# choyingw/SynergyNet

Hardware: AMD Instinct MI355X
Metric: faces/sec (120x120, 68-lmk + 53215-vert) (higher is better)
Workload: dtype f32 (fp16x2 split operands, fp32 accumulate)

## Files before the change

include/synergy_hip.h:

```cpp
#ifndef SYNERGY_HIP_H
#define SYNERGY_HIP_H

#include <stddef.h>
#include <stdint.h>

#ifdef __cplusplus
extern "C" {
#endif

typedef struct syn_handle syn_handle;

typedef enum {
    SYN_OK = 0,
    SYN_ERR_INVALID = -1,
    SYN_ERR_HIP = -2,
    SYN_ERR_NOT_LOADED = -3,
    SYN_ERR_PARAM_LEN = -4
} syn_status;

#define SYN_PARAM_DIM 62
#define SYN_POOL_DIM 1280
#define SYN_STD_SIZE 120

const char *syn_last_error(void);
int syn_abi_version(void);

int syn_create(int device, syn_handle **out);
int syn_destroy(syn_handle *h);


size_t syn_backbone_flat_count(void);

int syn_load_backbone(syn_handle *h, const float *flat, size_t n_floats);

int syn_numerics_report(syn_handle *h, char *buf, size_t n);

int syn_set_schedule(syn_handle *h, int fusion);

int syn_backbone_calibrate(syn_handle *h, const uint8_t *crops_u8, int B, float tol, void *stream);

int syn_backbone_range_status(syn_handle *h, float *layer_max, int max_layers, int fallback);
int syn_backbone_range_events(syn_handle *h);

size_t syn_resnet50_flat_count(void);
int syn_load_backbone_resnet50(syn_handle *h, const float *flat, size_t n_floats);
double syn_resnet50_flops_per_face(void);

int syn_load_basis(syn_handle *h, const float *w_shp, const float *w_exp, const float *u,
                   const float *param_mean, const float *param_std,
                   const int64_t *keypoints, int n_lmk, int n_vert);

size_t syn_constants_bytes(syn_handle *h);
int syn_export_constants(syn_handle *h, void *dev_dst, size_t bytes, void *stream);
int syn_import_constants(syn_handle *h, const void *dev_src, size_t bytes, void *stream);
int syn_bcast_constants(syn_handle *h, void *nccl_comm, int root, void *stream);
int syn_describe_constants(syn_handle *h, void *host_header, size_t bytes);

size_t syn_pack_constants_host_bytes(int arch, int have_backbone, int n_vert, int n_lmk);
int syn_pack_constants_host(int arch, const float *backbone_flat, size_t n_floats, const float *w_shp, const float *w_exp,
                            const float *u, const float *param_mean, const float *param_std, const int64_t *keypoints,
                            int n_lmk, int n_vert, void *host_dst, size_t bytes);
int syn_check_constants_host(const void *host_blob, size_t bytes);


size_t syn_workspace_bytes(syn_handle *h, int B);

int syn_backbone_forward(syn_handle *h, const float *img, int B, float *param, float *pool,
                         void *stream);

int syn_backbone_forward_u8(syn_handle *h, const uint8_t *img_hwc, int B, float *param,
                            float *pool, void *stream);

int syn_crop_resize(syn_handle *h, const uint8_t *frame, int H, int W, const int *box, const int *xofs,
                    const int16_t *xcoef, const int *yofs, const int16_t *ycoef, uint8_t *out, int B, void *stream);

int syn_crop_resize_frames(syn_handle *h, const uint8_t *frames, const long long *frame_off, const int *frame_dim,
                           const int *face_frame, const int *box, const int *xofs, const int16_t *xcoef, const int *yofs,
                           const int16_t *ycoef, uint8_t *out, int B, void *stream);

int syn_reconstruct(syn_handle *h, const float *param, int B, int param_len, int dense,
                    int transform, const float *roi, float *out, void *stream);

int syn_reconstruct_pitched(syn_handle *h, const float *param, int B, int param_len, int dense,
                            int transform, const float *roi, float *out, int row_pitch, int pad_writable, void *stream);

int syn_load_triangles(syn_handle *h, const int32_t *tri, int ntri, int nver);

int syn_mesh_shade(syn_handle *h, const float *vertices, int F, int planar, const float *cfg16, float *normal,
                   float *light, void *stream);

int syn_rasterize(syn_handle *h, const float *vertices, const float *colors, int F, int planar, int channels,
                  uint8_t *image, int H, int W, int reverse, void *stream);

int syn_add_weighted(syn_handle *h, const uint8_t *a, float alpha, const uint8_t *b, float beta, uint8_t *out,
                     size_t n, void *stream);

int syn_load_uv_map(syn_handle *h, const int32_t *coord_u, const int32_t *coord_v, int nver, const int32_t *keep_ind, int n_keep,
                    const int32_t *tri_kept, int ntri_kept);

int syn_select_topology(syn_handle *h, int slot);

int syn_uv_colors(syn_handle *h, const uint8_t *uv_tex, int T, int tex_h, int tex_w, int channels, int kept, int normalize, float *out,
                  void *stream);

int syn_gather_vertices(syn_handle *h, const float *vertices, int F, int planar, float *out, void *stream);

int syn_mesh_shade_textured(syn_handle *h, const float *vertices, int F, int planar, const float *cfg16, float *normal, float *light,
                            float *tex, int shared, float *colors, void *stream);

int syn_rasterize_triangles(syn_handle *h, const float *vertices, int F, int planar, float *depth_buffer, int32_t *triangle_buffer,
                            float *barycentric_weight, int H, int W, void *stream);

int syn_vertex_visibility(syn_handle *h, const int32_t *triangle_buffer, int F, int H, int W, uint8_t *visible, void *stream);

int syn_sample_vertex_colors(syn_handle *h, const float *vertices, int F, int planar, const uint8_t *image, int H, int W, int channels,
                             int normalize, float *out, void *stream);

int syn_uv_scatter(syn_handle *h, const float *colors, const uint8_t *visible, int F, int channels, uint8_t *tex, uint8_t *mask, int tex_h,
                   int tex_w, void *stream);

int syn_texture_fill(syn_handle *h, const uint8_t *tex_in, const uint8_t *mask, int T, int tex_h, int tex_w, int channels, int merge,
                     uint8_t *tex_out, void *stream);

int syn_load_tex_coords(syn_handle *h, const float *tex_coords, int tex_nver, const int32_t *tex_triangles);

int syn_render_texture(syn_handle *h, const float *vertices, int F, int planar, const void *texture, int tex_u8, int T, int tex_h, int tex_w,
                       int tex_c, int mapping_type, void *image, int image_u8, float *depth_buffer, int H, int W, int c, int shared,
                       void *stream);

size_t syn_detector_flat_count(void);
int syn_load_detector(syn_handle *h, const float *flat, size_t count);
int syn_detector_prior_count(int Hs, int Ws);
int syn_detect(syn_handle *h, const uint8_t *frame, int H, int W, int Hs, int Ws, float scale, float conf_thr, float nms_thr,
               int top_k, int keep_top_k, float *dets, int *n_dets, void *stream);

int syn_nme(syn_handle *h, const float *fit, const float *gt, const float *roi, float *nme, int N, void *stream);

int syn_pose(syn_handle *h, const float *param, int B, const float *roi, double *angles,
             float *t3d, void *stream);

int syn_landmarks_pose(syn_handle *h, const float *param, int B, int param_len, int transform, const float *roi ,
                       float *lmk, double *angles , float *t3d , void *stream);

int syn_pose_matrix(syn_handle *h, const float *param, int B, float *pmat, void *stream);

size_t syn_synergy_flat_count(void);
size_t syn_synergy_folded_count(void);
int syn_fold_synergy_host(const float *flat, size_t n, float *folded, size_t n_folded);

int syn_load_synergy(syn_handle *h, const float *flat, size_t n);

int syn_refine_landmarks(syn_handle *h, const float *param , const float *pool , int B, int transform,
                         const float *roi , float *lmk_coarse , float *lmk_refined ,
                         float *global_feat , void *stream);

int syn_refine_points(syn_handle *h, const float *lmk , const float *pool, const float *param, int B, float *lmk_refined,
                      float *global_feat , void *stream);

int syn_landmarks_to_param(syn_handle *h, const float *lmk , int B, float *param , void *stream);


int syn_backbone_launch_count(syn_handle *h);

int syn_backbone_profile(syn_handle *h, const uint8_t *img_hwc, int B, int max_launches,
                         int *feature_of_launch, float *ms_of_launch, double *flops_of_launch);

int syn_reconstruct_profile(syn_handle *h, const float *param, int B, const float *roi, float *out, int row_pitch, int pad_writable,
                            float *ms2);

double syn_backbone_flops_per_face(void);
double syn_pointwise_flops_per_face(void);

#ifdef __cplusplus
}
#endif
#endif
```

synergynet_amd/abi.py:

```python
from __future__ import annotations

import ctypes as C
import os

import torch

from .build import LIB

SYN_ERR_INVALID, SYN_ERR_NOT_LOADED = -1, -3
SYN_ERR_PARAM_LEN = -4
_lib = None


class SynergyHipError(RuntimeError):
    def __init__(self, code, msg):
        super().__init__(f'libsynergy_hip: {msg} (status {code})')
        self.code = code
        self.msg = msg


_SIGS = {
    'syn_last_error': (C.c_char_p, []),
    'syn_abi_version': (C.c_int, []),
    'syn_create': (C.c_int, [C.c_int, C.POINTER(C.c_void_p)]),
    'syn_destroy': (C.c_int, [C.c_void_p]),
    'syn_backbone_flat_count': (C.c_size_t, []),
    'syn_load_backbone': (C.c_int, [C.c_void_p, C.c_void_p, C.c_size_t]),
    'syn_numerics_report': (C.c_int, [C.c_void_p, C.c_char_p, C.c_size_t]),
    'syn_set_schedule': (C.c_int, [C.c_void_p, C.c_int]),
    'syn_backbone_range_status': (C.c_int, [C.c_void_p, C.c_void_p, C.c_int, C.c_int]),
    'syn_backbone_range_events': (C.c_int, [C.c_void_p]),
    'syn_backbone_calibrate': (C.c_int, [C.c_void_p, C.c_void_p, C.c_int, C.c_float, C.c_void_p]),
    'syn_resnet50_flat_count': (C.c_size_t, []),
    'syn_load_backbone_resnet50': (C.c_int, [C.c_void_p, C.c_void_p, C.c_size_t]),
    'syn_resnet50_flops_per_face': (C.c_double, []),
    'syn_load_basis': (C.c_int, [C.c_void_p] + [C.c_void_p] * 6 + [C.c_int, C.c_int]),
    'syn_constants_bytes': (C.c_size_t, [C.c_void_p]),
    'syn_export_constants': (C.c_int, [C.c_void_p, C.c_void_p, C.c_size_t, C.c_void_p]),
    'syn_import_constants': (C.c_int, [C.c_void_p, C.c_void_p, C.c_size_t, C.c_void_p]),
    'syn_bcast_constants': (C.c_int, [C.c_void_p, C.c_void_p, C.c_int, C.c_void_p]),
    'syn_describe_constants': (C.c_int, [C.c_void_p, C.c_void_p, C.c_size_t]),
    'syn_pack_constants_host_bytes': (C.c_size_t, [C.c_int, C.c_int, C.c_int, C.c_int]),
    'syn_pack_constants_host': (C.c_int, [C.c_int, C.c_void_p, C.c_size_t] + [C.c_void_p] * 6 + [C.c_int, C.c_int, C.c_void_p, C.c_size_t]),
    'syn_check_constants_host': (C.c_int, [C.c_void_p, C.c_size_t]),
    'syn_workspace_bytes': (C.c_size_t, [C.c_void_p, C.c_int]),
    'syn_backbone_forward': (C.c_int, [C.c_void_p, C.c_void_p, C.c_int, C.c_void_p, C.c_void_p, C.c_void_p]),
    'syn_backbone_forward_u8': (C.c_int, [C.c_void_p, C.c_void_p, C.c_int, C.c_void_p, C.c_void_p, C.c_void_p]),
    'syn_crop_resize': (C.c_int, [C.c_void_p, C.c_void_p, C.c_int, C.c_int] + [C.c_void_p] * 6 + [C.c_int, C.c_void_p]),
    'syn_crop_resize_frames': (C.c_int, [C.c_void_p] * 11 + [C.c_int, C.c_void_p]),
    'syn_detector_flat_count': (C.c_size_t, []),
    'syn_load_detector': (C.c_int, [C.c_void_p, C.c_void_p, C.c_size_t]),
    'syn_detector_prior_count': (C.c_int, [C.c_int, C.c_int]),
    'syn_detect': (C.c_int, [C.c_void_p, C.c_void_p, C.c_int, C.c_int, C.c_int, C.c_int, C.c_float, C.c_float, C.c_float, C.c_int, C.c_int,
                             C.c_void_p, C.POINTER(C.c_int), C.c_void_p]),
    'syn_nme': (C.c_int, [C.c_void_p, C.c_void_p, C.c_void_p, C.c_void_p, C.c_void_p, C.c_int, C.c_void_p]),
    'syn_load_triangles': (C.c_int, [C.c_void_p, C.c_void_p, C.c_int, C.c_int]),
    'syn_mesh_shade': (C.c_int, [C.c_void_p, C.c_void_p, C.c_int, C.c_int, C.c_void_p, C.c_void_p, C.c_void_p, C.c_void_p]),
    'syn_rasterize': (C.c_int, [C.c_void_p, C.c_void_p, C.c_void_p, C.c_int, C.c_int, C.c_int, C.c_void_p, C.c_int, C.c_int, C.c_int, C.c_void_p]),
    'syn_add_weighted': (C.c_int, [C.c_void_p, C.c_void_p, C.c_float, C.c_void_p, C.c_float, C.c_void_p, C.c_size_t, C.c_void_p]),
    'syn_load_uv_map': (C.c_int, [C.c_void_p, C.c_void_p, C.c_void_p, C.c_int, C.c_void_p, C.c_int, C.c_void_p, C.c_int]),
    'syn_select_topology': (C.c_int, [C.c_void_p, C.c_int]),
    'syn_uv_colors': (C.c_int, [C.c_void_p, C.c_void_p, C.c_int, C.c_int, C.c_int, C.c_int, C.c_int, C.c_int, C.c_void_p, C.c_void_p]),
    'syn_gather_vertices': (C.c_int, [C.c_void_p, C.c_void_p, C.c_int, C.c_int, C.c_void_p, C.c_void_p]),
    'syn_mesh_shade_textured': (C.c_int, [C.c_void_p, C.c_void_p, C.c_int, C.c_int, C.c_void_p, C.c_void_p, C.c_void_p, C.c_void_p, C.c_int,
                                          C.c_void_p, C.c_void_p]),
    'syn_rasterize_triangles': (C.c_int, [C.c_void_p, C.c_void_p, C.c_int, C.c_int, C.c_void_p, C.c_void_p, C.c_void_p, C.c_int, C.c_int, C.c_void_p]),
    'syn_vertex_visibility': (C.c_int, [C.c_void_p, C.c_void_p, C.c_int, C.c_int, C.c_int, C.c_void_p, C.c_void_p]),
    'syn_sample_vertex_colors': (C.c_int, [C.c_void_p, C.c_void_p, C.c_int, C.c_int, C.c_void_p, C.c_int, C.c_int, C.c_int, C.c_int, C.c_void_p,
                                           C.c_void_p]),
    'syn_uv_scatter': (C.c_int, [C.c_void_p, C.c_void_p, C.c_void_p, C.c_int, C.c_int, C.c_void_p, C.c_void_p, C.c_int, C.c_int, C.c_void_p]),
    'syn_texture_fill': (C.c_int, [C.c_void_p, C.c_void_p, C.c_void_p, C.c_int, C.c_int, C.c_int, C.c_int, C.c_int, C.c_void_p, C.c_void_p]),
    'syn_load_tex_coords': (C.c_int, [C.c_void_p, C.c_void_p, C.c_int, C.c_void_p]),
    'syn_render_texture': (C.c_int, [C.c_void_p, C.c_void_p, C.c_int, C.c_int, C.c_void_p, C.c_int, C.c_int, C.c_int, C.c_int, C.c_int, C.c_int,
                                     C.c_void_p, C.c_int, C.c_void_p, C.c_int, C.c_int, C.c_int, C.c_int, C.c_void_p]),
    'syn_reconstruct': (C.c_int, [C.c_void_p, C.c_void_p, C.c_int, C.c_int, C.c_int, C.c_int, C.c_void_p, C.c_void_p, C.c_void_p]),
    'syn_reconstruct_pitched': (C.c_int, [C.c_void_p, C.c_void_p, C.c_int, C.c_int, C.c_int, C.c_int, C.c_void_p, C.c_void_p, C.c_int, C.c_int, C.c_void_p]),
    'syn_pose': (C.c_int, [C.c_void_p, C.c_void_p, C.c_int, C.c_void_p, C.c_void_p, C.c_void_p, C.c_void_p]),
    'syn_landmarks_pose': (C.c_int, [C.c_void_p, C.c_void_p, C.c_int, C.c_int, C.c_int, C.c_void_p, C.c_void_p, C.c_void_p, C.c_void_p, C.c_void_p]),
    'syn_pose_matrix': (C.c_int, [C.c_void_p, C.c_void_p, C.c_int, C.c_void_p, C.c_void_p]),
    'syn_synergy_flat_count': (C.c_size_t, []),
    'syn_synergy_folded_count': (C.c_size_t, []),
    'syn_fold_synergy_host': (C.c_int, [C.c_void_p, C.c_size_t, C.c_void_p, C.c_size_t]),
    'syn_load_synergy': (C.c_int, [C.c_void_p, C.c_void_p, C.c_size_t]),
    'syn_refine_landmarks': (C.c_int, [C.c_void_p, C.c_void_p, C.c_void_p, C.c_int, C.c_int, C.c_void_p, C.c_void_p, C.c_void_p, C.c_void_p, C.c_void_p]),
    'syn_refine_points': (C.c_int, [C.c_void_p, C.c_void_p, C.c_void_p, C.c_void_p, C.c_int, C.c_void_p, C.c_void_p, C.c_void_p]),
    'syn_landmarks_to_param': (C.c_int, [C.c_void_p, C.c_void_p, C.c_int, C.c_void_p, C.c_void_p]),
    'syn_backbone_launch_count': (C.c_int, [C.c_void_p]),
    'syn_backbone_profile': (C.c_int, [C.c_void_p, C.c_void_p, C.c_int, C.c_int, C.c_void_p, C.c_void_p, C.c_void_p]),
    'syn_reconstruct_profile': (C.c_int, [C.c_void_p, C.c_void_p, C.c_int, C.c_void_p, C.c_void_p, C.c_int, C.c_int, C.c_void_p]),
    'syn_backbone_flops_per_face': (C.c_double, []),
    'syn_pointwise_flops_per_face': (C.c_double, []),
}

EXPORTED_SYMBOLS = tuple(_SIGS)
_SIGS = dict(_SIGS, syn_debug_feature=(C.c_int, [C.c_void_p, C.c_void_p, C.c_int, C.c_int, C.c_void_p, C.c_void_p]),
             syn_debug_profile_block=(C.c_int, [C.c_void_p, C.c_void_p, C.c_int, C.c_int, C.c_void_p]),
             syn_debug_detect_raw=(C.c_int, [C.c_void_p, C.c_void_p, C.c_int, C.c_int, C.c_int, C.c_int, C.c_float] + [C.c_void_p] * 5),
             syn_debug_poison_workspace=(C.c_int, [C.c_void_p, C.c_int, C.c_int]))


def lib():
    global _lib
    if _lib is None:
        path = os.environ.get('SYNERGY_HIP_LIB', LIB)
        if not os.path.isfile(path):
            raise SynergyHipError(-100, f'{path} not built; run `python -c "import __graft_entry__ as g; g.build()"`')
        l = C.CDLL(path)
        for name, (res, args) in _SIGS.items():
            fn = getattr(l, name)
            fn.restype, fn.argtypes = res, args
        _lib = l
    return _lib


def check(rc: int):
    if rc != 0:
        msg = lib().syn_last_error().decode(errors='replace')
        raise SynergyHipError(rc, msg)
```

synergynet_amd/csrc/head_kernel.hip:

```cpp
#include <cstdlib>

#include "syn_internal.h"

namespace syn {

typedef float f32x4 __attribute__((ext_vector_type(4)));

namespace {
constexpr int NF = 2, PX = NF * 16, K = 320, KCH = K / 16, N = 1280, NTL = N / 16, XS = K + 4;
__device__ __forceinline__ float r6h(float v) { return __builtin_amdgcn_fmed3f(v, 0.0f, 6.0f); }
__device__ __forceinline__ float row16_sum(float v) {
    v += __builtin_bit_cast(float, __builtin_amdgcn_update_dpp(0, __builtin_bit_cast(int, v), 0xB1, 0xF, 0xF, true));
    v += __builtin_bit_cast(float, __builtin_amdgcn_update_dpp(0, __builtin_bit_cast(int, v), 0x4E, 0xF, 0xF, true));
    v += __builtin_bit_cast(float, __builtin_amdgcn_update_dpp(0, __builtin_bit_cast(int, v), 0x141, 0xF, 0xF, true));
    v += __builtin_bit_cast(float, __builtin_amdgcn_update_dpp(0, __builtin_bit_cast(int, v), 0x140, 0xF, 0xF, true));
    return v;
}
__device__ __forceinline__ float wave64_sum(float v) {
    const int b = __builtin_bit_cast(int, row16_sum(v));
    return __builtin_bit_cast(float, __builtin_amdgcn_readlane(b, 0)) + __builtin_bit_cast(float, __builtin_amdgcn_readlane(b, 16)) +
           __builtin_bit_cast(float, __builtin_amdgcn_readlane(b, 32)) + __builtin_bit_cast(float, __builtin_amdgcn_readlane(b, 48));
}
}

__global__ __launch_bounds__(256) void head_kernel(const float *__restrict__ X , const float *__restrict__ Wpk,
                                                   const float *__restrict__ scale, const float *__restrict__ shift,
                                                   const float *__restrict__ Wfc , const float *__restrict__ bfc,
                                                   float *__restrict__ param, float *__restrict__ pool, int B) {
    __shared__ __attribute__((aligned(16))) float Xs[PX * XS];
    __shared__ __attribute__((aligned(16))) float Ps[NF * N];
    const int tid = threadIdx.x, lane = tid & 63, wave = __builtin_amdgcn_readfirstlane(tid >> 6);
    const int r16 = lane & 15, g = lane >> 4;
    const int f0 = blockIdx.x * NF;
    const f32x4 z4 = {0.f, 0.f, 0.f, 0.f};

    f32x4 an[KCH], hn;
    auto fetch = [&](int nt) {
        const float *w = Wpk + (size_t)nt * KCH * 256 + lane * 4;
#pragma unroll
        for (int kc = 0; kc < KCH; ++kc) an[kc] = *(const f32x4 *)(w + kc * 256);
        hn = *(const f32x4 *)&shift[nt * 16 + 4 * g];
    };
    fetch(wave);
    for (int it = tid; it < PX * (K / 4); it += 256) {
        const int c4 = it % (K / 4), p = it / (K / 4);
        const int f = f0 + (p >> 4);
        f32x4 v = z4;
        if (f < B) v = *(const f32x4 *)&X[((size_t)f * 16 + (p & 15)) * K + 4 * c4];
        *(f32x4 *)&Xs[p * XS + 4 * c4] = v;
    }
    __syncthreads();

    for (int nt = wave; nt < NTL; nt += 4) {
        f32x4 a[KCH];
#pragma unroll
        for (int kc = 0; kc < KCH; ++kc) a[kc] = an[kc];
        const f32x4 sh = hn;
        if (nt + 4 < NTL) fetch(nt + 4);
        f32x4 acc[NF];
#pragma unroll
        for (int j = 0; j < NF; ++j) acc[j] = sh;
        f32x4 bc[NF], bn[NF];
#pragma unroll
        for (int j = 0; j < NF; ++j) bc[j] = *(const f32x4 *)&Xs[(j * 16 + r16) * XS + 4 * g];
#pragma unroll
        for (int kc = 0; kc < KCH; ++kc) {
            if (kc + 1 < KCH) {
#pragma unroll
                for (int j = 0; j < NF; ++j) bn[j] = *(const f32x4 *)&Xs[(j * 16 + r16) * XS + (kc + 1) * 16 + 4 * g];
            }
#pragma unroll
            for (int s = 0; s < 4; ++s)
#pragma unroll
                for (int j = 0; j < NF; ++j) acc[j] = __builtin_amdgcn_mfma_f32_16x16x4f32(a[kc][s], bc[j][s], acc[j], 0, 0, 0);
#pragma unroll
            for (int j = 0; j < NF; ++j) bc[j] = bn[j];
            __builtin_amdgcn_sched_barrier(0);
        }
#pragma unroll
        for (int j = 0; j < NF; ++j) {
            f32x4 v;
#pragma unroll
            for (int t = 0; t < 4; ++t) v[t] = r6h(acc[j][t]);
#pragma unroll
            for (int t = 0; t < 4; ++t) v[t] = row16_sum(v[t]);
            if (r16 == 0) *(f32x4 *)&Ps[j * N + nt * 16 + 4 * g] = v * 0.0625f;
        }
    }
    __syncthreads();
    if (pool) {
        for (int it = tid; it < NF * (N / 4); it += 256) {
            const int j = it / (N / 4), c4 = it % (N / 4);
            if (f0 + j < B) *(f32x4 *)&pool[(size_t)(f0 + j) * N + 4 * c4] = *(const f32x4 *)&Ps[j * N + 4 * c4];
        }
    }
    {
        f32x4 xv[NF][N / 256];
#pragma unroll
        for (int j = 0; j < NF; ++j)
#pragma unroll
            for (int i = 0; i < N / 256; ++i) xv[j][i] = *(const f32x4 *)&Ps[j * N + (i * 64 + lane) * 4];
#pragma unroll 2
        for (int o = wave; o < kParam; o += 4) {
            const float *wr = Wfc + (size_t)o * N;
            f32x4 wv[N / 256];
#pragma unroll
            for (int i = 0; i < N / 256; ++i) wv[i] = *(const f32x4 *)&wr[(i * 64 + lane) * 4];
            const float bo = bfc[o];
#pragma unroll
            for (int j = 0; j < NF; ++j) {
                float a = 0.f;
#pragma unroll
                for (int i = 0; i < N / 256; ++i)
                    a += wv[i][0] * xv[j][i][0] + wv[i][1] * xv[j][i][1] + wv[i][2] * xv[j][i][2] + wv[i][3] * xv[j][i][3];
                const float tot = wave64_sum(a);
                if (lane == 0 && f0 + j < B) param[(size_t)(f0 + j) * kParam + o] = tot + bo;
            }
        }
    }
}

void launch_head(const float *X, const float *Wpk, const float *scale, const float *shift, const float *Wfc,
                 const float *bfc, float *param, float *pool, int B, hipStream_t s) {
    head_kernel<<<(B + NF - 1) / NF, 256, 0, s>>>(X, Wpk, scale, shift, Wfc, bfc, param, pool, B);
}


typedef _Float16 f16x8 __attribute__((ext_vector_type(8)));
typedef _Float16 f16x2 __attribute__((ext_vector_type(2)));
typedef unsigned u32x4 __attribute__((ext_vector_type(4)));
typedef unsigned u32x2 __attribute__((ext_vector_type(2)));

namespace {
constexpr int KC32 = K / 32;
constexpr int XSD = K / 2 + 4;
constexpr int PLANE = PX * XSD;
__device__ __forceinline__ void split2(float x0, float x1, unsigned &a, unsigned &b) {
    a = __builtin_bit_cast(unsigned, __builtin_amdgcn_cvt_pkrtz(x0, x1));
    float r0, r1;
    asm("v_fma_mix_f32 %0, %1, -1.0, %2 op_sel_hi:[1,0,0]" : "=v"(r0) : "v"(a), "v"(x0));
    asm("v_fma_mix_f32 %0, %1, -1.0, %2 op_sel:[1,0,0] op_sel_hi:[1,0,0]" : "=v"(r1) : "v"(a), "v"(x1));
    b = __builtin_bit_cast(unsigned, __builtin_amdgcn_cvt_pkrtz(r0, r1));
}
__device__ __forceinline__ f32x4 mfma_h(u32x4 a, u32x4 b, f32x4 c) {
    return __builtin_amdgcn_mfma_f32_16x16x32_f16(__builtin_bit_cast(f16x8, a), __builtin_bit_cast(f16x8, b), c, 0, 0, 0);
}
}

template <int NR, int NFK = NF, int NWV = 4>
__device__ __forceinline__ void fc_rows(const f32x4 (&xv)[NFK][N / 256], const float *__restrict__ Wfc, const float *__restrict__ bfc,
                                        float *__restrict__ param, int f0, int B, int rbase, int wave, int lane) {
    f32x4 wq[2][N / 256];
    auto ldw = [&](int o, f32x4(&w)[N / 256]) {
        const float *wr = Wfc + (size_t)(o < kParam ? o : kParam - 1) * N;
#pragma unroll
        for (int i = 0; i < N / 256; ++i) w[i] = *(const f32x4 *)&wr[(i * 64 + lane) * 4];
    };
    ldw(wave + NWV * rbase, wq[0]);
#pragma unroll
    for (int r = 0; r < NR; ++r) {
        const int o = wave + NWV * (rbase + r);
        if (r + 1 < NR) ldw(o + NWV, wq[(r + 1) & 1]);
        if (o >= kParam) continue;
        const f32x4(&wv)[N / 256] = wq[r & 1];
        const float bo = bfc[o];
#pragma unroll
        for (int j = 0; j < NFK; ++j) {
            float a = 0.f;
#pragma unroll
            for (int i = 0; i < N / 256; ++i)
                a += wv[i][0] * xv[j][i][0] + wv[i][1] * xv[j][i][1] + wv[i][2] * xv[j][i][2] + wv[i][3] * xv[j][i][3];
            const float tot = wave64_sum(a);
            if (lane == 0 && f0 + j < B) param[(size_t)(f0 + j) * kParam + o] = tot + bo;
        }
    }
}

constexpr int kFcRounds = (kParam + 3) / 4;

template <int NS, int NFK = NF, int NWV = 4, bool SIN = false>
__global__ __launch_bounds__(NWV * 64) void head_f16x2_kernel(const float *__restrict__ X ,
                                                          const unsigned *__restrict__ Wb3 ,
                                                          const float *__restrict__ shift, const float *__restrict__ Wfc,
                                                          const float *__restrict__ bfc, float *__restrict__ param,
                                                          float *__restrict__ pool, int B, HeadSliced hs = HeadSliced{nullptr, 0, nullptr, nullptr}) {
    constexpr int PXK = NFK * 16, PLANEK = PXK * XSD, NT = NWV * 64;
    __shared__ __attribute__((aligned(16))) unsigned Xb[2 * PLANEK];
    __shared__ __attribute__((aligned(16))) float Ps[NFK * N];
    const int tid = threadIdx.x, lane = tid & 63, wave = __builtin_amdgcn_readfirstlane(tid >> 6);
    const int r16 = lane & 15, g = lane >> 4;
    const int gsw = g ^ (((r16 >> 2) ^ (r16 >> 3)) & 1);
    const int f0 = blockIdx.x * NFK;
    const float S = __builtin_bit_cast(float, Wb3[80 * 10 * 2 * 256]), inv_s = __builtin_bit_cast(float, Wb3[80 * 10 * 2 * 256 + 1]);
    constexpr int NTS = NTL / NS;
    static_assert(NTL % NS == 0 && NTS % NWV == 0, "whole rounds of the waves per slice");
    const int nt0 = NS > 1 ? (int)blockIdx.y * NTS : 0, nt_end = nt0 + NTS;

    u32x4 ring[5][2];
    auto lda = [&](int nt, int kc, u32x4(&dst)[2]) {
        const unsigned *w = Wb3 + ((size_t)(nt * KC32 + kc) * 2) * 256 + lane * 4;
#pragma unroll
        for (int p = 0; p < 2; ++p) dst[p] = *(const u32x4 *)(w + p * 256);
    };
#pragma unroll
    for (int kc = 0; kc < 5; ++kc) lda(nt0 + wave, kc, ring[kc]);
    {
        constexpr int XI = PXK * (K / 4) / NT;
        static_assert(PXK * (K / 4) % NT == 0, "whole rounds");
        f32x4 xv[XI];
        if constexpr (SIN) {
            const size_t total = (size_t)B * 16 * K;
            size_t at[XI];
#pragma unroll
            for (int ii = 0; ii < XI; ++ii) {
                const int it = tid + ii * NT, c4 = it % (K / 4), p = it / (K / 4);
                int f = f0 + (p >> 4);
                f = f < B ? f : B - 1;
                at[ii] = ((size_t)f * 16 + (p & 15)) * K + 4 * c4;
                xv[ii] = *(const f32x4 *)&hs.part[at[ii]];
            }
            for (int sl = 1; sl < hs.S; sl += 2) {
                const bool two = sl + 1 < hs.S;
                f32x4 t0[XI], t1[XI];
#pragma unroll
                for (int ii = 0; ii < XI; ++ii) t0[ii] = *(const f32x4 *)&hs.part[(size_t)sl * total + at[ii]];
#pragma unroll
                for (int ii = 0; ii < XI; ++ii) t1[ii] = *(const f32x4 *)&hs.part[(size_t)(two ? sl + 1 : sl) * total + at[ii]];
#pragma unroll
                for (int ii = 0; ii < XI; ++ii) { xv[ii] += t0[ii]; if (two) xv[ii] += t1[ii]; }
            }
            const float inv_p = *hs.inv_p;
#pragma unroll
            for (int ii = 0; ii < XI; ++ii) {
                const int c4 = (tid + ii * NT) % (K / 4);
                xv[ii] = xv[ii] * inv_p + *(const f32x4 *)&hs.p_shift[4 * c4];
            }
        } else {
#pragma unroll
        for (int ii = 0; ii < XI; ++ii) {
            const int it = tid + ii * NT, c4 = it % (K / 4), p = it / (K / 4);
            int f = f0 + (p >> 4);
            f = f < B ? f : B - 1;
            xv[ii] = *(const f32x4 *)&X[((size_t)f * 16 + (p & 15)) * K + 4 * c4];
        }
        }
#pragma unroll
        for (int ii = 0; ii < XI; ++ii) asm volatile("" : "+v"(xv[ii]));
#pragma unroll
        for (int ii = 0; ii < XI; ++ii) {
            const int it = tid + ii * NT, c4 = it % (K / 4), p = it / (K / 4);
            const f32x4 v = f0 + (p >> 4) < B ? xv[ii] : (f32x4){0.f, 0.f, 0.f, 0.f};
            unsigned a0, b0, a1, b1;
            split2(v[0], v[1], a0, b0);
            split2(v[2], v[3], a1, b1);
            const int csw = ((((c4 >> 1) ^ ((((p & 15) >> 2) ^ ((p & 15) >> 3)) & 1)) << 1) | (c4 & 1)) * 2;
            *(u32x2 *)&Xb[0 * PLANEK + p * XSD + csw] = (u32x2){a0, a1};
            *(u32x2 *)&Xb[1 * PLANEK + p * XSD + csw] = (u32x2){b0, b1};
        }
    }
    __syncthreads();

    f32x4 sh_n = *(const f32x4 *)&shift[(nt0 + wave) * 16 + 4 * g];
    auto tile = [&](int nt) __attribute__((always_inline)) {
        const f32x4 sh = sh_n * S;
        sh_n = *(const f32x4 *)&shift[(nt + NWV < nt_end ? nt + NWV : nt) * 16 + 4 * g];
        f32x4 acc[NFK];
#pragma unroll
        for (int j = 0; j < NFK; ++j) acc[j] = sh;
        u32x4 bq[2][NFK][2];
        auto ldb = [&](int kc, u32x4(&b)[NFK][2]) {
#pragma unroll
            for (int j = 0; j < NFK; ++j)
#pragma unroll
                for (int p = 0; p < 2; ++p) b[j][p] = *(const u32x4 *)&Xb[p * PLANEK + (j * 16 + r16) * XSD + kc * 16 + 4 * gsw];
        };
        ldb(0, bq[0]);
#pragma unroll
        for (int kc = 0; kc < KC32; ++kc) {
            if (kc + 1 < KC32) ldb(kc + 1, bq[(kc + 1) & 1]);
            const u32x4(&bc)[NFK][2] = bq[kc & 1];
            const u32x4 aa = ring[kc % 5][0], ab = ring[kc % 5][1];
#pragma unroll
            for (int j = 0; j < NFK; ++j) acc[j] = mfma_h(ab, bc[j][0], acc[j]);
#pragma unroll
            for (int j = 0; j < NFK; ++j) acc[j] = mfma_h(aa, bc[j][1], acc[j]);
#pragma unroll
            for (int j = 0; j < NFK; ++j) acc[j] = mfma_h(aa, bc[j][0], acc[j]);
            if (kc + 5 < KC32) lda(nt, kc + 5, ring[kc % 5]);
            else lda(nt + NWV < nt_end ? nt + NWV : nt, kc + 5 - KC32, ring[kc % 5]);
            __builtin_amdgcn_sched_barrier(0);
        }
#pragma unroll
        for (int j = 0; j < NFK; ++j) {
            f32x4 v;
#pragma unroll
            for (int t = 0; t < 4; ++t) v[t] = row16_sum(r6h(acc[j][t] * inv_s));
            if (r16 == 0) *(f32x4 *)&Ps[j * N + nt * 16 + 4 * g] = v * 0.0625f;
        }
    };
    tile(nt0 + wave);
    for (int nt = nt0 + wave + NWV; nt < nt_end; nt += NWV) tile(nt);
    __syncthreads();
    if (NS > 1) {
        for (int it = tid; it < NFK * (NTS * 4); it += NT) {
            const int j = it / (NTS * 4), c4 = nt0 * 4 + it % (NTS * 4);
            if (f0 + j < B) *(f32x4 *)&pool[(size_t)(f0 + j) * N + 4 * c4] = *(const f32x4 *)&Ps[j * N + 4 * c4];
        }
        return;
    }
    if (pool) {
        for (int it = tid; it < NFK * (N / 4); it += NT) {
            const int j = it / (N / 4), c4 = it % (N / 4);
            if (f0 + j < B) *(f32x4 *)&pool[(size_t)(f0 + j) * N + 4 * c4] = *(const f32x4 *)&Ps[j * N + 4 * c4];
        }
    }
    f32x4 xv[NFK][N / 256];
#pragma unroll
    for (int j = 0; j < NFK; ++j)
#pragma unroll
        for (int i = 0; i < N / 256; ++i) xv[j][i] = *(const f32x4 *)&Ps[j * N + (i * 64 + lane) * 4];
    fc_rows<(kParam + NWV - 1) / NWV, NFK, NWV>(xv, Wfc, bfc, param, f0, B, 0, wave, lane);
}

constexpr int kFcSlices = 4;
__global__ __launch_bounds__(256) void head_fc_kernel(const float *__restrict__ pool, const float *__restrict__ Wfc,
                                                      const float *__restrict__ bfc, float *__restrict__ param, int B) {
    const int tid = threadIdx.x, lane = tid & 63, wave = __builtin_amdgcn_readfirstlane(tid >> 6);
    const int f0 = blockIdx.x * NF;
    f32x4 xv[NF][N / 256];
#pragma unroll
    for (int j = 0; j < NF; ++j) {
        const int f = f0 + j < B ? f0 + j : B - 1;
#pragma unroll
        for (int i = 0; i < N / 256; ++i) xv[j][i] = *(const f32x4 *)&pool[(size_t)f * N + (i * 64 + lane) * 4];
    }
    fc_rows<kFcRounds / kFcSlices>(xv, Wfc, bfc, param, f0, B, blockIdx.y * (kFcRounds / kFcSlices), wave, lane);
}

void launch_head_f16x2(const float *X, const unsigned *Wb3, const float *shift, const float *Wfc, const float *bfc,
                        float *param, float *pool, float *scratch, int B, hipStream_t s, const HeadSliced *sin) {
    const int grid = (B + NF - 1) / NF;
    if (grid <= 96) {
        float *pl = pool ? pool : scratch;
        if (sin) head_f16x2_kernel<5, NF, 4, true><<<dim3(grid, 5), 256, 0, s>>>(X, Wb3, shift, Wfc, bfc, param, pl, B, *sin);
        else head_f16x2_kernel<5><<<dim3(grid, 5), 256, 0, s>>>(X, Wb3, shift, Wfc, bfc, param, pl, B);
        head_fc_kernel<<<dim3(grid, kFcSlices), 256, 0, s>>>(pl, Wfc, bfc, param, B);
        return;
    }
    if (sin) {
        head_f16x2_kernel<1, NF, 4, true><<<grid, 256, 0, s>>>(X, Wb3, shift, Wfc, bfc, param, pool, B, *sin);
        return;
    }
    static const int wide_min = (int)test_knob("head_wide_min", 513);
    if (B >= wide_min) {
        head_f16x2_kernel<1, 4, 8><<<(B + 3) / 4, 512, 0, s>>>(X, Wb3, shift, Wfc, bfc, param, pool, B);
        return;
    }
    head_f16x2_kernel<1><<<grid, 256, 0, s>>>(X, Wb3, shift, Wfc, bfc, param, pool, B);
}
}
```

synergynet_amd/csrc/recon_kernels.hip:

```cpp
#include <cstdio>
#include <cstdlib>

#include "syn_internal.h"

namespace syn {

typedef float f32x2 __attribute__((ext_vector_type(2)));
typedef float f32x4 __attribute__((ext_vector_type(4)));
typedef float f32x16 __attribute__((ext_vector_type(16)));

__device__ __forceinline__ void lds_barrier() { asm volatile("s_waitcnt lgkmcnt(0)\n\ts_barrier" ::: "memory"); }

constexpr int kFaceRec = 64;
constexpr int kStageStride = 132;

__global__ __launch_bounds__(64) void recon_prep_kernel(const float *__restrict__ param, const float *__restrict__ mean,
                                                        const float *__restrict__ stdv, const float *__restrict__ roi,
                                                        int transform, float *__restrict__ rec, int B) {
    const int b = blockIdx.x;
    const int l = threadIdx.x;
    __shared__ float p[64];
    if (l < kParam) p[l] = param[(size_t)b * kParam + l] * stdv[l] + mean[l];
    __syncthreads();
    float *r = rec + (size_t)b * kFaceRec;
    if (l < 50) r[l] = p[12 + l];
    else if (l == 50) r[l] = 1.0f;
    else if (l == 51) r[l] = 0.0f;
    else if (l < 55) {
        const int c = l - 52;
        float sc = 1.0f, of = 0.0f;
        if (roi) {
            const float sx = roi[b * 5 + 0], sy = roi[b * 5 + 1], ex = roi[b * 5 + 2], ey = roi[b * 5 + 3];
            const float scx = (ex - sx) / 120.0f, scy = (ey - sy) / 120.0f;
            if (c == 0) { sc = scx; of = sx; }
            else if (c == 1) { sc = scy; of = sy; }
            else { sc = (scx + scy) * 0.5f; }
        }
        float m0 = p[4 * c + 0], m1 = p[4 * c + 1], m2 = p[4 * c + 2], t = p[4 * c + 3];
        if (transform && c == 1) { m0 = -m0; m1 = -m1; m2 = -m2; t = (float)(kImg + 1) - t; }
        r[52 + 3 * c + 0] = m0 * sc;
        r[52 + 3 * c + 1] = m1 * sc;
        r[52 + 3 * c + 2] = m2 * sc;
        r[61 + c] = t * sc + of;
    }
}

__global__ __launch_bounds__(256) void recon_kernel(const float *__restrict__ rec, const float *__restrict__ basis,
                                                    float *__restrict__ out, int B, int n_vert, int pitch, int n_tiles,
                                                    int n_split, int ftiles_per_split, int n_ftiles, int n_units) {
    __shared__ __attribute__((aligned(16))) float smt[4][32][12];
    __shared__ __attribute__((aligned(16))) float stage[96 * kStageStride];
    const int lane = threadIdx.x & 63, wave = __builtin_amdgcn_readfirstlane(threadIdx.x >> 6);
    const int per_xcd = (n_units + 7) / 8;
    const int unit = (blockIdx.x & 7) * per_xcd + (blockIdx.x >> 3);
    if ((int)(blockIdx.x >> 3) >= per_xcd || unit >= n_units) return;
    const int tg = unit / n_split, split = unit - tg * n_split;
    int T = tg * 4 + wave;
    const bool t_ok = T < n_tiles;
    T = t_ok ? T : n_tiles - 1;
    const int j = lane & 31, h = lane >> 5;

    f32x4 bw[3][6];
    f32x2 bt[3];
    const float *bp = basis + (size_t)T * 3 * (kBasisK * 32);
#pragma unroll
    for (int c = 0; c < 3; ++c) {
        const float *bc = bp + c * (kBasisK * 32);
#pragma unroll
        for (int t = 0; t < 6; ++t) bw[c][t] = *(const f32x4 *)(bc + t * 256 + lane * 4);
        bt[c] = *(const f32x2 *)(bc + 6 * 256 + lane * 2);
    }
    const int ft0 = split * ftiles_per_split;
    int ft1 = ft0 + ftiles_per_split;
    ft1 = ft1 < n_ftiles ? ft1 : n_ftiles;
    float(*mt)[12] = smt[wave];
    const int v_base = tg * 128;
    if ((blockIdx.x >> 8) & 1) __builtin_amdgcn_s_sleep(56);

    for (int ft = ft0; ft < ft1; ++ft) {
        const int f0 = ft * 32;
        int fa = f0 + j;
        fa = fa < B ? fa : B - 1;
        const float *ra = rec + (size_t)fa * kFaceRec;
        f32x4 aw[6];
#pragma unroll
        for (int t = 0; t < 6; ++t) aw[t] = *(const f32x4 *)(ra + 8 * t + 4 * h);
        const f32x2 at = *(const f32x2 *)(ra + 48 + 2 * h);
        if (lane < 32) {
#pragma unroll
            for (int q = 0; q < 3; ++q) *(f32x4 *)&mt[lane][4 * q] = *(const f32x4 *)(ra + 52 + 4 * q);
        }
        f32x16 acc[3];
#pragma unroll
        for (int c = 0; c < 3; ++c) {
#pragma unroll
            for (int r = 0; r < 16; ++r) acc[c][r] = 0.f;
#pragma unroll
            for (int t = 0; t < 6; ++t)
#pragma unroll
                for (int s = 0; s < 4; ++s)
                    acc[c] = __builtin_amdgcn_mfma_f32_32x32x2f32(aw[t][s], bw[c][t][s], acc[c], 0, 0, 0);
#pragma unroll
            for (int s = 0; s < 2; ++s) acc[c] = __builtin_amdgcn_mfma_f32_32x32x2f32(at[s], bt[c][s], acc[c], 0, 0, 0);
        }
        __builtin_amdgcn_fence(__ATOMIC_RELEASE, "wavefront");
        __builtin_amdgcn_wave_barrier();
        __builtin_amdgcn_fence(__ATOMIC_ACQUIRE, "wavefront");
#pragma unroll
        for (int r = 0; r < 16; ++r) {
            const int i = (r & 3) + 8 * (r >> 2) + 4 * h;
            const f32x4 q0 = *(const f32x4 *)&mt[i][0];
            const f32x4 q1 = *(const f32x4 *)&mt[i][4];
            const f32x4 q2 = *(const f32x4 *)&mt[i][8];
            const float sx = acc[0][r], sy = acc[1][r], sz = acc[2][r];
            float *st = stage + (i * 3) * kStageStride + wave * 32 + j;
            st[0] = q0[0] * sx + q0[1] * sy + q0[2] * sz + q2[1];
            st[kStageStride] = q0[3] * sx + q1[0] * sy + q1[1] * sz + q2[2];
            st[2 * kStageStride] = q1[2] * sx + q1[3] * sy + q2[0] * sz + q2[3];
        }
        lds_barrier();
        {
            const int seg = threadIdx.x & 31, rsub = threadIdx.x >> 5;
            const int vq = v_base + 4 * seg;
#pragma unroll
            for (int k = 0; k < 12; ++k) {
                const int row = k * 8 + rsub;
                const int f = f0 + row / 3, c = row % 3;
                const f32x4 vv = *(const f32x4 *)&stage[row * kStageStride + 4 * seg];
                if (f < B) {
                    float *o = out + ((size_t)f * 3 + c) * pitch + vq;
                    if (vq + 3 < n_vert) *(f32x4 *)o = vv;
                    else {
#pragma unroll
                        for (int t = 0; t < 4; ++t) if (vq + t < n_vert) o[t] = vv[t];
                    }
                }
            }
        }
        lds_barrier();
    }
}

void launch_reconstruct(const float *param, const float *mean62, const float *std62, const float *basis, int n_vert,
                        int nvp, const float *roi, int transform, float *out, int pitch, int B, hipStream_t s, float *rec) {
    recon_prep_kernel<<<B, 64, 0, s>>>(param, mean62, std62, roi, transform, rec, B);
    const int n_tiles = nvp / 32;
    const int n_groups = (n_tiles + 3) / 4;
    const int n_ftiles = (B + 31) / 32;
    int n_split = (3072 + n_groups - 1) / n_groups;
    n_split = n_split < 1 ? 1 : n_split;
    n_split = n_split > n_ftiles ? n_ftiles : n_split;
    const int per = (n_ftiles + n_split - 1) / n_split;
    n_split = (n_ftiles + per - 1) / per;
    const int n_units = n_groups * n_split;
    const int grid = ((n_units + 7) / 8) * 8;
    recon_kernel<<<grid, 256, 0, s>>>(rec, basis, out, B, n_vert, pitch, n_tiles, n_split, per, n_ftiles, n_units);
}

typedef unsigned u32x4 __attribute__((ext_vector_type(4)));
typedef _Float16 f16x8r __attribute__((ext_vector_type(8)));
typedef _Float16 f16x2r __attribute__((ext_vector_type(2)));

namespace {
__device__ __forceinline__ void split2r(float x0, float x1, unsigned &a, unsigned &b) {
    a = __builtin_bit_cast(unsigned, __builtin_amdgcn_cvt_pkrtz(x0, x1));
    float r0, r1;
    asm("v_fma_mix_f32 %0, %1, -1.0, %2 op_sel_hi:[1,0,0]" : "=v"(r0) : "v"(a), "v"(x0));
    asm("v_fma_mix_f32 %0, %1, -1.0, %2 op_sel:[1,0,0] op_sel_hi:[1,0,0]" : "=v"(r1) : "v"(a), "v"(x1));
    b = __builtin_bit_cast(unsigned, __builtin_amdgcn_cvt_pkrtz(r0, r1));
}
__device__ __forceinline__ f32x16 mfma32(u32x4 a, u32x4 b, f32x16 c) {
    return __builtin_amdgcn_mfma_f32_32x32x16_f16(__builtin_bit_cast(f16x8r, a), __builtin_bit_cast(f16x8r, b), c, 0, 0, 0);
}
}

__global__ __launch_bounds__(64) void recon_prep_f16_kernel(const float *__restrict__ param, const float *__restrict__ mean,
                                                           const float *__restrict__ stdv, const float *__restrict__ roi,
                                                           int transform, unsigned *__restrict__ rec3, int B) {
    const int ft = blockIdx.x, l = threadIdx.x, i = l & 31, hh = l >> 5;
    const int b = ft * 32 + i;
    const bool ok = b < B;
    const float *pp = param + (size_t)(ok ? b : 0) * kParam;
    unsigned *rt = rec3 + (size_t)ft * kRecTileF16;
    float al[3][8];
    float amax = 0.f;
#pragma unroll
    for (int ks = 0; ks < 3; ++ks)
#pragma unroll
        for (int e = 0; e < 8; ++e) {
            const int k = 12 + 16 * ks + 8 * hh + e;
            al[ks][e] = ok ? pp[k] * stdv[k] + mean[k] : 0.f;
            amax = fmaxf(amax, fabsf(al[ks][e]));
        }
    const float a48 = ok ? pp[12 + 48] * stdv[12 + 48] + mean[12 + 48] : 0.f;
    const float a49 = ok ? pp[12 + 49] * stdv[12 + 49] + mean[12 + 49] : 0.f;
    amax = fmaxf(amax, fmaxf(fabsf(a48), fabsf(a49)));
    amax = fmaxf(amax, __shfl_xor(amax, 32));
    const float cu = mean[62];
    amax = fmaxf(amax, cu);
    int ex = (int)((__builtin_bit_cast(unsigned, amax) >> 23) & 0xff) - 126;
    ex = 14 - ex;
    const int ex_cu = (int)((__builtin_bit_cast(unsigned, cu) >> 23) & 0xff) - 127;
    ex = ex < -14 - ex_cu ? -14 - ex_cu : ex;
    ex = ex < -100 ? -100 : (ex > 100 ? 100 : ex);
    const float Sa = __builtin_bit_cast(float, (unsigned)(127 + ex) << 23);
    const float inv_ab = __builtin_bit_cast(float, (unsigned)(127 - ex) << 23);
#pragma unroll
    for (int ks = 0; ks < 3; ++ks) {
        u32x4 pc[2];
#pragma unroll
        for (int d = 0; d < 4; ++d) {
            unsigned a, b2;
            split2r(al[ks][2 * d] * Sa, al[ks][2 * d + 1] * Sa, a, b2);
            pc[0][d] = a; pc[1][d] = b2;
        }
#pragma unroll
        for (int p = 0; p < 2; ++p) *(u32x4 *)&rt[((ks * 2 + p) * 64 + l) * 4] = pc[p];
    }
    {
        unsigned a, b2;
        split2r(a48 * Sa, a49 * Sa, a, b2);
        const unsigned a8 = a & 0xffffu, b8 = b2 & 0xffffu, a9 = a >> 16, b9 = b2 >> 16;
        const unsigned sa16 = ok ? (__builtin_bit_cast(unsigned, __builtin_amdgcn_cvt_pkrtz(cu * Sa, cu * Sa)) & 0xffffu) : 0u;
        u32x4 fx = {0u, 0u, 0u, 0u};
        if (hh == 0) fx = (u32x4){a8 | (b8 << 16), a8 | (a9 << 16), b9 | (a9 << 16), sa16 | (sa16 << 16)};
        *(u32x4 *)&rt[(6 * 64 + l) * 4] = fx;
    }
    if (hh == 0) {
        float r[16];
        float p12[12];
#pragma unroll
        for (int q = 0; q < 12; ++q) p12[q] = ok ? pp[q] * stdv[q] + mean[q] : 0.f;
#pragma unroll
        for (int c = 0; c < 3; ++c) {
            float sc = 1.0f, of = 0.0f;
            if (roi && ok) {
                const float sx = roi[b * 5 + 0], sy = roi[b * 5 + 1], ex = roi[b * 5 + 2], ey = roi[b * 5 + 3];
                const float scx = (ex - sx) / 120.0f, scy = (ey - sy) / 120.0f;
                if (c == 0) { sc = scx; of = sx; }
                else if (c == 1) { sc = scy; of = sy; }
                else { sc = (scx + scy) * 0.5f; }
            }
            float m0 = p12[4 * c + 0], m1 = p12[4 * c + 1], m2 = p12[4 * c + 2], t = p12[4 * c + 3];
            if (transform && c == 1) { m0 = -m0; m1 = -m1; m2 = -m2; t = (float)(kImg + 1) - t; }
            r[3 * c + 0] = m0 * sc * inv_ab; r[3 * c + 1] = m1 * sc * inv_ab; r[3 * c + 2] = m2 * sc * inv_ab;
            r[9 + c] = t * sc + of;
        }
        r[12] = 0.f; r[13] = 0.f; r[14] = 0.f; r[15] = 0.f;
        float *rr = reinterpret_cast<float *>(rt + 7 * 256) + i * 16;
#pragma unroll
        for (int q = 0; q < 4; ++q) *(f32x4 *)&rr[4 * q] = (f32x4){r[4 * q], r[4 * q + 1], r[4 * q + 2], r[4 * q + 3]};
    }
}

#define RLAP(i) do { if (PROF) { asm volatile("s_waitcnt vmcnt(0) lgkmcnt(0)" ::: "memory"); tn = __builtin_amdgcn_s_memtime(); pt_[i] += tn - tk; tk = tn; } } while (0)
template <int WPG, bool FAST, bool PROF = false, bool PK = false>
__global__ __launch_bounds__(WPG * 64) __attribute__((amdgpu_waves_per_eu(2, 2)))
void recon_f16_kernel(const unsigned *__restrict__ rec3, const unsigned *__restrict__ basis3, float *__restrict__ out, int B,
                     int n_vert, int pitch, int n_tiles, int n_split, int ftiles_per_split, int ft_lo, int ft_hi, int n_units,
                     unsigned long long *prof = nullptr) {
    unsigned long long pt_[8] = {0, 0, 0, 0, 0, 0, 0, 0}, tk = PROF ? __builtin_amdgcn_s_memtime() : 0ull, tn = 0;
    constexpr int SS = WPG * 32 + 4;
    constexpr int NTH = WPG * 64, TQ = kRecTileF16 / 4, NPF = (TQ + NTH - 1) / NTH, TQP = NPF * NTH;
    __shared__ __attribute__((aligned(16))) unsigned optile[2][TQP * 4];
    __shared__ __attribute__((aligned(16))) float stage[96 * SS];
    const int lane = threadIdx.x & 63, wave = __builtin_amdgcn_readfirstlane(threadIdx.x >> 6);
    const int per_xcd = (n_units + 7) / 8;
    const int unit = (blockIdx.x & 7) * per_xcd + (blockIdx.x >> 3);
    if ((int)(blockIdx.x >> 3) >= per_xcd || unit >= n_units) return;
    const int tg = unit / n_split, split = unit - tg * n_split;
    constexpr int RUN = WPG * 32;
    static_assert(!PK || !FAST, "the packed-row schedule has its own store path");
    constexpr int PKW = (WPG - 1) * 32;
    int T = tg * (PK ? WPG - 1 : WPG) + wave;
    T = T < n_tiles ? T : n_tiles - 1;
    const int j = lane & 31, h = lane >> 5;

    u32x4 bb[3][3][2], bx[3];
#pragma unroll
    for (int c = 0; c < 3; ++c) {
        const unsigned *bc = basis3 + ((size_t)T * 3 + c) * kBasisF16;
#pragma unroll
        for (int ks = 0; ks < 3; ++ks)
#pragma unroll
            for (int p = 0; p < 2; ++p) bb[c][ks][p] = *(const u32x4 *)(bc + ((ks * 2 + p) * 64 + lane) * 4);
        bx[c] = *(const u32x4 *)(bc + (6 * 64 + lane) * 4);
    }
    const int ft0 = ft_lo + split * ftiles_per_split;
    int ft1 = ft0 + ftiles_per_split;
    ft1 = ft1 < ft_hi ? ft1 : ft_hi;
    const int v_base = tg * (PK ? PKW : RUN);
    if (ft0 >= ft1) return;

    u32x4 pf[NPF];
    auto fetch = [&](int ft) {
        const unsigned *rt = rec3 + (size_t)ft * kRecTileF16;
#pragma unroll
        for (int i = 0; i < NPF; ++i) pf[i] = *(const u32x4 *)(rt + 4 * (i * NTH + (int)threadIdx.x));
    };
    auto park = [&](int buf) {
#pragma unroll
        for (int i = 0; i < NPF; ++i) *(u32x4 *)&optile[buf][4 * (i * NTH + (int)threadIdx.x)] = pf[i];
    };
    fetch(ft0);
    park(0);
    __builtin_amdgcn_s_waitcnt(0x0F70);
    RLAP(0);
    lds_barrier();

    for (int ft = ft0; ft < ft1; ++ft) {
        const int f0 = ft * 32, buf = (ft - ft0) & 1;
        const unsigned *ot = optile[buf];
        f32x16 acc[3];
        {
            const u32x4 ax = *(const u32x4 *)(ot + (6 * 64 + lane) * 4);
            const f32x16 z16 = {0.f, 0.f, 0.f, 0.f, 0.f, 0.f, 0.f, 0.f, 0.f, 0.f, 0.f, 0.f, 0.f, 0.f, 0.f, 0.f};
#pragma unroll
            for (int c = 0; c < 3; ++c) acc[c] = mfma32(bx[c], ax, z16);
        }
#pragma unroll
        for (int ks = 0; ks < 3; ++ks) {
            u32x4 aa[2];
#pragma unroll
            for (int p = 0; p < 2; ++p) aa[p] = *(const u32x4 *)(ot + ((ks * 2 + p) * 64 + lane) * 4);
            constexpr int PA[3] = {1, 0, 0}, PB[3] = {0, 1, 0};
#pragma unroll
            for (int q = 0; q < 3; ++q)
#pragma unroll
                for (int c = 0; c < 3; ++c) acc[c] = mfma32(bb[c][ks][PB[q]], aa[PA[q]], acc[c]);
        }
        RLAP(1);
        fetch(ft + 1 < ft1 ? ft + 1 : ft);
        RLAP(2);
        {
            const float *rec = reinterpret_cast<const float *>(ot + 7 * 256) + j * 16;
// ... 20 lines not shown
        {
            if constexpr (PK) {
                constexpr int LPRK = PKW / 4, RPIK = WPG * 64 / LPRK, NIT = (96 + RPIK - 1) / RPIK;
                int tid_ = threadIdx.x;
                asm volatile("" : "+v"(tid_));
                const int seg = tid_ % LPRK, rsub = tid_ / LPRK;
                const int nv32 = n_vert & 31;
                const long long r0 = 3ll * f0;
                long long tile_rows = 3ll * B - r0;
                tile_rows = tile_rows < 96 ? tile_rows : 96;
                const __amdgpu_buffer_rsrc_t rs_o = __builtin_amdgcn_make_buffer_rsrc(out + (size_t)r0 * n_vert, 0, (int)(tile_rows * n_vert * 4), 0x00027000);
#pragma unroll
                for (int k = 0; k < NIT; ++k) {
                    const int rr = RPIK * k + rsub;
                    const int sh = (32 - (int)(((r0 + rr) * nv32) & 31)) & 31;
                    const int vq = v_base + sh + 4 * seg;
                    const float *sp = &stage[(rr < 96 ? rr : 95) * SS + sh + 4 * seg];
                    const f32x4 vv = {sp[0], sp[1], sp[2], sp[3]};
                    const bool ok = rsub < RPIK && rr < 96 && vq + 3 < n_vert;
                    __builtin_amdgcn_raw_buffer_store_b128(__builtin_bit_cast(u32x4, vv), rs_o, ok ? (unsigned)(rr * n_vert + vq) * 4u : 0x80000000u, 0, 0);
                }
                __builtin_amdgcn_sched_barrier(0);
                park(buf ^ 1);
                __builtin_amdgcn_sched_barrier(0);
                if (tg == 0 || v_base + PKW + 31 + 3 >= n_vert) {
#pragma unroll 1
                    for (int k = 0; k < NIT; ++k) {
                        const int rr = RPIK * k + rsub;
                        const long long r = r0 + rr;
                        if (rsub >= RPIK || rr >= 96 || r >= 3ll * B) continue;
                        const int sh = (32 - (int)((r * nv32) & 31)) & 31;
                        const int vq = v_base + sh + 4 * seg;
                        if (vq < n_vert && vq + 3 >= n_vert) {
                            for (int t = 0; t < 4; ++t) if (vq + t < n_vert) out[(size_t)r * n_vert + vq + t] = stage[rr * SS + sh + 4 * seg + t];
                        }
                        if (tg == 0 && 4 * seg < sh) {
                            for (int t = 0; t < 4; ++t) if (4 * seg + t < sh) out[(size_t)r * n_vert + 4 * seg + t] = stage[rr * SS + 4 * seg + t];
                        }
                    }
                }
            } else {
            constexpr int LPR = RUN / 4, RPI = WPG * 64 / LPR;
            int tid_ = threadIdx.x;
            asm volatile("" : "+v"(tid_));
            const int seg = tid_ % LPR, rsub = tid_ / LPR;
            const int vq = v_base + 4 * seg;
            const int rows_live = 3 * (B - f0);
            float *o = out + ((size_t)3 * f0 + rsub) * pitch + vq;
            const size_t ostep = (size_t)RPI * pitch;
            const float *sp = &stage[rsub * SS + 4 * seg];
            if (FAST) {
#pragma unroll
                for (int k = 0; k < 96 / RPI; ++k, o += ostep) *(f32x4 *)o = *(const f32x4 *)(sp + k * RPI * SS);
            } else {
                const bool whole = vq + 3 < n_vert;
#pragma unroll
                for (int k = 0; k < 96 / RPI; ++k, o += ostep) {
                    const f32x4 vv = *(const f32x4 *)(sp + k * RPI * SS);
                    if (k * RPI + rsub < rows_live) {
                        if (whole) *(f32x4 *)o = vv;
                        else {
#pragma unroll
                            for (int t = 0; t < 4; ++t) if (vq + t < n_vert) o[t] = vv[t];
                        }
                    }
                }
            }
            __builtin_amdgcn_sched_barrier(0);
            park(buf ^ 1);
            }
        }
        RLAP(5);
        lds_barrier();
        RLAP(6);
    }
    if (PROF && threadIdx.x == 0) {
        for (int i = 0; i < 7; ++i) atomicAdd(&prof[i], pt_[i]);
        atomicAdd(&prof[7], 1ull);
    }
}

void launch_reconstruct_f16(const float *param, const float *mean62, const float *std62, const unsigned *basis3, int n_vert,
                           int nvp, const float *roi, int transform, float *out, int pitch, int pad_writable, int B, hipStream_t s, float *rec3f,
                           hipEvent_t *marks ) {
    unsigned *rec3 = reinterpret_cast<unsigned *>(rec3f);
    const int n_ftiles = (B + 31) / 32;
    if (marks) (void)hipEventRecord(marks[0], s);
    recon_prep_f16_kernel<<<n_ftiles, 64, 0, s>>>(param, mean62, std62, roi, transform, rec3, B);
    if (marks) (void)hipEventRecord(marks[1], s);
    const int n_tiles = nvp / 32;
    constexpr int WPG = 4;
    const int fast_groups = (n_tiles + WPG - 1) / WPG;
    const bool fast_ok = pad_writable && pitch >= fast_groups * WPG * 32;
    const bool pk = !fast_ok && pitch == n_vert && n_vert >= 4096 && (reinterpret_cast<uintptr_t>(out) & 127) == 0 && !test_knob("recon_no_pk", 0);
    static const int pk_wpg = (int)test_knob("recon_pk_wpg", 8);
    const int pkw = (pk_wpg == 8 ? 7 : 3) * 32;
    const int n_groups = pk ? (n_vert + pkw - 1) / pkw : fast_groups;
    static const int wg_target = (int)test_knob("recon_wgs", 1664);
    static const int prof3 = (int)test_knob("recon_prof", 0);
    auto run = [&](int lo, int hi, bool fast) {
        const int nft = hi - lo;
        if (nft <= 0) return;
        const int target = (pk && pk_wpg == 8 && !test_knob_set("recon_wgs")) ? wg_target / 2 : wg_target;
        int n_split = (target + n_groups - 1) / n_groups;
        n_split = n_split < 1 ? 1 : n_split;
        n_split = n_split > nft ? nft : n_split;
        const int per = (nft + n_split - 1) / n_split;
        n_split = (nft + per - 1) / per;
        const int n_units = n_groups * n_split;
        const int grid = ((n_units + 7) / 8) * 8;
        if (prof3 && fast && n_vert > 1000) {
            unsigned long long *d = nullptr, hst[8];
            (void)hipMalloc((void **)&d, sizeof(hst));
            (void)hipMemsetAsync(d, 0, sizeof(hst), s);
            recon_f16_kernel<WPG, true, true><<<grid, WPG * 64, 0, s>>>(rec3, basis3, out, B, n_vert, pitch, n_tiles, n_split, per, lo, hi, n_units, d);
            (void)hipStreamSynchronize(s);
            (void)hipMemcpy(hst, d, sizeof(hst), hipMemcpyDeviceToHost);
            (void)hipFree(d);
            const char *nm[7] = {"basis+first tile", "mfma", "fetch issue", "epilogue", "barrier1", "store+park", "barrier2"};
            for (int i = 0; i < 7; ++i) fprintf(stderr, "recon prof %-18s %10.0f ticks/wg\n", nm[i], (double)hst[i] / (double)hst[7]);
            fprintf(stderr, "recon prof workgroups %llu\n", hst[7]);
        } else if (fast)
            recon_f16_kernel<WPG, true><<<grid, WPG * 64, 0, s>>>(rec3, basis3, out, B, n_vert, pitch, n_tiles, n_split, per, lo, hi, n_units);
        else if (pk && pk_wpg == 8)
            recon_f16_kernel<8, false, false, true><<<grid, 8 * 64, 0, s>>>(rec3, basis3, out, B, n_vert, pitch, n_tiles, n_split, per, lo, hi, n_units);
        else if (pk)
            recon_f16_kernel<WPG, false, false, true><<<grid, WPG * 64, 0, s>>>(rec3, basis3, out, B, n_vert, pitch, n_tiles, n_split, per, lo, hi, n_units);
        else
            recon_f16_kernel<WPG, false><<<grid, WPG * 64, 0, s>>>(rec3, basis3, out, B, n_vert, pitch, n_tiles, n_split, per, lo, hi, n_units);
    };
    if (fast_ok) {
        run(0, B / 32, true);
        run(B / 32, n_ftiles, false);
    } else
        run(0, n_ftiles, false);
    if (marks) (void)hipEventRecord(marks[2], s);
}

__device__ __forceinline__ void pose_of_face(const float (&p)[12], const float *__restrict__ roi5 , double *__restrict__ angles3 ,
                                             float *__restrict__ t3d3, float *__restrict__ pmat12 ) {
    const float n1 = sqrtf(p[0] * p[0] + p[1] * p[1] + p[2] * p[2]);
    const float n2 = sqrtf(p[4] * p[4] + p[5] * p[5] + p[6] * p[6]);
    const float r1[3] = {p[0] / n1, p[1] / n1, p[2] / n1};
    const float r2[3] = {p[4] / n2, p[5] / n2, p[6] / n2};
    const float r3[3] = {r1[1] * r2[2] - r1[2] * r2[1], r1[2] * r2[0] - r1[0] * r2[2], r1[0] * r2[1] - r1[1] * r2[0]};
    const double PI = 3.14159265358979323846;
    double x, y, z;
    if (r3[0] != 1.0f && r3[0] != -1.0f) {
        x = asin((double)r3[0]);
        const double cx = cos(x);
        y = atan2((double)r2[2] / cx, (double)r3[2] / cx);
        z = atan2((double)r1[1] / cx, (double)r1[0] / cx);
    } else {
        z = 0.0;
        if (r3[0] == -1.0f) { x = PI / 2; y = z + atan2((double)r1[1], (double)r1[2]); }
        else                { x = -PI / 2; y = -z + atan2(-(double)r1[1], -(double)r1[2]); }
    }
    if (pmat12) {
        float *m = pmat12;
        m[0] = r1[0]; m[1] = r1[1]; m[2] = r1[2]; m[3] = p[3];
        m[4] = r2[0]; m[5] = r2[1]; m[6] = r2[2]; m[7] = p[7];
        m[8] = r3[0]; m[9] = r3[1]; m[10] = r3[2]; m[11] = p[11];
    }
    if (!angles3) return;
    angles3[0] = x * 180.0 / PI;
    angles3[1] = y * 180.0 / PI;
    angles3[2] = z * 180.0 / PI;
    float tx = p[3], ty = p[7], tz = p[11];
    if (roi5) {
        const float sx = roi5[0], sy = roi5[1], ex = roi5[2], ey = roi5[3];
        tx = tx * ((ex - sx) / 120.0f) + sx;
        ty = ty * ((ey - sy) / 120.0f) + sy;
    }
    t3d3[0] = tx;
    t3d3[1] = ty;
    t3d3[2] = tz;
}

__global__ __launch_bounds__(64) void pose_kernel(const float *__restrict__ param, const float *__restrict__ mean,
                                                  const float *__restrict__ stdv, const float *__restrict__ roi,
                                                  double *__restrict__ angles, float *__restrict__ t3d,
                                                  float *__restrict__ pmat , int B) {
    const int b = blockIdx.x * 64 + threadIdx.x;
    if (b >= B) return;
    float p[12];
#pragma unroll
    for (int i = 0; i < 12; ++i) p[i] = param[(size_t)b * kParam + i] * stdv[i] + mean[i];
    pose_of_face(p, roi ? roi + (size_t)b * 5 : nullptr, angles ? angles + (size_t)b * 3 : nullptr, t3d + (size_t)b * 3, pmat ? pmat + (size_t)b * 12 : nullptr);
}

void launch_pose(const float *param, const float *mean62, const float *std62, const float *roi, double *angles,
                 float *t3d, float *pmat, int B, hipStream_t s) {
    pose_kernel<<<(B + 63) / 64, 64, 0, s>>>(param, mean62, std62, roi, angles, t3d, pmat, B);
}

__global__ __launch_bounds__(256) void lmk_pose_kernel(const float *__restrict__ param, const float *__restrict__ mean, const float *__restrict__ stdv,
                                                       const float *__restrict__ basis , int n_lmk, int nlp,
                                                       const float *__restrict__ roi, int transform, float *__restrict__ lmk ,
                                                       double *__restrict__ angles, float *__restrict__ t3d, int B) {
    const int b = blockIdx.x, l = threadIdx.x;
    __shared__ float p[64];
    if (l < kParam) p[l] = param[(size_t)b * kParam + l] * stdv[l] + mean[l];
    __syncthreads();
    if (l == 255 && angles) {
        float pp[12];
#pragma unroll
        for (int i = 0; i < 12; ++i) pp[i] = p[i];
        pose_of_face(pp, roi ? roi + (size_t)b * 5 : nullptr, angles + (size_t)b * 3, t3d + (size_t)b * 3, nullptr);
    }
    float aff[12];
#pragma unroll
    for (int c = 0; c < 3; ++c) {
        float sc = 1.0f, of = 0.0f;
        if (roi) {
            const float sx = roi[b * 5 + 0], sy = roi[b * 5 + 1], ex = roi[b * 5 + 2], ey = roi[b * 5 + 3];
            const float scx = (ex - sx) / 120.0f, scy = (ey - sy) / 120.0f;
            if (c == 0) { sc = scx; of = sx; }
            else if (c == 1) { sc = scy; of = sy; }
            else { sc = (scx + scy) * 0.5f; }
        }
        float m0 = p[4 * c + 0], m1 = p[4 * c + 1], m2 = p[4 * c + 2], t = p[4 * c + 3];
        if (transform && c == 1) { m0 = -m0; m1 = -m1; m2 = -m2; t = (float)(kImg + 1) - t; }
        aff[3 * c + 0] = m0 * sc;
        aff[3 * c + 1] = m1 * sc;
        aff[3 * c + 2] = m2 * sc;
        aff[9 + c] = t * sc + of;
    }
    for (int v = l; v < n_lmk; v += 256) {
        const int T = v >> 5, j = v & 31;
        float S[3];
#pragma unroll
        for (int c = 0; c < 3; ++c) {
            const float *bc = basis + ((size_t)T * 3 + c) * (kBasisK * 32);
            float acc = 0.f;
#pragma unroll
            for (int t = 0; t < 6; ++t)
#pragma unroll
                for (int h = 0; h < 2; ++h) {
                    const f32x4 w = *(const f32x4 *)(bc + t * 256 + (32 * h + j) * 4);
#pragma unroll
                    for (int s = 0; s < 4; ++s) acc = __builtin_fmaf(w[s], p[12 + 8 * t + 4 * h + s], acc);
                }
            const f32x2 w0 = *(const f32x2 *)(bc + 6 * 256 + j * 2), w1 = *(const f32x2 *)(bc + 6 * 256 + (32 + j) * 2);
            acc = __builtin_fmaf(w0[0], p[12 + 48], acc);
            acc = __builtin_fmaf(w0[1], p[12 + 49], acc);
            acc += w1[0];
            S[c] = acc;
        }
#pragma unroll
        for (int c = 0; c < 3; ++c)
            lmk[((size_t)b * 3 + c) * n_lmk + v] = aff[3 * c + 0] * S[0] + aff[3 * c + 1] * S[1] + aff[3 * c + 2] * S[2] + aff[9 + c];
    }
}

void launch_lmk_pose(const float *param, const float *mean62, const float *std62, const float *basis_lmk, int n_lmk, int nlp, const float *roi,
                     int transform, float *lmk, double *angles, float *t3d, int B, hipStream_t s) {
    lmk_pose_kernel<<<B, 256, 0, s>>>(param, mean62, std62, basis_lmk, n_lmk, nlp, roi, transform, lmk, angles, t3d, B);
}

}
```

synergynet_amd/csrc/syn_internal.h:

```cpp
#pragma once
#include <hip/hip_runtime.h>
#include <stddef.h>
#include <stdint.h>

namespace syn {

#ifdef __HIPCC__
__device__ __forceinline__ void l2_touch(const void *base, unsigned bytes, unsigned gi, unsigned nth, unsigned &sink) {
    for (unsigned ofs = gi * 128u; ofs < bytes; ofs += nth * 128u) {
        const char *p = static_cast<const char *>(base) + ofs;
        asm volatile("global_load_dword %0, %1, off" : "+v"(sink) : "v"(p) : "memory");
    }
}
__device__ __forceinline__ void l2_touch_done(unsigned &sink) { asm volatile("s_waitcnt vmcnt(0)" : "+v"(sink) :: "memory"); }
#endif

long long test_knob(const char *name, long long dflt);
bool test_knob_set(const char *name);

constexpr int kImg = 120;
constexpr int kParam = 62;
constexpr int kPool = 1280;
constexpr int kBasisK = 52;
constexpr int kVertTile = 32;


void launch_stem(const float *img_nchw, const uint8_t *img_hwc_u8, const float *w27x32,
                 const float *scale, const float *shift, float *out, int B, hipStream_t s);

void launch_pointwise(const float *A, const float *W, const float *scale, const float *shift,
                      const float *residual, float *C, int M, int K, int Kpad, int N,
                      int relu6, hipStream_t s);

void launch_depthwise(const float *in, const float *w9xC, const float *scale, const float *shift,
                      float *out, int B, int Hin, int Hout, int C, int stride, hipStream_t s);

void launch_pool_fc(const float *feat , const float *Wfc ,
                    const float *bias , float *param , float *pool ,
                    int B, hipStream_t s);

struct FusedBlockArgs {
    const float *X;
    const float *We, *e_scale, *e_shift;
    const float *Wd, *d_scale, *d_shift;
    const float *Wp, *p_scale, *p_shift;
    float *Y;
    unsigned long long *prof = nullptr;
    const unsigned *We3 = nullptr, *Wp3 = nullptr;
    const float *scl_e = nullptr, *scl_p = nullptr;
    const unsigned *Arm_e = nullptr, *Arm_p = nullptr;
    const unsigned *Alb_p = nullptr;
    const unsigned *Alb_e = nullptr;
    const float *Tlb = nullptr;
    const unsigned *Glb = nullptr;
    float *scratch = nullptr;
    size_t scratch_floats = 0;
};
bool launch_fused_block(int feature, const FusedBlockArgs &a, int B, hipStream_t s);
constexpr int early_block_hc(int hid) { return hid % 32 == 0 ? 32 : 48; }
bool launch_fused_block_early(int feature, const FusedBlockArgs &a, int B, hipStream_t s);
constexpr int rm_expand_dwords(int cin, int hid) { return ((hid + 31) / 32) * ((cin + 15) / 16) * 512; }
constexpr int rm_project_dwords(int hid) { return ((hid + 31) / 32) * 2 * 512; }
bool launch_fused_block_rm(int feature, const FusedBlockArgs &a, int B, hipStream_t s);
bool launch_fused_pair_rm(int first, const FusedBlockArgs &a, const FusedBlockArgs &b, int B, hipStream_t s);
bool launch_fused_pair_f16(const FusedBlockArgs &a5, const FusedBlockArgs &a6, int B, hipStream_t s);
constexpr int lb_project_dwords(int hid, int cout) { return (hid / 32) * (cout / 16) * 512; }
constexpr int lb_expand_dwords(int cin, int hid) { return (hid / 16) * (cin / 32) * 512; }
constexpr int lb_table_floats(int hid) { return (hid / 32) * 12 * 32; }
bool launch_fused_block_lb(int feature, const FusedBlockArgs &a, int B, hipStream_t s);
int lb_chain_mode(int B, bool small = true);
bool launch_fused_chain_lb(const FusedBlockArgs *a, int first, int n_blocks, int B, hipStream_t s);
constexpr int lb4_group_dwords(int cin, int cout) { return (2 * (cin / 32) * 512 + (cout / 16) * 512 + 512 + 2047) / 2048 * 2048; }
bool launch_fused_block_lb4(int feature, const FusedBlockArgs &a, int B, hipStream_t s);
bool launch_fused_chain_lb4(const FusedBlockArgs *a, int B, hipStream_t s);
bool launch_fused_block_f16(int feature, const FusedBlockArgs &a, int B, hipStream_t s);

void launch_stem_block1(const float *img_nchw, const uint8_t *img_hwc_u8, const float *w0, const unsigned *w0b3, const float *s0,
                        const float *b0, const float *wd, const float *sd, const float *bd, const float *wp_pk,
                        const float *sp, const float *bp, float *Y, int B, hipStream_t s);

constexpr int rm_stem_set_dwords() { return 3 * 2 * 256 + 32 + 4; }
constexpr int rm_stem_dwords() { return 2 * rm_stem_set_dwords(); }
bool launch_stem_rm(const uint8_t *img8, const unsigned *As3, const float *s_shift, const float *Wd, const float *d_shift,
                    const unsigned *Ap3, const float *p_shift, const float *scl_p, float *Y, int B, hipStream_t s);
bool launch_stem_rm_f32(const float *img, const unsigned *As3, const float *s_shift, const float *Wd, const float *d_shift,
                        const unsigned *Ap3, const float *p_shift, const float *scl_p, float *Y, int B, hipStream_t s);

void launch_head(const float *X, const float *Wpk , const float *scale, const float *shift,
                 const float *Wfc , const float *bfc, float *param, float *pool , int B,
                 hipStream_t s);

struct HeadSliced {
    const float *part;
    int S;
    const float *inv_p;
    const float *p_shift;
};
void launch_head_f16x2(const float *X, const unsigned *Wb3 , const float *shift, const float *Wfc,
                        const float *bfc, float *param, float *pool, float *scratch , int B, hipStream_t s,
                       const HeadSliced *sliced_in = nullptr);
bool launch_lb4_sliced17_deferred(const FusedBlockArgs &a, int B, hipStream_t s, HeadSliced *out);

void launch_crop_resize(const uint8_t *frame, int H, int W, const int *box, const int *xofs, const short *xcoef,
                        const int *yofs, const short *ycoef, uint8_t *out, int B, hipStream_t s,
                        const long long *foff = nullptr, const int *fdim = nullptr, const int *fidx = nullptr);

constexpr int kFmtOutPair = 1, kFmtResPair = 2;
void launch_conv(const float *in, const float *W, const float *scale, const float *shift, const float *residual, float *out,
                 int B, int Hin, int Hout, int Cin, int N, int KH, int KW, int stride, int pad, int act, hipStream_t s,
                 float *stat = nullptr , int in_pair = 0, int fmt = 0);
void launch_conv_f16x2(const float *in, const unsigned *W3, const float *scale, const float *shift, const float *residual,
                     float *out, int B, int Hin, int Hout, int Cin, int N, int KH, int KW, int stride, int pad, int act,
                     hipStream_t s, float *stat = nullptr, int lt = 0 ,
                     int fmt = kFmtOutPair);
constexpr float kRangeHi = 6.0e4f, kRangeLo = 9.765625e-4f;
constexpr int kRangeSub = 64, kRangeStride = 64;
struct C2Args {
    const float *T1 = nullptr;
    const unsigned *W2 = nullptr;
    const float *scale2 = nullptr, *shift2 = nullptr;
    int Hin = 0, Hout = 0, stride = 1;
    unsigned in_bytes = 0;
    float *stat2 = nullptr;
};
bool launch_conv_c3f(const float *T2, const unsigned *W3, const float *scale3, const float *shift3, const float *identity, float *out,
                     const unsigned *W1f, const float *s1 , const float *scale1, const float *shift1, float *T1n, int M, int K, int N3, int N1,
                     hipStream_t s, float *stat3, float *stat1, int res_pair, const C2Args *c2 = nullptr);
bool launch_conv_c3f_ds(const float *T2, const unsigned *W3, const float *scale3, const float *shift3, const float *X, const unsigned *Wd,
                        const float *scale_d, const float *shift_d, float *out, const unsigned *W1f, const float *s1, const float *scale1,
                        const float *shift1, float *T1n, int M, int K, int Kd, int N3, int N1, hipStream_t s, float *stat3, float *stat1, const C2Args *c2 = nullptr);
bool launch_conv_dual(const float *a, const float *x, const unsigned *W3d, const float *ones, const float *shift, float *out, int B, int H, int C1,
                      int Hin2, int stride2, int Cin2, int N, int act, hipStream_t s, float *stat, int fmt);
bool conv_c3f_supported(int K, int N3, int N1);
void launch_resnet_stem(const float *img_nchw, const uint8_t *img_hwc_u8, const float *w147x64, const float *scale,
                        const float *shift, float *out , int B, hipStream_t s);
constexpr int rn_stem_dwords() { return 2 * 10 * 2 * 256 + 64 + 4; }
bool launch_resnet_stem_mfma(const uint8_t *img8, const unsigned *As3, const float *s_shift, float *out, int B, hipStream_t s, int pool = 0,
                             float *stat = nullptr, int out_pair = 0 );
void launch_maxpool3x3s2(const float *in, float *out, int B, int Hin, int Hout, int C, hipStream_t s, float *stat = nullptr, int out_pair = 0);
void launch_pool_fc_generic(const float *feat, const float *Wfc, const float *bias, float *param, float *pool, int B, int P,
                            int C, int n_out, int out_stride, hipStream_t s, const float *stat = nullptr, int n_stat = 0,
                            unsigned *guard_word = nullptr );

void launch_reconstruct(const float *param, const float *mean62, const float *std62,
                        const float *basis, int n_vert, int nvp, const float *roi,
                        int transform, float *out, int pitch , int B, hipStream_t s, float *rec);

constexpr int kBasisF16 = (3 * 2 + 1) * 256;
constexpr int kRecTileF16 = (3 * 2 + 1) * 256 + 32 * 16;
constexpr int kRecFloatsPerFace = 96;
constexpr int kRecSlack = 4096;
void launch_reconstruct_f16(const float *param, const float *mean62, const float *std62, const unsigned *basis3, int n_vert,
                           int nvp, const float *roi, int transform, float *out, int pitch, int pad_writable, int B, hipStream_t s, float *rec3,
                           hipEvent_t *marks = nullptr);

void launch_mesh_normals(const float *vertices, const int *tri, const int *adj_off, const int *adj_tri, float *tri_normal,
                         float *normal , unsigned *mm , int F, int nver,
                         int ntri, int planar, hipStream_t s);
void launch_mesh_lighting(const float *vertices, const float *normal, const unsigned *mm, const float *cfg ,
                          float *light , int F, int nver, int planar, hipStream_t s);
void launch_mesh_lighting_tex(const float *vertices, const float *normal, const unsigned *mm, const float *cfg, float *light,
                              float *tex, int shared, float *colors , int F, int nver, int planar, hipStream_t s);
void launch_uv_colors(const unsigned char *uv_tex , const int *coord_u, const int *coord_v, const int *keep ,
                      float *out , int T, int n, int th, int tw, int ch, int normalize, hipStream_t s);
void launch_gather_vertices(const float *vertices , const int *keep, float *out , int F,
                            int n_keep, int pitch, hipStream_t s);
void launch_rasterize(const float *vertices, const int *tri, const float *colors , unsigned long long *zkey ,
                      unsigned char *image , int F, int nver, int ntri, int h, int w, int c, int planar,
                      int reverse, hipStream_t s);
void launch_add_weighted(const unsigned char *a, float alpha, const unsigned char *b, float beta, unsigned char *out, size_t n,
                         hipStream_t s);
void launch_rasterize_triangles(const float *vertices, const int *tri, unsigned long long *zkey , float *depth ,
                                int *tri_buf , float *weight , int F, int nver, int ntri, int h, int w, int planar,
                                hipStream_t s);
void launch_render_texture(const float *vertices, const int *tri, const int *tex_tri, const float *tex_coords ,
                           const void *texture, int tex_u8, int tex_per_face, int th, int tw, int tc, int mapping, unsigned long long *zkey,
                           void *image, int image_u8, float *depth, int F, int nver, int ntri, int h, int w, int c, int planar, int shared,
                           hipStream_t s);
void launch_vertex_visibility(const int *tri_buf , const int *tri, unsigned char *visible , int F,
                              int nver, int ntri, int h, int w, hipStream_t s);
void launch_sample_vertex_colors(const float *vertices, const unsigned char *image , float *out , int F, int nver,
                                 int h, int w, int ch, int planar, int normalize, hipStream_t s);
void launch_uv_scatter(const float *colors , const unsigned char *visible , const int *coord_u,
                       const int *coord_v, unsigned *owner , unsigned char *tex ,
                       unsigned char *mask , int F, int nver, int th, int tw, int ch, hipStream_t s);

constexpr int kTextureFillMaxDim = 4096;
size_t texture_fill_scratch_bytes(int Tout, int th, int tw, int ch);
void launch_texture_fill(const unsigned char *tex , const unsigned char *mask , unsigned *scratch,
                         unsigned char *out, int T, int th, int tw, int ch, int merge, hipStream_t s);

void launch_nme(const float *fit, const float *gt, const float *roi, float *nme, int N, hipStream_t s);

void launch_det_preproc(const unsigned char *frame, int H, int W, float *out, int Ho, int Wo, hipStream_t s);
void launch_det_conv(const float *in, const float *Wt, const float *shift, float *out, int Hi, int Wi, int cs_in, int ci0, int Cin, int Ho,
                     int Wo, int cs_out, int co0, int Cout, int K, int stride, int pad, int act, hipStream_t s);
void launch_det_pool(const float *in, float *out, int Hi, int Wi, int C, int Ho, int Wo, int stride, int is_max, hipStream_t s);
void launch_det_decode(const float *loc, const float *conf, int P, int Hn, int Wn, int H4, int W4, int H5, int W5, int H6, int W6,
                       float scale, float thr, float *cand, int *n_cand, int max_cand, float *boxes_out, float *scores_out,
                       hipStream_t s);
void launch_det_nms(const float *cand, const int *n_cand, int max_cand, int top_k, float nms_thr, int keep_top_k, float *dets, int *n_out,
                    hipStream_t s);
int det_sort_capacity();

constexpr int kSynPts = 68;
constexpr int kSynGlobal = 1024;
constexpr int kSynFaceK = kSynGlobal + kPool + 40 + 10;
constexpr int kSynFaceKpad = (kSynFaceK + 15) / 16 * 16;
struct SynTrunkW { const float *W[5], *scale[5], *shift[5]; };
struct SynHeadW {
    const float *W6p, *scale6, *shift6;
    const float *W7, *scale7, *shift7;
    const float *W8, *scale8, *shift8;
    const float *W9, *scale9, *shift9;
};
void launch_syn_trunk(const SynTrunkW &w, const float *lmk, int B, float *pf, float *gf, int gf_pitch, float *gf2, hipStream_t s);
void launch_syn_face_concat(const float *pool, const float *param, float *X6, int B, hipStream_t s);
void launch_syn_face_gemm(const float *X, int ldx, const float *W, int Kpad, const float *scale, const float *shift, float *out, int ldo,
                          int N, int B, hipStream_t s);
void launch_syn_point_head(const SynHeadW &w, const float *pf, const float *g6, const float *lmk_in, const float *roi, float *out, int B,
                           hipStream_t s);

void launch_pose(const float *param, const float *mean62, const float *std62, const float *roi,
                 double *angles , float *t3d, float *pmat , int B, hipStream_t s);
void launch_lmk_pose(const float *param, const float *mean62, const float *std62, const float *basis_lmk, int n_lmk, int nlp, const float *roi,
                     int transform, float *lmk, double *angles, float *t3d, int B, hipStream_t s);

}
```

synergynet_amd/csrc/synergy_abi.hip:

```cpp
#include "../../include/synergy_hip.h"

#include <algorithm>
#include <cmath>
#include <cstdarg>
#include <cstdio>
#include <cstdlib>
#include <cstring>
#include <dlfcn.h>
#include <string>
#include <vector>

#include "syn_internal.h"
#include "bcast_protocol.h"

namespace {

thread_local std::string g_err;

int fail(int code, const char *fmt, ...) {
    char buf[512];
    va_list ap;
    va_start(ap, fmt);
    vsnprintf(buf, sizeof buf, fmt, ap);
    va_end(ap);
// ... 196 lines not shown
            }
        size_t src = 0, dst = 0;
        std::vector<char> follows(convs.size(), 0);
        for (size_t bi = 1; bi < blocks.size(); ++bi) follows[blocks[bi].c1] = 1;
        for (auto &c : convs) {
            const size_t wn = (size_t)c.cout * c.cin * c.k * c.k;
            c.src_w = src; src += wn + 4 * (size_t)c.cout;
            const int npad = round_up(c.cout, 64);
            c.dst_w = dst; dst += (size_t)npad * c.cin * c.k * c.k;
            c.dst_scale = dst; dst += npad;
            c.dst_shift = dst; dst += npad;
            c.dst_w3 = 0;
            if (c.cin % 32 == 0) { c.dst_w3 = dst; dst += (size_t)npad * c.cin * c.k * c.k + 4; }
            if (c.cin == 3) { c.dst_wrm = dst; dst += syn::rn_stem_dwords(); }
            if (follows[&c - convs.data()] && c.cin <= 512) { c.dst_w1f = dst; dst += (size_t)c.cout * c.cin; }
            flops += 2.0 * c.cin * c.k * c.k * (double)c.cout * c.hout * c.hout;
            const size_t osz = (size_t)c.cout * c.hout * c.hout;
            buf_big = osz > buf_big ? osz : buf_big;
        }
        {
            int nd = 0;
            for (auto &b : blocks)
                if (b.ds >= 0 && convs[b.ds].stride == 2) {
                    const RConv &c3 = convs[b.c3], &cd = convs[b.ds];
                    b.dst_w3d = dst; dst += (size_t)c3.cout * (c3.cin + cd.cin) + 4;
                    b.dst_ones = dst; dst += c3.cout;
                    b.dst_shiftd = dst; dst += c3.cout;
                    b.dual_idx = nd++;
                }
        }
        buf_mid = 128 * 30 * 30;
        src_fc = src; src += (size_t)102 * 2048 + 102;
        flat_count = src;
        dst_fc_w = dst; dst += (size_t)104 * 2048;
        dst_fc_b = dst; dst += 104;
        dst_range = dst; dst += 4;
        packed_count = dst;
        flops += 2.0 * 2048 * 102;
    }
};
const ResNet50 &resnet50() {
    static const ResNet50 n;
    return n;
}

struct ConstHeader {
    uint64_t magic;
    uint32_t version, has_backbone, has_basis, n_vert, n_lmk, nvp, nlp, arch;
    uint64_t backbone_floats, basis_floats, total_bytes;
    uint8_t reserved[256 - 8 - 8 * 4 - 3 * 8];
};
static_assert(sizeof(ConstHeader) == 256, "header must be 256 bytes");
constexpr uint64_t kMagic = 0x53594e4833353558ull;
constexpr uint32_t kConstVersion = 6;

struct RangeInfo {
    uint32_t unsafe1 = 0, unsafe16 = 0;
    float in_bound[20] = {};
    float min_wmean[20] = {};
    float w_relerr[20] = {};
};

static_assert(sizeof(RangeInfo) <= 64 * sizeof(float), "RangeInfo must fit its slot in the backbone blob");

}

struct SynOffsets {
    size_t tW[2][5], tscale[2][5], tshift[2][5];
    size_t W6p, W6f, scale6, shift6, W7, scale7, shift7, W8, scale8, shift8, W9, scale9, shift9;
    size_t Wrev, scale_rev, shift_rev;
};

struct syn_handle {
    int device = 0;
    int arch = 0;
    float *d_backbone = nullptr;
    float *d_basis = nullptr;
    size_t basis_floats = 0;
    int n_vert = 0, n_lmk = 0, nvp = 0, nlp = 0;
    float *ws = nullptr;
    size_t ws_bytes = 0;
    float *rec = nullptr;
    size_t rec_bytes = 0;
    int *d_tri = nullptr, *d_adj_off = nullptr, *d_adj_tri = nullptr;
    int ntri = 0, tri_nver = 0;
    int *d_uv = nullptr;
    int uv_nver = 0, n_keep = 0, uv_max[4] = {0, 0, 0, 0};
    int *k_tri = nullptr, *k_adj_off = nullptr, *k_adj_tri = nullptr;
    int k_ntri = 0;
    int topo_slot = 0;
    float *d_texc[2] = {nullptr, nullptr};
    int texc_nver[2] = {0, 0}, texc_own_tri[2] = {0, 0};
    int tri_max[2] = {0, 0};
    void *rws = nullptr;
    size_t rws_bytes = 0;
    float *d_syn = nullptr;
    SynOffsets syn_off = {};
    float *sws = nullptr;
    size_t sws_bytes = 0;
    float *d_det = nullptr;
    void *dws = nullptr;
    size_t dws_bytes = 0;
    int early_rm = 2047;
    float *d_range = nullptr;
    uint32_t resnet_w_unsafe[3] = {0, 0, 0};
    int resnet_gemm = 1;
    int resnet_fuse = 4;
    int resnet_fp32 = 0;
    unsigned *guard_word = nullptr;
    unsigned *guard_word_dev = nullptr;
    int guard_armed = 0;
    int range_events = 0;
    RangeInfo ri;
    int range_guard = 1;
    int fusion = 2;
};

namespace {

size_t basis_float_count(int nvp, int nlp) {
    return (size_t)(nvp + nlp) * 3 * syn::kBasisK + 256 + (size_t)((nvp + nlp) / 32) * 3 * syn::kBasisF16;
}
const float *basis_dense(const syn_handle *h) { return h->d_basis; }
const float *basis_lmk(const syn_handle *h) { return h->d_basis + (size_t)h->nvp * 3 * syn::kBasisK; }
const float *basis_mean(const syn_handle *h) { return h->d_basis + (size_t)(h->nvp + h->nlp) * 3 * syn::kBasisK; }
const float *basis_std(const syn_handle *h) { return basis_mean(h) + 64; }
const float *basis_mean_cs(const syn_handle *h) { return basis_mean(h) + 128; }
const float *basis_std_cs(const syn_handle *h) { return basis_mean(h) + 192; }
const unsigned *basis_f16_dense(const syn_handle *h) { return reinterpret_cast<const unsigned *>(basis_mean(h) + 256); }
const unsigned *basis_f16_lmk(const syn_handle *h) { return basis_f16_dense(h) + (size_t)(h->nvp / 32) * 3 * syn::kBasisF16; }

size_t ws_floats_per_face() {
    const size_t mb = 2 * net().max_io + 2 * net().max_hidden, rn = 4 * resnet50().buf_big + 2 * resnet50().buf_mid;
    return mb > rn ? mb : rn;
}
size_t backbone_floats(int arch) { return arch == 1 ? resnet50().packed_count : net().packed_count; }

int ensure_ws(syn_handle *h, int B) {
    const size_t need = ((size_t)B * ws_floats_per_face() + 1024) * sizeof(float);
    if (need <= h->ws_bytes) return SYN_OK;
    if (h->ws) { HIP_TRY(hipDeviceSynchronize()); HIP_TRY(hipFree(h->ws)); h->ws = nullptr; h->ws_bytes = 0; }
    HIP_TRY(hipMalloc((void **)&h->ws, need));
    h->ws_bytes = need;
    return SYN_OK;
}
int ensure_rec(syn_handle *h, int B) {
    const size_t need = ((size_t)B * syn::kRecFloatsPerFace + syn::kRecSlack) * sizeof(float);
    if (need <= h->rec_bytes) return SYN_OK;
    if (h->rec) { HIP_TRY(hipDeviceSynchronize()); HIP_TRY(hipFree(h->rec)); h->rec = nullptr; h->rec_bytes = 0; }
    HIP_TRY(hipMalloc((void **)&h->rec, need));
    h->rec_bytes = need;
    return SYN_OK;
}

void pack_basis_tiles(float *dst, int n_rows_valid, int n_tiles, const float *w_shp, const float *w_exp, const float *u,
                      const int64_t *rows ) {
    auto wfull = [&](int v, int c, int k) -> float {
        if (v >= n_rows_valid) return 0.f;
        const size_t row = rows ? (size_t)rows[3 * v + c] : (size_t)3 * v + c;
        if (k < 40) return w_shp[row * 40 + k];
        if (k < 50) return w_exp[row * 10 + (k - 40)];
        if (k == 50) return u[row];
        return 0.f;
    };
    for (int t = 0; t < n_tiles; ++t)
        for (int c = 0; c < 3; ++c) {
            float *d = dst + ((size_t)t * 3 + c) * (syn::kBasisK * 32);
            for (int chunk = 0; chunk < 6; ++chunk)
                for (int lane = 0; lane < 64; ++lane)
                    for (int s = 0; s < 4; ++s)
                        d[chunk * 256 + lane * 4 + s] = wfull(32 * t + (lane & 31), c, 8 * chunk + 4 * (lane >> 5) + s);
            for (int lane = 0; lane < 64; ++lane)
                for (int s = 0; s < 2; ++s)
                    d[6 * 256 + lane * 2 + s] = wfull(32 * t + (lane & 31), c, 48 + 2 * (lane >> 5) + s);
        }
}

static unsigned f16_rtz(float x) {
    unsigned u; memcpy(&u, &x, 4);
    const unsigned sgn = (u >> 16) & 0x8000u;
    const int e = (int)((u >> 23) & 0xff) - 127 + 15;
    unsigned m = u & 0x7fffffu;
    if (((u >> 23) & 0xff) == 0) return sgn;
    if (e >= 31) return sgn | 0x7bffu;
    if (e <= 0) return e < -10 ? sgn : sgn | ((m | 0x800000u) >> (14 - e));
    return sgn | ((unsigned)e << 10) | (m >> 13);
}
static float f16_value(unsigned h) {
    const int e = (h >> 10) & 31, m = h & 1023;
    const float v = e ? ldexpf(1.0f + m / 1024.0f, e - 15) : ldexpf((float)m, -24);
    return (h & 0x8000u) ? -v : v;
}

static float pow2_scale(float mx) {
    int ex = 0;
    if (mx > 0.f && std::isfinite(mx)) { (void)frexpf(mx, &ex); ex = 14 - ex; }
    ex = ex < -100 ? -100 : (ex > 100 ? 100 : ex);
    return ldexpf(1.0f, ex);
}

void pack_basis_tiles_f16(unsigned *dst, int n_rows_valid, int n_tiles, const float *w_shp, const float *w_exp, const float *u,
                         const int64_t *rows, const float *colscale ) {
    auto wfull = [&](int v, int c, int k) -> float {
        if (v >= n_rows_valid) return 0.f;
        const size_t row = rows ? (size_t)rows[3 * v + c] : (size_t)3 * v + c;
        if (k < 40) return w_shp[row * 40 + k] * colscale[k];
        if (k < 50) return w_exp[row * 10 + (k - 40)] * colscale[k];
        return u[row] * colscale[50];
    };
    auto split = [](float x, unsigned (&pc)[2]) {
        pc[0] = f16_rtz(x);
        pc[1] = f16_rtz(x - f16_value(pc[0]));
    };
    for (int t = 0; t < n_tiles; ++t)
        for (int c = 0; c < 3; ++c) {
            unsigned *d = dst + ((size_t)t * 3 + c) * syn::kBasisF16;
            for (int ks = 0; ks < 3; ++ks)
                for (int lane = 0; lane < 64; ++lane)
                    for (int dd = 0; dd < 4; ++dd) {
                        unsigned lo[2], hi[2];
                        const int k0 = 16 * ks + 8 * (lane >> 5) + 2 * dd;
                        split(wfull(32 * t + (lane & 31), c, k0), lo);
                        split(wfull(32 * t + (lane & 31), c, k0 + 1), hi);
                        for (int pc = 0; pc < 2; ++pc) d[((ks * 2 + pc) * 64 + lane) * 4 + dd] = lo[pc] | (hi[pc] << 16);
                    }
            for (int lane = 0; lane < 64; ++lane) {
                unsigned b8[2], b9[2], uu[2];
                split(wfull(32 * t + (lane & 31), c, 48), b8);
                split(wfull(32 * t + (lane & 31), c, 49), b9);
                split(wfull(32 * t + (lane & 31), c, 50), uu);
                unsigned *x = d + (6 * 64 + lane) * 4;
                if ((lane >> 5) == 0) {
                    x[0] = b8[0] | (b8[0] << 16); x[1] = b8[1] | (b9[0] << 16); x[2] = b9[0] | (b9[1] << 16); x[3] = uu[0] | (uu[1] << 16);
                } else {
                    x[0] = x[1] = x[2] = x[3] = 0u;
                }
            }
        }
}

int run_backbone(syn_handle *h, const float *img, const uint8_t *img8, int B, float *param, float *pool, hipStream_t s,
                 int stop_feature = -1, float *feature_out = nullptr, int prof_feature = -1,
                 unsigned long long *prof = nullptr, std::vector<hipEvent_t> *marks = nullptr,
                 std::vector<int> *mark_feature = nullptr) {
    const Net &n = net();
    int rc = ensure_ws(h, B);
    if (rc) return rc;
    float *X = h->ws;
    float *Y = X + (size_t)B * n.max_io;
    float *H1 = Y + (size_t)B * n.max_io;
    float *H2 = H1 + (size_t)B * n.max_hidden;
    const float *P = h->d_backbone;
    const size_t nl = n.layers.size();
    const unsigned u1 = h->range_guard ? h->ri.unsafe1 : 0u, u16 = h->range_guard ? (h->ri.unsafe16 | h->ri.unsafe1) : 0u;
    auto any_unsafe16 = [&](int first, int last) { for (int f = first; f <= last; ++f) if ((u16 >> f) & 1u) return true; return false; };
    syn::HeadSliced head_sliced{nullptr, 0, nullptr, nullptr};
    bool have_head_sliced = false;
    auto mark = [&](int feature) {
        if (!marks) return;
        hipEvent_t e;
        if (hipEventCreate(&e) != hipSuccess) return;
        (void)hipEventRecord(e, s);
        marks->push_back(e);
        mark_feature->push_back(feature);
    };
    mark(-1);
    for (size_t li = 0; li < nl; ++li) {
        const Layer &L = n.layers[li];
        const float *w = P + L.dst_w, *sc = P + L.dst_scale, *sh = P + L.dst_shift;
        if (h->fusion && L.kind == STEM && stop_feature != 0) {
            const Layer &D = n.layers[li + 1], &Pj = n.layers[li + 2];
            const float *set32 = P + L.dst_wrm + syn::rm_stem_set_dwords();
            if (h->fusion >= 2 && (h->early_rm & 8) && !(u1 & 1u) &&
                (img8 ? syn::launch_stem_rm(img8, reinterpret_cast<const unsigned *>(P + L.dst_wrm), P + L.dst_wrm + 3 * 2 * 256, P + D.dst_wpk, P + D.dst_shift,
                                            reinterpret_cast<const unsigned *>(P + Pj.dst_wrm), P + Pj.dst_shift, P + Pj.dst_scl, X, B, s)
                      : syn::launch_stem_rm_f32(img, reinterpret_cast<const unsigned *>(set32), set32 + 3 * 2 * 256, P + D.dst_wpk, P + D.dst_shift,
                                                reinterpret_cast<const unsigned *>(P + Pj.dst_wrm), P + Pj.dst_shift, P + Pj.dst_scl, X, B, s))) {
                li += 2;
                mark(1);
                if (stop_feature == 1) {
                    HIP_TRY(hipMemcpyAsync(feature_out, X, (size_t)B * Pj.cout * Pj.hout * Pj.hout * sizeof(float), hipMemcpyDeviceToDevice, s));
                    return SYN_OK;
                }
                continue;
            }
            syn::launch_stem_block1(img, img8, P + L.dst_wpk, h->fusion >= 2 ? reinterpret_cast<const unsigned *>(P + L.dst_wb3) : nullptr, sc, sh, P + D.dst_wpk, P + D.dst_scale, P + D.dst_shift,
                                    P + Pj.dst_wpk, P + Pj.dst_scale, P + Pj.dst_shift, X, B, s);
            li += 2;
            mark(1);
            if (stop_feature == 1) {
                HIP_TRY(hipMemcpyAsync(feature_out, X, (size_t)B * Pj.cout * Pj.hout * Pj.hout * sizeof(float), hipMemcpyDeviceToDevice, s));
                return SYN_OK;
            }
            continue;
        }
        const int chain_mode = (h->fusion >= 2 && L.kind == PW && L.relu6 && (L.feature == 7 || L.feature == 8) && (h->early_rm & 128) && (h->early_rm & 512) &&
                                prof_feature < 0) ? syn::lb_chain_mode(B, (h->early_rm & 1024) != 0) : 0;
        const int chain_first = chain_mode == 3 ? 7 : 8, chain_last = chain_mode == 1 ? 13 : 14, chain_n = chain_last - chain_first + 1;
        if (chain_mode && L.feature == chain_first && !any_unsafe16(chain_first, chain_last) && (stop_feature < 0 || stop_feature >= chain_last) && li + 3 * chain_n <= nl &&
            n.max_hidden >= 2048 + 2 * (size_t)64 * 96 + 16 * 160 + 64 * 64) {
            syn::FusedBlockArgs ca[8];
            float *const Ha = H1 + (size_t)B * 2048, *const Hb = Ha + (size_t)B * 64 * 96, *const Hc = Hb + (size_t)B * 64 * 96,
                  *const Hd = Hc + (size_t)B * 16 * 160;
            float *const bin7[8] = {X, Y, Hd, Y, Hd, Ha, Hb, Ha}, *const bout7[8] = {Y, Hd, Y, Hd, Ha, Hb, Ha, Hc};
            float *const bin8[7] = {X, Y, X, Y, Ha, Hb, Ha}, *const bout8[7] = {Y, X, Y, Ha, Hb, Ha, Hc};
            float *const *bin = chain_first == 7 ? bin7 : bin8, *const *bout = chain_first == 7 ? bout7 : bout8;
            bool ok = true;
            for (int i = 0; i < chain_n && ok; ++i) {
                const Layer &E = n.layers[li + 3 * i], &Dw = n.layers[li + 3 * i + 1], &Pr = n.layers[li + 3 * i + 2];
                ok = E.kind == PW && E.relu6 && E.feature == chain_first + i && E.dst_weh && E.dst_tlb && Pr.dst_wlb;
                if (!ok) break;
                ca[i] = syn::FusedBlockArgs{bin[i], P + E.dst_wpk, P + E.dst_scale, P + E.dst_shift, P + Dw.dst_wpk, P + Dw.dst_scale, P + Dw.dst_shift,
                                            P + Pr.dst_wpk, P + Pr.dst_scale, P + Pr.dst_shift, bout[i]};
                ca[i].Alb_e = reinterpret_cast<const unsigned *>(P + E.dst_weh);
                ca[i].Alb_p = reinterpret_cast<const unsigned *>(P + Pr.dst_wlb);
                ca[i].Tlb = P + E.dst_tlb;
            }
            if (ok && syn::launch_fused_chain_lb(ca, chain_first, chain_n, B, s)) {
                li += 3 * chain_n - 1;
                X = bout[chain_n - 1];
                mark(100 * chain_first + chain_last);
                if (stop_feature == chain_last) {
                    const Layer &Lp = n.layers[li];
                    HIP_TRY(hipMemcpyAsync(feature_out, X, (size_t)B * Lp.cout * Lp.hout * Lp.hout * sizeof(float), hipMemcpyDeviceToDevice, s));
                    return SYN_OK;
                }
                continue;
// ... 17 lines not shown
                mark(1517);
                if (stop_feature == 17) {
                    const Layer &Lp = n.layers[li];
                    HIP_TRY(hipMemcpyAsync(feature_out, X, (size_t)B * Lp.cout * Lp.hout * Lp.hout * sizeof(float), hipMemcpyDeviceToDevice, s));
                    return SYN_OK;
                }
                continue;
            }
        }
        if (h->fusion && L.kind == PW && L.relu6 && L.feature >= 2 && L.feature <= 17) {
            auto block_args = [&](int l0, float *xin, float *yout) {
                const Layer &E = n.layers[l0], &D = n.layers[l0 + 1], &Pj = n.layers[l0 + 2];
                syn::FusedBlockArgs a{xin, P + E.dst_wpk, P + E.dst_scale, P + E.dst_shift, P + D.dst_wpk, P + D.dst_scale, P + D.dst_shift,
                                      P + Pj.dst_wpk, P + Pj.dst_scale, P + Pj.dst_shift, yout};
                if (prof_feature == E.feature) a.prof = prof;
                const bool ok1 = !((u1 >> E.feature) & 1u), ok16 = !((u16 >> E.feature) & 1u);
                if (h->fusion >= 2 && ok1 && E.dst_wb3 && Pj.dst_wb3) {
                    a.We3 = reinterpret_cast<const unsigned *>(P + E.dst_wb3);
                    a.Wp3 = reinterpret_cast<const unsigned *>(P + Pj.dst_wb3);
                }
                if (h->fusion >= 2 && E.dst_scl && Pj.dst_scl) { a.scl_e = P + E.dst_scl; a.scl_p = P + Pj.dst_scl; }
                if (h->fusion >= 2 && ok1 && E.dst_wrm && Pj.dst_wrm && ((h->early_rm >> (E.feature <= 4 ? E.feature - 2 : E.feature)) & 1)) {
                    a.Arm_e = reinterpret_cast<const unsigned *>(P + E.dst_wrm);
                    a.Arm_p = reinterpret_cast<const unsigned *>(P + Pj.dst_wrm);
                }
                if (h->fusion >= 2 && ok16 && a.We3 && Pj.dst_wlb && E.dst_tlb && (h->early_rm & 128)) {
                    a.Alb_p = reinterpret_cast<const unsigned *>(P + Pj.dst_wlb);
                    a.Alb_e = reinterpret_cast<const unsigned *>(P + E.dst_weh);
                    a.Tlb = P + E.dst_tlb;
                }
                if (h->fusion >= 2 && ok16 && E.dst_glb && (h->early_rm & 256)) a.Glb = reinterpret_cast<const unsigned *>(P + E.dst_glb);
                a.scratch = H2; a.scratch_floats = (size_t)B * n.max_hidden;
                return a;
            };
            syn::FusedBlockArgs a = block_args(li, X, Y);
            if ((L.feature == 3 || L.feature == 5) && (a.Arm_e || (L.feature == 5 && a.We3)) && prof_feature < 0 && (stop_feature < 0 || stop_feature >= L.feature + 1) && li + 6 <= nl &&
                n.layers[li + 3].kind == PW && n.layers[li + 3].relu6 && n.layers[li + 3].feature == L.feature + 1) {
                const Layer &Pb = n.layers[li + 5];
                const size_t in_a = (size_t)L.cin * L.hin * L.hin, out_b = (size_t)Pb.cout * Pb.hout * Pb.hout;
                float *const out2 = (L.feature == 3 && in_a + out_b <= n.max_io) ? X + (size_t)B * in_a : (L.feature == 5 ? X : nullptr);
                const syn::FusedBlockArgs b = block_args(li + 3, Y, out2);
                if (out2 && ((a.Arm_e && b.Arm_e && syn::launch_fused_pair_rm(L.feature, a, b, B, s)) ||
                             (L.feature == 5 && a.We3 && b.We3 && B < 513 && syn::launch_fused_pair_f16(a, b, B, s)))) {
                    X = out2;
                    li += 5;
                    mark(100 * L.feature + L.feature + 1);
                    if (stop_feature == L.feature + 1) {
                        const Layer &Lp = n.layers[li];
                        HIP_TRY(hipMemcpyAsync(feature_out, X, (size_t)B * Lp.cout * Lp.hout * Lp.hout * sizeof(float), hipMemcpyDeviceToDevice, s));
                        return SYN_OK;
                    }
                    continue;
                }
            }
            if (L.feature == 17 && a.Glb && stop_feature < 0 && prof_feature < 0 && !((u1 >> 18) & 1u) && syn::launch_lb4_sliced17_deferred(a, B, s, &head_sliced)) {
                have_head_sliced = true;
                float *t = X; X = Y; Y = t;
                li += 2;
                mark(L.feature);
                continue;
            }
            if ((a.Arm_e && syn::launch_fused_block_rm(L.feature, a, B, s)) ||
                (a.Alb_p && syn::launch_fused_block_lb(L.feature, a, B, s)) ||
                (a.Glb && syn::launch_fused_block_lb4(L.feature, a, B, s)) ||
                (a.We3 && (syn::launch_fused_block_early(L.feature, a, B, s) || syn::launch_fused_block_f16(L.feature, a, B, s))) ||
                syn::launch_fused_block(L.feature, a, B, s)) {
                float *t = X; X = Y; Y = t;
                li += 2;
                mark(L.feature);
                const Layer &Lp = n.layers[li];
                if (stop_feature >= 0 && Lp.feature == stop_feature) {
                    HIP_TRY(hipMemcpyAsync(feature_out, X, (size_t)B * Lp.cout * Lp.hout * Lp.hout * sizeof(float), hipMemcpyDeviceToDevice, s));
                    return SYN_OK;
                }
                continue;
            }
        }
        if (L.kind == STEM) {
            syn::launch_stem(img, img8, w, sc, sh, X, B, s);
        } else if (L.kind == DW) {
            const bool has_expand = li > 0 && n.layers[li - 1].kind == PW && n.layers[li - 1].feature == L.feature;
            syn::launch_depthwise(has_expand ? H1 : X, w, sc, sh, H2, B, L.hin, L.hout, L.cout, L.stride, s);
        } else if (L.feature == 18 && h->fusion >= 2 && !((u1 >> 18) & 1u) && stop_feature != 18) {
            syn::launch_head_f16x2(X, reinterpret_cast<const unsigned *>(P + n.dst_head_f16), sh, P + n.dst_fc_w, P + n.dst_fc_b,
                                    param, pool, H1, B, s, have_head_sliced ? &head_sliced : nullptr);
            mark(19);
            HIP_TRY(hipGetLastError());
            return SYN_OK;
        } else if (L.feature == 18 && h->fusion && stop_feature != 18) {
            syn::launch_head(X, P + L.dst_wpk, sc, sh, P + n.dst_fc_w, P + n.dst_fc_b, param, pool, B, s);
            mark(19);
            HIP_TRY(hipGetLastError());
            return SYN_OK;
        } else if (L.feature == 18) {
            syn::launch_pointwise(X, w, sc, sh, nullptr, H1, B * L.hout * L.hout, L.cin, L.kpad, L.cout, 1, s);
        } else if (L.relu6) {
            syn::launch_pointwise(X, w, sc, sh, nullptr, H1, B * L.hout * L.hout, L.cin, L.kpad, L.cout, 1, s);
        } else {
            syn::launch_pointwise(H2, w, sc, sh, L.residual ? X : nullptr, Y, B * L.hout * L.hout, L.cin, L.kpad, L.cout, 0, s);
            float *t = X; X = Y; Y = t;
        }
        mark(L.feature);
        if (stop_feature >= 0 && L.feature == stop_feature && (li + 1 == nl || n.layers[li + 1].feature != L.feature)) {
            const float *src = L.feature == 18 ? H1 : X;
            HIP_TRY(hipMemcpyAsync(feature_out, src, (size_t)B * L.cout * L.hout * L.hout * sizeof(float), hipMemcpyDeviceToDevice, s));
            return SYN_OK;
        }
    }
    syn::launch_pool_fc(H1, P + n.dst_fc_w, P + n.dst_fc_b, param, pool, B, s);
    mark(19);
    HIP_TRY(hipGetLastError());
    return SYN_OK;
}

constexpr int kResnetStat = 54;
bool resnet_stat_used(int slot) {
    const ResNet50 &n = resnet50();
    if (slot == 0) return true;
    const int ci = slot - 1;
    if (ci <= 0 || ci >= (int)n.convs.size()) return false;
    for (const RBlock &b : n.blocks) if (b.ds == ci) return false;
    return ci != n.blocks.back().c3;
}
constexpr size_t kRangeFloats = (size_t)64 * syn::kRangeSub * syn::kRangeStride;
float *range_slot(float *base, int t) { return base + (size_t)t * syn::kRangeSub * syn::kRangeStride; }
int ensure_range(syn_handle *h) {
    if (h->d_range) return SYN_OK;
    if (!h->guard_word) {
        HIP_TRY(hipHostMalloc((void **)&h->guard_word, 64, hipHostMallocMapped));
        h->guard_word[0] = 0;
        HIP_TRY(hipHostGetDevicePointer((void **)&h->guard_word_dev, h->guard_word, 0));
    }
    HIP_TRY(hipMalloc((void **)&h->d_range, 2 * kRangeFloats * sizeof(float)));
    std::vector<float> init(kRangeFloats, 0.f);
    for (int t = 0; t < 64; ++t)
        if (!(t < kResnetStat && resnet_stat_used(t)))
            for (int i = 0; i < syn::kRangeSub; ++i) init[((size_t)t * syn::kRangeSub + i) * syn::kRangeStride] = 1.0f;
    HIP_TRY(hipMemcpy(h->d_range + kRangeFloats, init.data(), kRangeFloats * sizeof(float), hipMemcpyHostToDevice));
    HIP_TRY(hipMemcpy(h->d_range, init.data(), kRangeFloats * sizeof(float), hipMemcpyHostToDevice));
    return SYN_OK;
}

int run_resnet50(syn_handle *h, const float *img, const uint8_t *img8, int B, float *param, float *pool, hipStream_t s,
                 int n_out = 62) {
    const ResNet50 &n = resnet50();
    int rc = ensure_ws(h, B);
    if (rc) return rc;
    float *A = h->ws, *X = A + (size_t)B * n.buf_big, *Y = X + (size_t)B * n.buf_big, *D = Y + (size_t)B * n.buf_big;
    float *T1 = D + (size_t)B * n.buf_big, *T2 = T1 + (size_t)B * n.buf_mid;
    const float *P = h->d_backbone;
    if (h->guard_word && *(volatile unsigned *)h->guard_word != 0 && h->range_guard) {
        *(volatile unsigned *)h->guard_word = 0;
        if (!h->resnet_fp32) { h->resnet_fp32 = 1; h->range_events += 1; }
    }
    const bool f16 = h->fusion >= 2 && !h->resnet_fp32;
    const bool guard = f16 && h->range_guard;
    h->guard_armed = guard;
    float *stat = nullptr;
    if (guard) {
        rc = ensure_range(h);
        if (rc) return rc;
        stat = h->d_range;
        HIP_TRY(hipMemcpyAsync(stat, stat + kRangeFloats, kRangeFloats * sizeof(float), hipMemcpyDeviceToDevice, s));
    }
    const int PF = f16 ? 1 : 0;
    static const unsigned long long force_exact = (unsigned long long)syn::test_knob("resnet_exact_mask", 0);
    auto unsafe_w = [&](int ci) { return ((force_exact >> ci) & 1ull) || (h->range_guard && ((h->resnet_w_unsafe[ci >> 5] >> (ci & 31)) & 1u)); };
    auto conv = [&](int ci, const float *in, const float *res, float *out, int act, int out_pair, int res_pair) {
// ... 1142 lines not shown

size_t syn_constants_bytes(syn_handle *h) {
    if (!h) return 0;
    return sizeof(ConstHeader) + ((h->d_backbone ? backbone_floats(h->arch) : 0) + (h->d_basis ? h->basis_floats : 0)) * sizeof(float);
}

static ConstHeader make_const_header(syn_handle *h) {
    ConstHeader hd{};
    hd.magic = kMagic; hd.version = kConstVersion;
    hd.has_backbone = h->d_backbone ? 1 : 0; hd.has_basis = h->d_basis ? 1 : 0;
    hd.n_vert = h->n_vert; hd.n_lmk = h->n_lmk; hd.nvp = h->nvp; hd.nlp = h->nlp;
    hd.arch = h->arch;
    hd.backbone_floats = hd.has_backbone ? backbone_floats(h->arch) : 0;
    hd.basis_floats = hd.has_basis ? h->basis_floats : 0;
    hd.total_bytes = syn_constants_bytes(h);
    return hd;
}

int syn_describe_constants(syn_handle *h, void *host_header, size_t bytes) {
    if (!h || !host_header) return fail(SYN_ERR_INVALID, "syn_describe_constants: NULL argument");
    if (bytes < sizeof(ConstHeader)) return fail(SYN_ERR_INVALID, "syn_describe_constants: %zu bytes is smaller than the header (%zu)", bytes, sizeof(ConstHeader));
    const ConstHeader hd = make_const_header(h);
    memcpy(host_header, &hd, sizeof hd);
    return SYN_OK;
}

int syn_export_constants(syn_handle *h, void *dev_dst, size_t bytes, void *stream) {
    if (!h || !dev_dst) return fail(SYN_ERR_INVALID, "syn_export_constants: NULL argument");
    const size_t need = syn_constants_bytes(h);
    if (bytes < need) return fail(SYN_ERR_INVALID, "syn_export_constants: buffer %zu < %zu bytes", bytes, need);
    ConstHeader hd = make_const_header(h);
    DeviceGuard g(h->device);
    hipStream_t s = (hipStream_t)stream;
    char *d = (char *)dev_dst;
    HIP_TRY(hipMemcpyAsync(d, &hd, sizeof hd, hipMemcpyHostToDevice, s));
    HIP_TRY(hipStreamSynchronize(s));
    d += sizeof hd;
    if (hd.has_backbone) {
        HIP_TRY(hipMemcpyAsync(d, h->d_backbone, hd.backbone_floats * sizeof(float), hipMemcpyDeviceToDevice, s));
        d += hd.backbone_floats * sizeof(float);
    }
    if (hd.has_basis) HIP_TRY(hipMemcpyAsync(d, h->d_basis, hd.basis_floats * sizeof(float), hipMemcpyDeviceToDevice, s));
    return SYN_OK;
}

int syn_import_constants(syn_handle *h, const void *dev_src, size_t bytes, void *stream) {
    if (!h || !dev_src) return fail(SYN_ERR_INVALID, "syn_import_constants: NULL argument");
    if (bytes < sizeof(ConstHeader)) return fail(SYN_ERR_INVALID, "syn_import_constants: %zu bytes is smaller than the header", bytes);
    DeviceGuard g(h->device);
    hipStream_t s = (hipStream_t)stream;
    ConstHeader hd{};
    HIP_TRY(hipMemcpyAsync(&hd, dev_src, sizeof hd, hipMemcpyDeviceToHost, s));
    HIP_TRY(hipStreamSynchronize(s));
    if (int rc = check_const_header(hd, bytes, "syn_import_constants")) return rc;
    const char *d = (const char *)dev_src + sizeof hd;
    if (hd.has_backbone) {
        if (h->d_backbone && h->arch != (int)hd.arch) { HIP_TRY(hipFree(h->d_backbone)); h->d_backbone = nullptr; }
        h->arch = (int)hd.arch;
        if (!h->d_backbone) HIP_TRY(hipMalloc((void **)&h->d_backbone, hd.backbone_floats * sizeof(float)));
        HIP_TRY(hipMemcpyAsync(h->d_backbone, d, hd.backbone_floats * sizeof(float), hipMemcpyDeviceToDevice, s));
        h->ri = RangeInfo{};
        h->resnet_fp32 = 0; h->range_events = 0; h->guard_armed = 0; if (h->guard_word) { (void)hipDeviceSynchronize(); *(volatile unsigned *)h->guard_word = 0; }
        h->resnet_w_unsafe[0] = h->resnet_w_unsafe[1] = h->resnet_w_unsafe[2] = 0;
        if (h->arch == 0) {
            HIP_TRY(hipMemcpyAsync(&h->ri, d + net().dst_range * sizeof(float), sizeof h->ri, hipMemcpyDeviceToHost, s));
            HIP_TRY(hipStreamSynchronize(s));
        } else {
            HIP_TRY(hipMemcpyAsync(h->resnet_w_unsafe, d + resnet50().dst_range * sizeof(float), sizeof h->resnet_w_unsafe, hipMemcpyDeviceToHost, s));
            HIP_TRY(hipStreamSynchronize(s));
        }
        d += hd.backbone_floats * sizeof(float);
    }
    if (hd.has_basis) {
        if (h->d_basis && h->basis_floats != hd.basis_floats) { HIP_TRY(hipFree(h->d_basis)); h->d_basis = nullptr; }
        if (!h->d_basis) HIP_TRY(hipMalloc((void **)&h->d_basis, hd.basis_floats * sizeof(float)));
        HIP_TRY(hipMemcpyAsync(h->d_basis, d, hd.basis_floats * sizeof(float), hipMemcpyDeviceToDevice, s));
        h->basis_floats = hd.basis_floats; h->n_vert = hd.n_vert; h->n_lmk = hd.n_lmk; h->nvp = hd.nvp; h->nlp = hd.nlp;
    }
    return SYN_OK;
}

size_t syn_workspace_bytes(syn_handle *, int B) {
    if (B <= 0) return 0;
    return ((size_t)B * (ws_floats_per_face() + syn::kRecFloatsPerFace) + 1024 + syn::kRecSlack) * sizeof(float);
}

int syn_backbone_forward(syn_handle *h, const float *img, int B, float *param, float *pool, void *stream) {
    if (!h || !img || !param) return fail(SYN_ERR_INVALID, "syn_backbone_forward: NULL argument");
    if (B <= 0) return fail(SYN_ERR_INVALID, "syn_backbone_forward: B=%d", B);
    if (!h->d_backbone) return fail(SYN_ERR_NOT_LOADED, "syn_backbone_forward: backbone weights not loaded");
    DeviceGuard g(h->device);
    if (h->arch == 1) return run_resnet50(h, img, nullptr, B, param, pool, (hipStream_t)stream);
    return run_backbone(h, img, nullptr, B, param, pool, (hipStream_t)stream);
}

int syn_backbone_forward_u8(syn_handle *h, const uint8_t *img, int B, float *param, float *pool, void *stream) {
    if (!h || !img || !param) return fail(SYN_ERR_INVALID, "syn_backbone_forward_u8: NULL argument");
    if (B <= 0) return fail(SYN_ERR_INVALID, "syn_backbone_forward_u8: B=%d", B);
    if (!h->d_backbone) return fail(SYN_ERR_NOT_LOADED, "syn_backbone_forward_u8: backbone weights not loaded");
    DeviceGuard g(h->device);
    if (h->arch == 1) return run_resnet50(h, nullptr, img, B, param, pool, (hipStream_t)stream);
    return run_backbone(h, nullptr, img, B, param, pool, (hipStream_t)stream);
}

int syn_backbone_profile(syn_handle *h, const uint8_t *img_hwc, int B, int max_launches, int *feature_of_launch,
                         float *ms_of_launch, double *flops_of_launch) {
    if (!h || !img_hwc || B <= 0 || !feature_of_launch || !ms_of_launch || !flops_of_launch)
        return fail(SYN_ERR_INVALID, "syn_backbone_profile: bad argument");
    if (!h->d_backbone) return fail(SYN_ERR_NOT_LOADED, "syn_backbone_profile: backbone weights not loaded");
    DeviceGuard g(h->device);
    float *param = nullptr;
    HIP_TRY(hipMalloc((void **)&param, (size_t)B * 62 * sizeof(float)));
    std::vector<hipEvent_t> marks;
    std::vector<int> feats;
    int rc = run_backbone(h, nullptr, img_hwc, B, param, nullptr, nullptr, -1, nullptr, -1, nullptr, &marks, &feats);
    int count = 0;
    if (rc == SYN_OK) {
        HIP_TRY(hipDeviceSynchronize());
        const Net &n = net();
        for (size_t i = 1; i < marks.size() && count < max_launches; ++i, ++count) {
            float ms = 0.f;
            (void)hipEventElapsedTime(&ms, marks[i - 1], marks[i]);
            feature_of_launch[count] = feats[i];
            ms_of_launch[count] = ms;
            double fl = 0;
            if (feats[i] == 19) {
                fl = 2.0 * 1280 * 62 + 16.0 * 1280;
                bool has18 = false;
                for (size_t j = 1; j < feats.size(); ++j) has18 |= feats[j] == 18;
                if (!has18) fl += 2.0 * 320 * 1280 * 16;
            }
            else if (feats[i] >= 100) {
                for (const Layer &L : n.layers)
                    if (L.feature >= feats[i] / 100 && L.feature <= feats[i] % 100)
                        fl += 2.0 * (L.kind == DW ? 9.0 * L.cout : (double)L.cin * L.cout) * L.hout * L.hout;
            }
            else if (i == 1 && feats[i] == 1) { for (const Layer &L : n.layers) if (L.feature <= 1) fl += 2.0 * (L.kind == STEM ? 27.0 * 32 : L.kind == DW ? 9.0 * L.cout : (double)L.cin * L.cout) * L.hout * L.hout; }
            else {
                int same = 0;
                for (size_t j = 1; j < feats.size(); ++j) same += feats[j] == feats[i];
                int seen = 0;
                for (size_t j = 1; j <= i; ++j) seen += feats[j] == feats[i];
                int idx = 0;
                for (const Layer &L : n.layers) {
                    if (L.feature != feats[i]) continue;
                    ++idx;
                    if (same > 1 && idx != seen) continue;
                    fl += 2.0 * (L.kind == STEM ? 27.0 * 32 : L.kind == DW ? 9.0 * L.cout : (double)L.cin * L.cout) * L.hout * L.hout;
                }
            }
            flops_of_launch[count] = fl * B;
        }
    }
    for (hipEvent_t e : marks) (void)hipEventDestroy(e);
    (void)hipFree(param);
    return rc == SYN_OK ? count : rc;
}

int syn_debug_profile_block(syn_handle *h, const float *img, int B, int feature, unsigned long long *out8) {
    if (!h || !img || !out8 || B <= 0) return fail(SYN_ERR_INVALID, "syn_debug_profile_block: bad argument");
    if (!h->d_backbone) return fail(SYN_ERR_NOT_LOADED, "syn_debug_profile_block: backbone weights not loaded");
    DeviceGuard g(h->device);
    unsigned long long *d = nullptr;
    HIP_TRY(hipMalloc((void **)&d, 32 * sizeof(unsigned long long)));
    HIP_TRY(hipMemset(d, 0, 32 * sizeof(unsigned long long)));
    float *param = nullptr;
    HIP_TRY(hipMalloc((void **)&param, (size_t)B * 62 * sizeof(float)));
    int rc = run_backbone(h, img, nullptr, B, param, nullptr, nullptr, -1, nullptr, feature, d);
    if (rc == SYN_OK) {
        HIP_TRY(hipDeviceSynchronize());
        HIP_TRY(hipMemcpy(out8, d, 32 * sizeof(unsigned long long), hipMemcpyDeviceToHost));
    }
    (void)hipFree(d);
    (void)hipFree(param);
    return rc;
}

int syn_debug_feature(syn_handle *h, const float *img, int B, int feature, float *out, void *stream) {
    if (!h || !img || !out || B <= 0 || feature < 0 || feature > 18) return fail(SYN_ERR_INVALID, "syn_debug_feature: bad argument");
    if (!h->d_backbone) return fail(SYN_ERR_NOT_LOADED, "syn_debug_feature: backbone weights not loaded");
    DeviceGuard g(h->device);
    return run_backbone(h, img, nullptr, B, nullptr, nullptr, (hipStream_t)stream, feature, out);
}

int syn_backbone_calibrate(syn_handle *h, const uint8_t *crops_u8, int B, float tol, void *stream) {
    if (!h || !crops_u8) return fail(SYN_ERR_INVALID, "syn_backbone_calibrate: NULL argument");
    if (B <= 0 || B > 256) return fail(SYN_ERR_INVALID, "syn_backbone_calibrate: B=%d (1 .. 256 crops)", B);
    if (!(tol > 0.f)) return fail(SYN_ERR_INVALID, "syn_backbone_calibrate: tol=%g", (double)tol);
    if (!h->d_backbone) return fail(SYN_ERR_NOT_LOADED, "syn_backbone_calibrate: backbone weights not loaded");
    if (h->arch != 0) return 0;
    DeviceGuard g(h->device);
    hipStream_t s = (hipStream_t)stream;
    const Net &n = net();
    const size_t cap = (size_t)B * 60 * 60 * 16;
    float *d_a = nullptr, *d_b = nullptr;
    HIP_TRY(hipMalloc((void **)&d_a, 2 * cap * sizeof(float)));
    d_b = d_a + cap;
    std::vector<float> ha(cap), hb(cap);
    const int fusion0 = h->fusion;
    int switched = 0, rc = SYN_OK;
    for (int f = 1; f <= 17 && rc == SYN_OK; ++f) {
        size_t count = 0;
        for (const Layer &L : n.layers) if (L.feature == f) count = (size_t)B * L.cout * L.hout * L.hout;
        const unsigned bit = f == 1 ? 1u : 1u << f;
        if ((h->ri.unsafe1 & bit) || count == 0 || count > cap) continue;
        h->fusion = 2;
        rc = run_backbone(h, nullptr, crops_u8, B, nullptr, nullptr, s, f, d_a);
        h->fusion = 1;
        if (rc == SYN_OK) rc = run_backbone(h, nullptr, crops_u8, B, nullptr, nullptr, s, f, d_b);
        h->fusion = fusion0;
        if (rc != SYN_OK) break;
        if (hipMemcpyAsync(ha.data(), d_a, count * sizeof(float), hipMemcpyDeviceToHost, s) != hipSuccess ||
            hipMemcpyAsync(hb.data(), d_b, count * sizeof(float), hipMemcpyDeviceToHost, s) != hipSuccess || hipStreamSynchronize(s) != hipSuccess) {
            rc = fail(SYN_ERR_HIP, "syn_backbone_calibrate: reading features.%d back failed", f);
            break;
        }
        double worst = 0, mag = 0;
        bool finite = true;
        for (size_t i = 0; i < count; ++i) {
            finite = finite && std::isfinite(ha[i]) && std::isfinite(hb[i]);
            const double d = fabs((double)ha[i] - (double)hb[i]);
            worst = d > worst ? d : worst;
            mag = fabs((double)hb[i]) > mag ? fabs((double)hb[i]) : mag;
        }
        if (!finite || worst > (double)tol * (mag > 0 ? mag : 1.0)) {
            h->ri.unsafe1 |= bit; h->ri.unsafe16 |= bit;
            ++switched;
        }
    }
    (void)hipFree(d_a);
    if (rc != SYN_OK) return rc;
    if (switched) HIP_TRY(hipMemcpy(h->d_backbone + n.dst_range, &h->ri, sizeof h->ri, hipMemcpyHostToDevice));
    return switched;
}

int syn_debug_poison_workspace(syn_handle *h, int B, int byte) {
    if (!h || B <= 0) return fail(SYN_ERR_INVALID, "syn_debug_poison_workspace: bad argument");
    DeviceGuard g(h->device);
    int rc = ensure_ws(h, B);
    if (rc) return rc;
    rc = ensure_rec(h, B);
    if (rc) return rc;
    HIP_TRY(hipDeviceSynchronize());
    HIP_TRY(hipMemset(h->ws, byte, h->ws_bytes));
    HIP_TRY(hipMemset(h->rec, byte, h->rec_bytes));
    if (h->rws) HIP_TRY(hipMemset(h->rws, byte, h->rws_bytes));
    if (h->dws) HIP_TRY(hipMemset(h->dws, byte, h->dws_bytes));
    HIP_TRY(hipDeviceSynchronize());
    return SYN_OK;
}

int syn_crop_resize(syn_handle *h, const uint8_t *frame, int H, int W, const int *box, const int *xofs, const int16_t *xcoef,
                    const int *yofs, const int16_t *ycoef, uint8_t *out, int B, void *stream) {
    if (!h || !frame || !box || !xofs || !xcoef || !yofs || !ycoef || !out) return fail(SYN_ERR_INVALID, "syn_crop_resize: NULL argument");
    if (B <= 0 || H <= 0 || W <= 0) return fail(SYN_ERR_INVALID, "syn_crop_resize: B=%d H=%d W=%d", B, H, W);
    DeviceGuard g(h->device);
    syn::launch_crop_resize(frame, H, W, box, xofs, xcoef, yofs, ycoef, out, B, (hipStream_t)stream);
    HIP_TRY(hipGetLastError());
    return SYN_OK;
}

int syn_crop_resize_frames(syn_handle *h, const uint8_t *frames, const long long *frame_off, const int *frame_dim, const int *face_frame,
                           const int *box, const int *xofs, const int16_t *xcoef, const int *yofs, const int16_t *ycoef, uint8_t *out, int B,
                           void *stream) {
    if (!h || !frames || !frame_off || !frame_dim || !face_frame || !box || !xofs || !xcoef || !yofs || !ycoef || !out)
        return fail(SYN_ERR_INVALID, "syn_crop_resize_frames: NULL argument");
    if (B <= 0) return fail(SYN_ERR_INVALID, "syn_crop_resize_frames: B=%d", B);
    DeviceGuard g(h->device);
    syn::launch_crop_resize(frames, 0, 0, box, xofs, xcoef, yofs, ycoef, out, B, (hipStream_t)stream, frame_off, frame_dim, face_frame);
    HIP_TRY(hipGetLastError());
    return SYN_OK;
}

int syn_reconstruct_pitched(syn_handle *h, const float *param, int B, int param_len, int dense, int transform, const float *roi,
                            float *out, int row_pitch, int pad_writable, void *stream) {
    if (!h || !param || !out) return fail(SYN_ERR_INVALID, "syn_reconstruct: NULL argument");
    if (param_len != SYN_PARAM_DIM) return fail(SYN_ERR_PARAM_LEN, "length of params mismatch");
    if (B <= 0) return fail(SYN_ERR_INVALID, "syn_reconstruct: B=%d", B);
    if (!h->d_basis) return fail(SYN_ERR_NOT_LOADED, "syn_reconstruct: 3DMM basis not loaded");
    const int n = dense ? h->n_vert : h->n_lmk;
    if (row_pitch < n) return fail(SYN_ERR_INVALID, "syn_reconstruct: row_pitch=%d < %d columns", row_pitch, n);
    DeviceGuard g(h->device);
    int rc = ensure_rec(h, B);
    if (rc) return rc;
    float *rec = h->rec;
    hipStream_t s = (hipStream_t)stream;
    if (h->fusion >= 2)
        syn::launch_reconstruct_f16(param, basis_mean_cs(h), basis_std_cs(h), dense ? basis_f16_dense(h) : basis_f16_lmk(h), n, dense ? h->nvp : h->nlp,
                                   roi, transform, out, row_pitch, pad_writable, B, s, rec);
    else
        syn::launch_reconstruct(param, basis_mean(h), basis_std(h), dense ? basis_dense(h) : basis_lmk(h), n, dense ? h->nvp : h->nlp,
                                roi, transform, out, row_pitch, B, s, rec);
    HIP_TRY(hipGetLastError());
    return SYN_OK;
}

int syn_reconstruct_profile(syn_handle *h, const float *param, int B, const float *roi, float *out, int row_pitch, int pad_writable, float *ms2) {
    if (!h || !param || !out || !ms2) return fail(SYN_ERR_INVALID, "syn_reconstruct_profile: NULL argument");
    if (B <= 0 || !h->d_basis || row_pitch < h->n_vert) return fail(SYN_ERR_INVALID, "syn_reconstruct_profile: bad argument");
    if (h->fusion < 2) return fail(SYN_ERR_INVALID, "syn_reconstruct_profile: the fp16x2 schedule only");
    DeviceGuard g(h->device);
    int rc = ensure_rec(h, B);
    if (rc) return rc;
    hipEvent_t ev[3];
    for (auto &e : ev) HIP_TRY(hipEventCreate(&e));
    syn::launch_reconstruct_f16(param, basis_mean_cs(h), basis_std_cs(h), basis_f16_dense(h), h->n_vert, h->nvp, roi, 1, out, row_pitch, pad_writable, B,
                                nullptr, h->rec, ev);
    hipError_t e = hipDeviceSynchronize();
    if (e == hipSuccess) { (void)hipEventElapsedTime(&ms2[0], ev[0], ev[1]); (void)hipEventElapsedTime(&ms2[1], ev[1], ev[2]); }
    for (auto &x : ev) (void)hipEventDestroy(x);
    if (e != hipSuccess) return fail(SYN_ERR_HIP, "syn_reconstruct_profile: %s", hipGetErrorString(e));
    return SYN_OK;
}

int syn_reconstruct(syn_handle *h, const float *param, int B, int param_len, int dense, int transform, const float *roi,
                    float *out, void *stream) {
    if (!h) return fail(SYN_ERR_INVALID, "syn_reconstruct: NULL argument");
    return syn_reconstruct_pitched(h, param, B, param_len, dense, transform, roi, out, dense ? h->n_vert : h->n_lmk, 0, stream);
}

namespace {
int ensure_rws(syn_handle *h, size_t bytes) {
    if (bytes <= h->rws_bytes) return SYN_OK;
    if (h->rws) { HIP_TRY(hipDeviceSynchronize()); HIP_TRY(hipFree(h->rws)); h->rws = nullptr; h->rws_bytes = 0; }
    HIP_TRY(hipMalloc(&h->rws, bytes));
    h->rws_bytes = bytes;
    return SYN_OK;
}
size_t align256(size_t x) { return (x + 255) & ~(size_t)255; }
}

namespace {
int upload_topology(syn_handle *h, const int32_t *tri, int ntri, int nver, int **d_tri, int **d_adj_off, int **d_adj_tri) {
    std::vector<int> off(nver + 1, 0), adj(3 * (size_t)ntri);
    for (int i = 0; i < 3 * ntri; ++i) off[tri[i] + 1]++;
    for (int v = 0; v < nver; ++v) off[v + 1] += off[v];
    std::vector<int> cur(off.begin(), off.end() - 1);
    for (int t = 0; t < ntri; ++t)
        for (int j = 0; j < 3; ++j) adj[cur[tri[3 * t + j]]++] = t;
    if (*d_tri) { HIP_TRY(hipDeviceSynchronize()); (void)hipFree(*d_tri); (void)hipFree(*d_adj_off); (void)hipFree(*d_adj_tri); *d_tri = *d_adj_off = *d_adj_tri = nullptr; }
    HIP_TRY(hipMalloc((void **)d_tri, sizeof(int) * 3 * (size_t)ntri));
    HIP_TRY(hipMalloc((void **)d_adj_off, sizeof(int) * (nver + 1)));
    HIP_TRY(hipMalloc((void **)d_adj_tri, sizeof(int) * 3 * (size_t)ntri));
    HIP_TRY(hipMemcpy(*d_tri, tri, sizeof(int) * 3 * (size_t)ntri, hipMemcpyHostToDevice));
    HIP_TRY(hipMemcpy(*d_adj_off, off.data(), sizeof(int) * (nver + 1), hipMemcpyHostToDevice));
    HIP_TRY(hipMemcpy(*d_adj_tri, adj.data(), sizeof(int) * 3 * (size_t)ntri, hipMemcpyHostToDevice));
    return SYN_OK;
}
struct Topo { const int *tri, *adj_off, *adj_tri; int ntri, nver; };
int drop_tex_coords(syn_handle *h, int slot) {
    if (h->d_texc[slot]) { HIP_TRY(hipDeviceSynchronize()); (void)hipFree(h->d_texc[slot]); h->d_texc[slot] = nullptr; }
    h->texc_nver[slot] = h->texc_own_tri[slot] = 0;
    return SYN_OK;
}
Topo current_topo(const syn_handle *h) {
    if (h->topo_slot == 1) return Topo{h->k_tri, h->k_adj_off, h->k_adj_tri, h->k_ntri, h->n_keep};
    return Topo{h->d_tri, h->d_adj_off, h->d_adj_tri, h->ntri, h->tri_nver};
}
}

int syn_load_triangles(syn_handle *h, const int32_t *tri, int ntri, int nver) {
    if (!h || !tri || ntri <= 0 || nver <= 0) return fail(SYN_ERR_INVALID, "syn_load_triangles: bad argument");
    if (ntri >= (1 << 24)) return fail(SYN_ERR_INVALID, "syn_load_triangles: ntri=%d exceeds the 24-bit z-key field", ntri);
    for (int i = 0; i < 3 * ntri; ++i)
        if (tri[i] < 0 || tri[i] >= nver) return fail(SYN_ERR_INVALID, "syn_load_triangles: tri[%d]=%d out of range", i, tri[i]);
    DeviceGuard g(h->device);
    int rc = drop_tex_coords(h, 0);
    if (rc) return rc;
    rc = upload_topology(h, tri, ntri, nver, &h->d_tri, &h->d_adj_off, &h->d_adj_tri);
    if (rc) { h->ntri = h->tri_nver = 0; return rc; }
    h->ntri = ntri; h->tri_nver = nver;
    h->tri_max[0] = *std::max_element(tri, tri + 3 * (size_t)ntri);
// ... 719 lines not shown
```

synergynet_amd/streams.py:

```python
from __future__ import annotations

import torch


_REC_STREAMS = {}


def reconstruction_stream(dev, priority=-1):
    key = (torch.device(dev).index, priority)
    if key not in _REC_STREAMS:
        _REC_STREAMS[key] = torch.cuda.Stream(device=dev, priority=priority)
    return _REC_STREAMS[key]


class OverlappedPipeline:
    def __init__(self, model, overlap=True, rec_priority=-1):
        self.model = model
        self.dev = model.device
        self.s_main = torch.cuda.current_stream(self.dev)
        self.s_rec = reconstruction_stream(self.dev, rec_priority) if overlap else self.s_main
        self._inflight = [None, None]
        self._n = 0
        self._tail_stream = None
        self.last_done = None

    def submit(self, crops_u8, rois, lmk_out=None, mesh_out=None, dense=True):
        m, k = self.model, self._n & 1
        self._n += 1
        if self._inflight[k] is not None:
            self.s_main.wait_event(self._inflight[k][1])
        with torch.cuda.stream(self.s_main):
            param = m.forward_crops_u8(crops_u8)
            ready = torch.cuda.Event()
            ready.record(self.s_main)
        s_tail = self.s_rec if dense else self.s_main
        with torch.cuda.stream(s_tail):
            s_tail.wait_event(ready)
            if self._tail_stream is not s_tail and self.last_done is not None:
                s_tail.wait_event(self.last_done)
            self._tail_stream = s_tail
            lmk, pose = m.landmarks_and_pose(param, roi=rois, out=lmk_out)
            mesh = m.reconstruct(param, roi=rois, dense=True, out=mesh_out) if dense else None
            done = torch.cuda.Event()
            done.record(s_tail)
        self._inflight[k] = ((param, lmk, mesh, pose, crops_u8, rois), done)
        self.last_done = done
        return param, lmk, mesh, pose

    def wait(self):
        for slot in self._inflight:
            if slot is not None:
                slot[1].synchronize()


class ReplicaRing:

    def __init__(self, make_model=None, n=4, models=None):
        self.models = list(models) if models is not None else [make_model() for _ in range(n)]
        dev = self.models[0].device
        self.streams = [torch.cuda.Stream(device=dev) for _ in self.models]
        self._k = 0

    def submit(self, crops_u8, rois, dense=False, lmk_out=None, mesh_out=None):
        i = self._k % len(self.models)
        self._k += 1
        m, st = self.models[i], self.streams[i]
        st.wait_stream(torch.cuda.current_stream(m.device))
        with torch.cuda.stream(st):
            param = m.forward_crops_u8(crops_u8)
            lmk, pose = m.landmarks_and_pose(param, roi=rois, out=lmk_out)
            mesh = m.reconstruct(param, roi=rois, dense=True, out=mesh_out) if dense else None
            done = torch.cuda.Event()
            done.record(st)
        for t in (crops_u8, rois):
            if isinstance(t, torch.Tensor) and t.is_cuda:
                t.record_stream(st)
        return param, lmk, mesh, pose, done

    def wait(self):
        for st in self.streams:
            st.synchronize()
```

synergynet_amd/synergy3DMM.py:

```python
from __future__ import annotations

import ctypes as C
import os
import warnings

import numpy as np
import torch
import torch.nn as nn

from . import abi
from .params import ParamsPack
from .synth import HEADS, RESNET_HEADS, mbv2_layers, resnet50_convs

BACKBONE_PREFIX = 'I2P.backbone.'
_BASIS_BUFFERS = ('param_mean', 'param_std', 'w_shp', 'u', 'w_exp', 'u_base', 'w_shp_base', 'w_exp_base')


def parse_param_62(param):
    p_ = param[:, :12].reshape(-1, 3, 4)
    p = p_[:, :, :3]
    offset = p_[:, :, -1].reshape(-1, 3, 1)
    alpha_shp = param[:, 12:52].reshape(-1, 40, 1)
    alpha_exp = param[:, 52:62].reshape(-1, 10, 1)
    return p, offset, alpha_shp, alpha_exp
# ... 296 lines not shown
            self.load_synergy_state(syn_sd)

    def load_synergy_state(self, sd, prefix=''):
        from .synth import flatten_synergy
        flat = flatten_synergy({k: (v.detach().cpu().numpy() if isinstance(v, torch.Tensor) else v) for k, v in sd.items()}, prefix)
        assert flat.size == self._lib.syn_synergy_flat_count()
        abi.check(self._lib.syn_load_synergy(self._h, flat.ctypes.data_as(C.c_void_p), flat.size))
        self.has_synergy = True

    def constants_nbytes(self) -> int:
        return int(self._lib.syn_constants_bytes(self._h))

    def export_constants(self) -> torch.Tensor:
        n = self.constants_nbytes()
        buf = torch.empty(n, dtype=torch.uint8, device=self.device)
        abi.check(self._lib.syn_export_constants(self._h, buf.data_ptr(), n, self._stream()))
        return buf

    def import_constants(self, buf: torch.Tensor):
        assert buf.is_cuda and buf.dtype == torch.uint8 and buf.is_contiguous()
        hdr = parse_constants_header(buf[:256].cpu().numpy().tobytes())
        abi.check(self._lib.syn_import_constants(self._h, buf.data_ptr(), buf.numel(), self._stream()))
        torch.cuda.current_stream(self.device).synchronize()
        self._follow_constants(hdr)

    def _after_import(self):
        raw = C.create_string_buffer(256)
        abi.check(self._lib.syn_describe_constants(self._h, raw, 256))
        self._follow_constants(parse_constants_header(raw.raw))

    def _follow_constants(self, hdr):
        if hdr['has_backbone']:
            self.arch = ('mobilenet_v2', 'resnet50')[hdr['arch']]
            self._have_backbone = True
            self._range_checked = False
            self._range_events = 0
            self._warn_numerics()
        if hdr['has_basis']:
            self._n_vert, self._n_lmk = hdr['n_vert'], hdr['n_lmk']
            self._have_basis = True

    @property
    def pool_dim(self):
        return 2048 if self.arch == 'resnet50' else 1280

    def _stream(self):
        return C.c_void_p(torch.cuda.current_stream(self.device).cuda_stream)

    def _dev_f32(self, t):
        if not isinstance(t, torch.Tensor):
            t = torch.as_tensor(np.asarray(t))
        return t.to(device=self.device, dtype=torch.float32).contiguous()

    def forward_test(self, input, return_pool=False):
        was_cpu = isinstance(input, torch.Tensor) and not input.is_cuda
        x = self._dev_f32(input)
        if x.dim() != 4 or tuple(x.shape[1:]) != (3, 120, 120):
            raise RuntimeError(f'forward_test expects [B,3,120,120], got {tuple(x.shape)}')
        B = x.shape[0]
        with torch.cuda.device(self.device):
            param = torch.empty((B, 62), dtype=torch.float32, device=self.device)
            pool = torch.empty((B, self.pool_dim), dtype=torch.float32, device=self.device) if return_pool else None
            self._guarded(lambda: abi.check(self._lib.syn_backbone_forward(self._h, x.data_ptr(), B, param.data_ptr(),
                                                                          pool.data_ptr() if return_pool else None, self._stream())))
        if was_cpu:
            param = param.cpu()
            pool = pool.cpu() if return_pool else None
        return (param, pool) if return_pool else param

    def forward_crops_u8(self, crops, return_pool=False):
        if not isinstance(crops, torch.Tensor):
            crops = torch.as_tensor(np.asarray(crops))
        if crops.dtype != torch.uint8 or crops.dim() != 4 or tuple(crops.shape[1:]) != (120, 120, 3):
            raise RuntimeError('forward_crops_u8 expects uint8 [B,120,120,3]')
        x = crops.to(self.device).contiguous()
        B = x.shape[0]
        with torch.cuda.device(self.device):
            param = torch.empty((B, 62), dtype=torch.float32, device=self.device)
            pool = torch.empty((B, self.pool_dim), dtype=torch.float32, device=self.device) if return_pool else None
            self._guarded(lambda: abi.check(self._lib.syn_backbone_forward_u8(self._h, x.data_ptr(), B, param.data_ptr(),
                                                                             pool.data_ptr() if return_pool else None, self._stream())))
        return (param, pool) if return_pool else param

    def reconstruct(self, param, roi=None, dense=False, transform=True, out=None):
        p = self._dev_f32(param)
        if p.dim() != 2:
            raise RuntimeError('param must be [B,62]')
        B = p.shape[0]
        n = self._n_vert if dense else self._n_lmk
        r = None
        if roi is not None:
            r = self._dev_f32(roi)
            if tuple(r.shape) != (B, 5):
                raise RuntimeError('roi must be [B,5] (sx,sy,ex,ey,score)')
        with torch.cuda.device(self.device):
            if out is None:
                out = self.empty_vertices(B, dense)
            if tuple(out.shape) != (B, 3, n) or out.dtype != torch.float32 or out.device != self.device:
                raise RuntimeError(f'out must be a float32 [B,3,{n}] tensor on {self.device}')
            pitch = out.stride(1)
            if out.stride(2) != 1 or pitch < n or (B > 1 and out.stride(0) != 3 * pitch):
                raise RuntimeError('out must have unit column stride and equally pitched rows (a [B,3,pitch][..., :n] view)')
            try:
                abi.check(self._lib.syn_reconstruct_pitched(self._h, p.data_ptr(), B, p.shape[1], int(dense), int(transform),
                                                            r.data_ptr() if r is not None else None, out.data_ptr(), int(pitch),
                                                            int(getattr(out, '_syn_pad_writable', False)), self._stream()))
            except abi.SynergyHipError as e:
                if e.code == abi.SYN_ERR_PARAM_LEN:
                    raise RuntimeError('length of params mismatch') from None
                raise
        return out

    def empty_vertices(self, B, dense=True):
        n = self._n_vert if dense else self._n_lmk
        pitch = (n + 127) // 128 * 128 if n >= 1024 else n
        out = torch.empty((B, 3, pitch), dtype=torch.float32, device=self.device)[:, :, :n]
        out._syn_pad_writable = pitch > n
        return out

    def reconstruct_vertex_62(self, param, whitening=True, dense=False, transform=True, lmk_pts=68):
        if not whitening:
            raise UnboundLocalError("local variable 'param_' referenced before assignment")
        if not dense and lmk_pts != self._n_lmk:
            raise RuntimeError(f'lmk_pts={lmk_pts} but the landmark basis has {self._n_lmk} points')
        was_cpu = isinstance(param, torch.Tensor) and not param.is_cuda
        out = self.reconstruct(param, roi=None, dense=dense, transform=transform)
        return out.cpu() if was_cpu else out

    def predict_pose_batch(self, param, roi=None):
        p = self._dev_f32(param)
        if p.dim() != 2 or p.shape[1] != 62:
            raise RuntimeError('length of params mismatch')
        B = p.shape[0]
        r = self._dev_f32(roi) if roi is not None else None
        if r is not None and tuple(r.shape) != (B, 5):
            raise RuntimeError('roi must be [B,5] (sx,sy,ex,ey,score)')
        with torch.cuda.device(self.device):
            ang = torch.empty((B, 3), dtype=torch.float64, device=self.device)
            t3d = torch.empty((B, 3), dtype=torch.float32, device=self.device)
            abi.check(self._lib.syn_pose(self._h, p.data_ptr(), B, r.data_ptr() if r is not None else None,
                                         ang.data_ptr(), t3d.data_ptr(), self._stream()))
        return ang, t3d

    def landmarks_and_pose(self, param, roi=None, transform=True, out=None):
        p = self._dev_f32(param)
        if p.dim() != 2:
            raise RuntimeError('param must be [B,62]')
        if p.shape[1] != 62:
            raise RuntimeError('length of params mismatch')
        B, n = p.shape[0], self._n_lmk
        r = self._dev_f32(roi) if roi is not None else None
        if r is not None and tuple(r.shape) != (B, 5):
            raise RuntimeError('roi must be [B,5] (sx,sy,ex,ey,score)')
        with torch.cuda.device(self.device):
            if out is None:
                out = torch.empty((B, 3, n), dtype=torch.float32, device=self.device)
            if tuple(out.shape) != (B, 3, n) or out.dtype != torch.float32 or out.device != self.device:
                raise RuntimeError(f'out must be a float32 [B,3,{n}] tensor on {self.device}')
            if not out.is_contiguous():
                self.reconstruct(p, roi=r, dense=False, transform=transform, out=out)
                return out, self.predict_pose_batch(p, roi=r)
            ang = torch.empty((B, 3), dtype=torch.float64, device=self.device)
            t3d = torch.empty((B, 3), dtype=torch.float32, device=self.device)
            abi.check(self._lib.syn_landmarks_pose(self._h, p.data_ptr(), B, 62, int(transform), r.data_ptr() if r is not None else None,
                                                   out.data_ptr(), ang.data_ptr(), t3d.data_ptr(), self._stream()))
        return out, (ang, t3d)

    def _need_synergy(self):
        if self.arch == 'resnet50':
            raise RuntimeError('the synergy refinement needs the 1280-d pooled feature of mobilenet_v2; arch=resnet50 pools 2048')
        if not self.has_synergy:
            raise RuntimeError('synergy weights not loaded: the checkpoint carried no forwardDirection.* / reverseDirection.* keys '
                               '(load_synergy_state)')

    def _check_faces(self, name, t, shape):
        t = self._dev_f32(t)
        if t.dim() != len(shape) + 1 or tuple(t.shape[1:]) != shape:
            raise RuntimeError(f'{name} must be [B,{",".join(map(str, shape))}], got {tuple(t.shape)}')
        return t

    def refine_landmarks(self, param, pool, roi=None, transform=True, return_coarse=False):
        self._need_synergy()
        p, po = self._check_faces('param', param, (62,)), self._check_faces('pool', pool, (1280,))
        B = p.shape[0]
        if po.shape[0] != B:
            raise RuntimeError('param and pool must hold the same number of faces')
        r = self._check_faces('roi', roi, (5,)) if roi is not None else None
# ... 278 lines not shown
```

Before: 1.024 million.

## Fuse landmark, pose and recon-prep tail into the backbone head kernel

```diff
diff --git a/include/synergy_hip.h b/include/synergy_hip.h
--- a/include/synergy_hip.h
+++ b/include/synergy_hip.h
@@ -15,7 +15,8 @@
     SYN_ERR_INVALID = -1,
     SYN_ERR_HIP = -2,
     SYN_ERR_NOT_LOADED = -3,
-    SYN_ERR_PARAM_LEN = -4
+    SYN_ERR_PARAM_LEN = -4,
+    SYN_ERR_STALE_RECORDS = -5
 } syn_status;
 
 #define SYN_PARAM_DIM 62
@@ -80,6 +81,7 @@
 
 int syn_reconstruct(syn_handle *h, const float *param, int B, int param_len, int dense,
                     int transform, const float *roi, float *out, void *stream);
+#define SYN_RECON_RECORDS_CURRENT 2
 
 int syn_reconstruct_pitched(syn_handle *h, const float *param, int B, int param_len, int dense,
                             int transform, const float *roi, float *out, int row_pitch, int pad_writable, void *stream);
@@ -142,6 +144,9 @@
 int syn_landmarks_pose(syn_handle *h, const float *param, int B, int param_len, int transform, const float *roi ,
                        float *lmk, double *angles , float *t3d , void *stream);
 
+int syn_forward_tail_u8(syn_handle *h, const uint8_t *crops_hwc, int B, int transform, const float *roi , float *param,
+                        float *pool , float *lmk, double *angles, float *t3d, int *records_current , void *stream);
+
 int syn_pose_matrix(syn_handle *h, const float *param, int B, float *pmat, void *stream);
 
 size_t syn_synergy_flat_count(void);
diff --git a/synergynet_amd/abi.py b/synergynet_amd/abi.py
--- a/synergynet_amd/abi.py
+++ b/synergynet_amd/abi.py
@@ -9,6 +9,8 @@
 
 SYN_ERR_INVALID, SYN_ERR_NOT_LOADED = -1, -3
 SYN_ERR_PARAM_LEN = -4
+SYN_ERR_STALE_RECORDS = -5
+SYN_RECON_RECORDS_CURRENT = 2
 _lib = None
 
 
@@ -77,6 +79,7 @@
     'syn_reconstruct_pitched': (C.c_int, [C.c_void_p, C.c_void_p, C.c_int, C.c_int, C.c_int, C.c_int, C.c_void_p, C.c_void_p, C.c_int, C.c_int, C.c_void_p]),
     'syn_pose': (C.c_int, [C.c_void_p, C.c_void_p, C.c_int, C.c_void_p, C.c_void_p, C.c_void_p, C.c_void_p]),
     'syn_landmarks_pose': (C.c_int, [C.c_void_p, C.c_void_p, C.c_int, C.c_int, C.c_int, C.c_void_p, C.c_void_p, C.c_void_p, C.c_void_p, C.c_void_p]),
+    'syn_forward_tail_u8': (C.c_int, [C.c_void_p, C.c_void_p, C.c_int, C.c_int] + [C.c_void_p] * 6 + [C.POINTER(C.c_int), C.c_void_p]),
     'syn_pose_matrix': (C.c_int, [C.c_void_p, C.c_void_p, C.c_int, C.c_void_p, C.c_void_p]),
     'syn_synergy_flat_count': (C.c_size_t, []),
     'syn_synergy_folded_count': (C.c_size_t, []),
diff --git a/synergynet_amd/csrc/head_kernel.hip b/synergynet_amd/csrc/head_kernel.hip
--- a/synergynet_amd/csrc/head_kernel.hip
+++ b/synergynet_amd/csrc/head_kernel.hip
@@ -1,6 +1,7 @@
 #include <cstdlib>
 
 #include "syn_internal.h"
+#include "tail_face.h"
 
 namespace syn {
 
@@ -147,9 +148,9 @@
 }
 }
 
-template <int NR, int NFK = NF, int NWV = 4>
+template <int NR, int NFK = NF, int NWV = 4, bool KEEP = false>
 __device__ __forceinline__ void fc_rows(const f32x4 (&xv)[NFK][N / 256], const float *__restrict__ Wfc, const float *__restrict__ bfc,
-                                        float *__restrict__ param, int f0, int B, int rbase, int wave, int lane) {
+                                        float *__restrict__ param, int f0, int B, int rbase, int wave, int lane, float *keep = nullptr) {
     f32x4 wq[2][N / 256];
     auto ldw = [&](int o, f32x4(&w)[N / 256]) {
         const float *wr = Wfc + (size_t)(o < kParam ? o : kParam - 1) * N;
@@ -172,18 +173,56 @@
                 a += wv[i][0] * xv[j][i][0] + wv[i][1] * xv[j][i][1] + wv[i][2] * xv[j][i][2] + wv[i][3] * xv[j][i][3];
             const float tot = wave64_sum(a);
             if (lane == 0 && f0 + j < B) param[(size_t)(f0 + j) * kParam + o] = tot + bo;
+            if (KEEP && lane == 0) keep[j * 64 + o] = tot + bo;
+        }
+    }
+}
+
+template <int NFK, int NT>
+__device__ __forceinline__ void head_tail_faces(const float *raw, float *dw, const HeadTail &ht, int f0, int B, int tid) {
+    for (int it = tid; it < NFK * 64; it += NT) {
+        const int l = it & 63;
+        if (l < kParam) dw[it] = raw[it] * ht.stdv[l] + ht.mean[l];
+    }
+    __syncthreads();
+    if (tid >= NT - NFK) {
+        const int j = NT - 1 - tid, b = f0 + j;
+        if (b < B) {
+            float pp[12];
+#pragma unroll
+            for (int i = 0; i < 12; ++i) pp[i] = dw[j * 64 + i];
+            pose_of_face(pp, ht.roi ? ht.roi + (size_t)b * 5 : nullptr, ht.angles + (size_t)b * 3, ht.t3d + (size_t)b * 3, nullptr);
+        }
+    }
+    for (int it = tid; it < NFK * ht.n_lmk; it += NT) {
+        const int j = it / ht.n_lmk, v = it - j * ht.n_lmk, b = f0 + j;
+        if (b < B) {
+            float aff[12];
+            lmk_affine(dw + j * 64, ht.roi, b, ht.transform, aff);
+            lmk_of_point<true>(dw + j * 64, ht.basis_lmk, aff, v, ht.n_lmk, b, ht.lmk);
+        }
+    }
+    if (ht.rec3 && tid >= NT - 128 && tid < NT - 64) {
+        const int end = f0 + NFK < B ? f0 + NFK : (B + 31) / 32 * 32;
+        for (int q = tid - (NT - 128); q < 2 * (end - f0); q += 64) {
+            const int b = f0 + (q >> 1), hh = q & 1;
+            const bool ok = b < B;
+            recon_prep_lane(raw + (ok ? b - f0 : 0) * 64, ok, b, (b & 31) + 32 * hh, ht.mean_cs, ht.std_cs, ht.roi, ht.transform,
+                            ht.rec3 + (size_t)(b >> 5) * kRecTileF16);
         }
     }
 }
 
 constexpr int kFcRounds = (kParam + 3) / 4;
 
-template <int NS, int NFK = NF, int NWV = 4, bool SIN = false>
+template <int NS, int NFK = NF, int NWV = 4, bool SIN = false, bool TAIL = false>
 __global__ __launch_bounds__(NWV * 64) void head_f16x2_kernel(const float *__restrict__ X ,
                                                           const unsigned *__restrict__ Wb3 ,
                                                           const float *__restrict__ shift, const float *__restrict__ Wfc,
                                                           const float *__restrict__ bfc, float *__restrict__ param,
-                                                          float *__restrict__ pool, int B, HeadSliced hs = HeadSliced{nullptr, 0, nullptr, nullptr}) {
+                                                          float *__restrict__ pool, int B, HeadSliced hs = HeadSliced{nullptr, 0, nullptr, nullptr},
+                                                          HeadTail ht = HeadTail{}) {
+    static_assert(!TAIL || NS == 1, "the tail needs a workgroup that holds all 62 parameters of its faces");
     constexpr int PXK = NFK * 16, PLANEK = PXK * XSD, NT = NWV * 64;
     __shared__ __attribute__((aligned(16))) unsigned Xb[2 * PLANEK];
     __shared__ __attribute__((aligned(16))) float Ps[NFK * N];
@@ -319,6 +358,13 @@
     for (int j = 0; j < NFK; ++j)
 #pragma unroll
         for (int i = 0; i < N / 256; ++i) xv[j][i] = *(const f32x4 *)&Ps[j * N + (i * 64 + lane) * 4];
+    if constexpr (TAIL) {
+        float *const raw = reinterpret_cast<float *>(Xb), *const dw = raw + NFK * 64;
+        static_assert(2 * NFK * 64 <= 2 * PLANEK, "the parameter copies fit in the input planes");
+        fc_rows<(kParam + NWV - 1) / NWV, NFK, NWV, true>(xv, Wfc, bfc, param, f0, B, 0, wave, lane, raw);
+        __syncthreads();
+        head_tail_faces<NFK, NT>(raw, dw, ht, f0, B, tid);
+    } else
     fc_rows<(kParam + NWV - 1) / NWV, NFK, NWV>(xv, Wfc, bfc, param, f0, B, 0, wave, lane);
 }
 
@@ -337,9 +383,15 @@
     fc_rows<kFcRounds / kFcSlices>(xv, Wfc, bfc, param, f0, B, blockIdx.y * (kFcRounds / kFcSlices), wave, lane);
 }
 
+bool head_tail_supported(int B, bool sliced_in) {
+    (void)sliced_in;
+    return (B + NF - 1) / NF > 96;
+}
+
 void launch_head_f16x2(const float *X, const unsigned *Wb3, const float *shift, const float *Wfc, const float *bfc,
-                        float *param, float *pool, float *scratch, int B, hipStream_t s, const HeadSliced *sin) {
+                        float *param, float *pool, float *scratch, int B, hipStream_t s, const HeadSliced *sin, const HeadTail *tail) {
     const int grid = (B + NF - 1) / NF;
+    const HeadSliced hs0{nullptr, 0, nullptr, nullptr};
     if (grid <= 96) {
         float *pl = pool ? pool : scratch;
         if (sin) head_f16x2_kernel<5, NF, 4, true><<<dim3(grid, 5), 256, 0, s>>>(X, Wb3, shift, Wfc, bfc, param, pl, B, *sin);
@@ -348,14 +400,17 @@
         return;
     }
     if (sin) {
-        head_f16x2_kernel<1, NF, 4, true><<<grid, 256, 0, s>>>(X, Wb3, shift, Wfc, bfc, param, pool, B, *sin);
+        if (tail) head_f16x2_kernel<1, NF, 4, true, true><<<grid, 256, 0, s>>>(X, Wb3, shift, Wfc, bfc, param, pool, B, *sin, *tail);
+        else head_f16x2_kernel<1, NF, 4, true><<<grid, 256, 0, s>>>(X, Wb3, shift, Wfc, bfc, param, pool, B, *sin);
         return;
     }
     static const int wide_min = (int)test_knob("head_wide_min", 513);
     if (B >= wide_min) {
-        head_f16x2_kernel<1, 4, 8><<<(B + 3) / 4, 512, 0, s>>>(X, Wb3, shift, Wfc, bfc, param, pool, B);
+        if (tail) head_f16x2_kernel<1, 4, 8, false, true><<<(B + 3) / 4, 512, 0, s>>>(X, Wb3, shift, Wfc, bfc, param, pool, B, hs0, *tail);
+        else head_f16x2_kernel<1, 4, 8><<<(B + 3) / 4, 512, 0, s>>>(X, Wb3, shift, Wfc, bfc, param, pool, B);
         return;
     }
-    head_f16x2_kernel<1><<<grid, 256, 0, s>>>(X, Wb3, shift, Wfc, bfc, param, pool, B);
-}
-}
+    if (tail) head_f16x2_kernel<1, NF, 4, false, true><<<grid, 256, 0, s>>>(X, Wb3, shift, Wfc, bfc, param, pool, B, hs0, *tail);
+    else head_f16x2_kernel<1><<<grid, 256, 0, s>>>(X, Wb3, shift, Wfc, bfc, param, pool, B);
+}
+}
diff --git a/synergynet_amd/csrc/recon_kernels.hip b/synergynet_amd/csrc/recon_kernels.hip
--- a/synergynet_amd/csrc/recon_kernels.hip
+++ b/synergynet_amd/csrc/recon_kernels.hip
@@ -2,6 +2,7 @@
 #include <cstdlib>
 
 #include "syn_internal.h"
+#include "tail_face.h"
 
 namespace syn {
 
@@ -162,13 +163,6 @@
 typedef _Float16 f16x2r __attribute__((ext_vector_type(2)));
 
 namespace {
-__device__ __forceinline__ void split2r(float x0, float x1, unsigned &a, unsigned &b) {
-    a = __builtin_bit_cast(unsigned, __builtin_amdgcn_cvt_pkrtz(x0, x1));
-    float r0, r1;
-    asm("v_fma_mix_f32 %0, %1, -1.0, %2 op_sel_hi:[1,0,0]" : "=v"(r0) : "v"(a), "v"(x0));
-    asm("v_fma_mix_f32 %0, %1, -1.0, %2 op_sel:[1,0,0] op_sel_hi:[1,0,0]" : "=v"(r1) : "v"(a), "v"(x1));
-    b = __builtin_bit_cast(unsigned, __builtin_amdgcn_cvt_pkrtz(r0, r1));
-}
 __device__ __forceinline__ f32x16 mfma32(u32x4 a, u32x4 b, f32x16 c) {
     return __builtin_amdgcn_mfma_f32_32x32x16_f16(__builtin_bit_cast(f16x8r, a), __builtin_bit_cast(f16x8r, b), c, 0, 0, 0);
 }
@@ -177,80 +171,10 @@
 __global__ __launch_bounds__(64) void recon_prep_f16_kernel(const float *__restrict__ param, const float *__restrict__ mean,
                                                            const float *__restrict__ stdv, const float *__restrict__ roi,
                                                            int transform, unsigned *__restrict__ rec3, int B) {
-    const int ft = blockIdx.x, l = threadIdx.x, i = l & 31, hh = l >> 5;
-    const int b = ft * 32 + i;
+    const int ft = blockIdx.x, l = threadIdx.x;
+    const int b = ft * 32 + (l & 31);
     const bool ok = b < B;
-    const float *pp = param + (size_t)(ok ? b : 0) * kParam;
-    unsigned *rt = rec3 + (size_t)ft * kRecTileF16;
-    float al[3][8];
-    float amax = 0.f;
-#pragma unroll
-    for (int ks = 0; ks < 3; ++ks)
-#pragma unroll
-        for (int e = 0; e < 8; ++e) {
-            const int k = 12 + 16 * ks + 8 * hh + e;
-            al[ks][e] = ok ? pp[k] * stdv[k] + mean[k] : 0.f;
-            amax = fmaxf(amax, fabsf(al[ks][e]));
-        }
-    const float a48 = ok ? pp[12 + 48] * stdv[12 + 48] + mean[12 + 48] : 0.f;
-    const float a49 = ok ? pp[12 + 49] * stdv[12 + 49] + mean[12 + 49] : 0.f;
-    amax = fmaxf(amax, fmaxf(fabsf(a48), fabsf(a49)));
-    amax = fmaxf(amax, __shfl_xor(amax, 32));
-    const float cu = mean[62];
-    amax = fmaxf(amax, cu);
-    int ex = (int)((__builtin_bit_cast(unsigned, amax) >> 23) & 0xff) - 126;
-    ex = 14 - ex;
-    const int ex_cu = (int)((__builtin_bit_cast(unsigned, cu) >> 23) & 0xff) - 127;
-    ex = ex < -14 - ex_cu ? -14 - ex_cu : ex;
-    ex = ex < -100 ? -100 : (ex > 100 ? 100 : ex);
-    const float Sa = __builtin_bit_cast(float, (unsigned)(127 + ex) << 23);
-    const float inv_ab = __builtin_bit_cast(float, (unsigned)(127 - ex) << 23);
-#pragma unroll
-    for (int ks = 0; ks < 3; ++ks) {
-        u32x4 pc[2];
-#pragma unroll
-        for (int d = 0; d < 4; ++d) {
-            unsigned a, b2;
-            split2r(al[ks][2 * d] * Sa, al[ks][2 * d + 1] * Sa, a, b2);
-            pc[0][d] = a; pc[1][d] = b2;
-        }
-#pragma unroll
-        for (int p = 0; p < 2; ++p) *(u32x4 *)&rt[((ks * 2 + p) * 64 + l) * 4] = pc[p];
-    }
-    {
-        unsigned a, b2;
-        split2r(a48 * Sa, a49 * Sa, a, b2);
-        const unsigned a8 = a & 0xffffu, b8 = b2 & 0xffffu, a9 = a >> 16, b9 = b2 >> 16;
-        const unsigned sa16 = ok ? (__builtin_bit_cast(unsigned, __builtin_amdgcn_cvt_pkrtz(cu * Sa, cu * Sa)) & 0xffffu) : 0u;
-        u32x4 fx = {0u, 0u, 0u, 0u};
-        if (hh == 0) fx = (u32x4){a8 | (b8 << 16), a8 | (a9 << 16), b9 | (a9 << 16), sa16 | (sa16 << 16)};
-        *(u32x4 *)&rt[(6 * 64 + l) * 4] = fx;
-    }
-    if (hh == 0) {
-        float r[16];
-        float p12[12];
-#pragma unroll
-        for (int q = 0; q < 12; ++q) p12[q] = ok ? pp[q] * stdv[q] + mean[q] : 0.f;
-#pragma unroll
-        for (int c = 0; c < 3; ++c) {
-            float sc = 1.0f, of = 0.0f;
-            if (roi && ok) {
-                const float sx = roi[b * 5 + 0], sy = roi[b * 5 + 1], ex = roi[b * 5 + 2], ey = roi[b * 5 + 3];
-                const float scx = (ex - sx) / 120.0f, scy = (ey - sy) / 120.0f;
-                if (c == 0) { sc = scx; of = sx; }
-                else if (c == 1) { sc = scy; of = sy; }
-                else { sc = (scx + scy) * 0.5f; }
-            }
-            float m0 = p12[4 * c + 0], m1 = p12[4 * c + 1], m2 = p12[4 * c + 2], t = p12[4 * c + 3];
-            if (transform && c == 1) { m0 = -m0; m1 = -m1; m2 = -m2; t = (float)(kImg + 1) - t; }
-            r[3 * c + 0] = m0 * sc * inv_ab; r[3 * c + 1] = m1 * sc * inv_ab; r[3 * c + 2] = m2 * sc * inv_ab;
-            r[9 + c] = t * sc + of;
-        }
-        r[12] = 0.f; r[13] = 0.f; r[14] = 0.f; r[15] = 0.f;
-        float *rr = reinterpret_cast<float *>(rt + 7 * 256) + i * 16;
-#pragma unroll
-        for (int q = 0; q < 4; ++q) *(f32x4 *)&rr[4 * q] = (f32x4){r[4 * q], r[4 * q + 1], r[4 * q + 2], r[4 * q + 3]};
-    }
+    recon_prep_lane(param + (size_t)(ok ? b : 0) * kParam, ok, b, l, mean, stdv, roi, transform, rec3 + (size_t)ft * kRecTileF16);
 }
 
 #define RLAP(i) do { if (PROF) { asm volatile("s_waitcnt vmcnt(0) lgkmcnt(0)" ::: "memory"); tn = __builtin_amdgcn_s_memtime(); pt_[i] += tn - tk; tk = tn; } } while (0)
@@ -437,11 +361,12 @@
 
 void launch_reconstruct_f16(const float *param, const float *mean62, const float *std62, const unsigned *basis3, int n_vert,
                            int nvp, const float *roi, int transform, float *out, int pitch, int pad_writable, int B, hipStream_t s, float *rec3f,
-                           hipEvent_t *marks ) {
+                           hipEvent_t *marks ,
+                           bool records_current ) {
     unsigned *rec3 = reinterpret_cast<unsigned *>(rec3f);
     const int n_ftiles = (B + 31) / 32;
     if (marks) (void)hipEventRecord(marks[0], s);
-    recon_prep_f16_kernel<<<n_ftiles, 64, 0, s>>>(param, mean62, std62, roi, transform, rec3, B);
+    if (!records_current) recon_prep_f16_kernel<<<n_ftiles, 64, 0, s>>>(param, mean62, std62, roi, transform, rec3, B);
     if (marks) (void)hipEventRecord(marks[1], s);
     const int n_tiles = nvp / 32;
     constexpr int WPG = 4;
@@ -492,46 +417,6 @@
     if (marks) (void)hipEventRecord(marks[2], s);
 }
 
-__device__ __forceinline__ void pose_of_face(const float (&p)[12], const float *__restrict__ roi5 , double *__restrict__ angles3 ,
-                                             float *__restrict__ t3d3, float *__restrict__ pmat12 ) {
-    const float n1 = sqrtf(p[0] * p[0] + p[1] * p[1] + p[2] * p[2]);
-    const float n2 = sqrtf(p[4] * p[4] + p[5] * p[5] + p[6] * p[6]);
-    const float r1[3] = {p[0] / n1, p[1] / n1, p[2] / n1};
-    const float r2[3] = {p[4] / n2, p[5] / n2, p[6] / n2};
-    const float r3[3] = {r1[1] * r2[2] - r1[2] * r2[1], r1[2] * r2[0] - r1[0] * r2[2], r1[0] * r2[1] - r1[1] * r2[0]};
-    const double PI = 3.14159265358979323846;
-    double x, y, z;
-    if (r3[0] != 1.0f && r3[0] != -1.0f) {
-        x = asin((double)r3[0]);
-        const double cx = cos(x);
-        y = atan2((double)r2[2] / cx, (double)r3[2] / cx);
-        z = atan2((double)r1[1] / cx, (double)r1[0] / cx);
-    } else {
-        z = 0.0;
-        if (r3[0] == -1.0f) { x = PI / 2; y = z + atan2((double)r1[1], (double)r1[2]); }
-        else                { x = -PI / 2; y = -z + atan2(-(double)r1[1], -(double)r1[2]); }
-    }
-    if (pmat12) {
-        float *m = pmat12;
-        m[0] = r1[0]; m[1] = r1[1]; m[2] = r1[2]; m[3] = p[3];
-        m[4] = r2[0]; m[5] = r2[1]; m[6] = r2[2]; m[7] = p[7];
-        m[8] = r3[0]; m[9] = r3[1]; m[10] = r3[2]; m[11] = p[11];
-    }
-    if (!angles3) return;
-    angles3[0] = x * 180.0 / PI;
-    angles3[1] = y * 180.0 / PI;
-    angles3[2] = z * 180.0 / PI;
-    float tx = p[3], ty = p[7], tz = p[11];
-    if (roi5) {
-        const float sx = roi5[0], sy = roi5[1], ex = roi5[2], ey = roi5[3];
-        tx = tx * ((ex - sx) / 120.0f) + sx;
-        ty = ty * ((ey - sy) / 120.0f) + sy;
-    }
-    t3d3[0] = tx;
-    t3d3[1] = ty;
-    t3d3[2] = tz;
-}
-
 __global__ __launch_bounds__(64) void pose_kernel(const float *__restrict__ param, const float *__restrict__ mean,
                                                   const float *__restrict__ stdv, const float *__restrict__ roi,
                                                   double *__restrict__ angles, float *__restrict__ t3d,
@@ -564,48 +449,8 @@
         pose_of_face(pp, roi ? roi + (size_t)b * 5 : nullptr, angles + (size_t)b * 3, t3d + (size_t)b * 3, nullptr);
     }
     float aff[12];
-#pragma unroll
-    for (int c = 0; c < 3; ++c) {
-        float sc = 1.0f, of = 0.0f;
-        if (roi) {
-            const float sx = roi[b * 5 + 0], sy = roi[b * 5 + 1], ex = roi[b * 5 + 2], ey = roi[b * 5 + 3];
-            const float scx = (ex - sx) / 120.0f, scy = (ey - sy) / 120.0f;
-            if (c == 0) { sc = scx; of = sx; }
-            else if (c == 1) { sc = scy; of = sy; }
-            else { sc = (scx + scy) * 0.5f; }
-        }
-        float m0 = p[4 * c + 0], m1 = p[4 * c + 1], m2 = p[4 * c + 2], t = p[4 * c + 3];
-        if (transform && c == 1) { m0 = -m0; m1 = -m1; m2 = -m2; t = (float)(kImg + 1) - t; }
-        aff[3 * c + 0] = m0 * sc;
-        aff[3 * c + 1] = m1 * sc;
-        aff[3 * c + 2] = m2 * sc;
-        aff[9 + c] = t * sc + of;
-    }
-    for (int v = l; v < n_lmk; v += 256) {
-        const int T = v >> 5, j = v & 31;
-        float S[3];
-#pragma unroll
-        for (int c = 0; c < 3; ++c) {
-            const float *bc = basis + ((size_t)T * 3 + c) * (kBasisK * 32);
-            float acc = 0.f;
-#pragma unroll
-            for (int t = 0; t < 6; ++t)
-#pragma unroll
-                for (int h = 0; h < 2; ++h) {
-                    const f32x4 w = *(const f32x4 *)(bc + t * 256 + (32 * h + j) * 4);
-#pragma unroll
-                    for (int s = 0; s < 4; ++s) acc = __builtin_fmaf(w[s], p[12 + 8 * t + 4 * h + s], acc);
-                }
-            const f32x2 w0 = *(const f32x2 *)(bc + 6 * 256 + j * 2), w1 = *(const f32x2 *)(bc + 6 * 256 + (32 + j) * 2);
-            acc = __builtin_fmaf(w0[0], p[12 + 48], acc);
-            acc = __builtin_fmaf(w0[1], p[12 + 49], acc);
-            acc += w1[0];
-            S[c] = acc;
-        }
-#pragma unroll
-        for (int c = 0; c < 3; ++c)
-            lmk[((size_t)b * 3 + c) * n_lmk + v] = aff[3 * c + 0] * S[0] + aff[3 * c + 1] * S[1] + aff[3 * c + 2] * S[2] + aff[9 + c];
-    }
+    lmk_affine(p, roi, b, transform, aff);
+    for (int v = l; v < n_lmk; v += 256) lmk_of_point(p, basis, aff, v, n_lmk, b, lmk);
 }
 
 void launch_lmk_pose(const float *param, const float *mean62, const float *std62, const float *basis_lmk, int n_lmk, int nlp, const float *roi,
diff --git a/synergynet_amd/csrc/syn_internal.h b/synergynet_amd/csrc/syn_internal.h
--- a/synergynet_amd/csrc/syn_internal.h
+++ b/synergynet_amd/csrc/syn_internal.h
@@ -96,9 +96,21 @@
     const float *inv_p;
     const float *p_shift;
 };
+struct HeadTail {
+    const float *mean, *stdv;
+    const float *mean_cs, *std_cs;
+    const float *basis_lmk;
+    const float *roi;
+    float *lmk;
+    double *angles;
+    float *t3d;
+    unsigned *rec3;
+    int n_lmk, transform;
+};
+bool head_tail_supported(int B, bool sliced_in);
 void launch_head_f16x2(const float *X, const unsigned *Wb3 , const float *shift, const float *Wfc,
                         const float *bfc, float *param, float *pool, float *scratch , int B, hipStream_t s,
-                       const HeadSliced *sliced_in = nullptr);
+                       const HeadSliced *sliced_in = nullptr, const HeadTail *tail = nullptr);
 bool launch_lb4_sliced17_deferred(const FusedBlockArgs &a, int B, hipStream_t s, HeadSliced *out);
 
 void launch_crop_resize(const uint8_t *frame, int H, int W, const int *box, const int *xofs, const short *xcoef,
@@ -152,7 +164,7 @@
 constexpr int kRecSlack = 4096;
 void launch_reconstruct_f16(const float *param, const float *mean62, const float *std62, const unsigned *basis3, int n_vert,
                            int nvp, const float *roi, int transform, float *out, int pitch, int pad_writable, int B, hipStream_t s, float *rec3,
-                           hipEvent_t *marks = nullptr);
+                           hipEvent_t *marks = nullptr, bool records_current = false);
 
 void launch_mesh_normals(const float *vertices, const int *tri, const int *adj_off, const int *adj_tri, float *tri_normal,
                          float *normal , unsigned *mm , int F, int nver,
diff --git a/synergynet_amd/csrc/synergy_abi.hip b/synergynet_amd/csrc/synergy_abi.hip
--- a/synergynet_amd/csrc/synergy_abi.hip
+++ b/synergynet_amd/csrc/synergy_abi.hip
@@ -302,6 +302,9 @@
     size_t ws_bytes = 0;
     float *rec = nullptr;
     size_t rec_bytes = 0;
+    size_t rec_region_floats = 0;
+    int tail_slot = 0;
+    struct { const float *param = nullptr, *roi = nullptr; int B = 0, transform = 0, slot = 0; } rec_cur;
     int *d_tri = nullptr, *d_adj_off = nullptr, *d_adj_tri = nullptr;
     int ntri = 0, tri_nver = 0;
     int *d_uv = nullptr;
@@ -365,13 +368,16 @@
     return SYN_OK;
 }
 int ensure_rec(syn_handle *h, int B) {
-    const size_t need = ((size_t)B * syn::kRecFloatsPerFace + syn::kRecSlack) * sizeof(float);
+    const size_t region = (size_t)B * syn::kRecFloatsPerFace + syn::kRecSlack, need = 3 * region * sizeof(float);
     if (need <= h->rec_bytes) return SYN_OK;
     if (h->rec) { HIP_TRY(hipDeviceSynchronize()); HIP_TRY(hipFree(h->rec)); h->rec = nullptr; h->rec_bytes = 0; }
+    h->rec_cur.param = nullptr;
     HIP_TRY(hipMalloc((void **)&h->rec, need));
     h->rec_bytes = need;
-    return SYN_OK;
-}
+    h->rec_region_floats = region;
+    return SYN_OK;
+}
+float *rec_region(const syn_handle *h, int i) { return h->rec + (size_t)i * h->rec_region_floats; }
 
 void pack_basis_tiles(float *dst, int n_rows_valid, int n_tiles, const float *w_shp, const float *w_exp, const float *u,
                       const int64_t *rows ) {
@@ -462,7 +468,8 @@
 int run_backbone(syn_handle *h, const float *img, const uint8_t *img8, int B, float *param, float *pool, hipStream_t s,
                  int stop_feature = -1, float *feature_out = nullptr, int prof_feature = -1,
                  unsigned long long *prof = nullptr, std::vector<hipEvent_t> *marks = nullptr,
-                 std::vector<int> *mark_feature = nullptr) {
+                 std::vector<int> *mark_feature = nullptr, const syn::HeadTail *tail = nullptr ,
+                 bool *tail_done = nullptr ) {
     const Net &n = net();
     int rc = ensure_ws(h, B);
     if (rc) return rc;
@@ -646,8 +653,10 @@
             const bool has_expand = li > 0 && n.layers[li - 1].kind == PW && n.layers[li - 1].feature == L.feature;
             syn::launch_depthwise(has_expand ? H1 : X, w, sc, sh, H2, B, L.hin, L.hout, L.cout, L.stride, s);
         } else if (L.feature == 18 && h->fusion >= 2 && !((u1 >> 18) & 1u) && stop_feature != 18) {
+            const bool fold = tail && syn::head_tail_supported(B, have_head_sliced);
             syn::launch_head_f16x2(X, reinterpret_cast<const unsigned *>(P + n.dst_head_f16), sh, P + n.dst_fc_w, P + n.dst_fc_b,
-                                    param, pool, H1, B, s, have_head_sliced ? &head_sliced : nullptr);
+                                    param, pool, H1, B, s, have_head_sliced ? &head_sliced : nullptr, fold ? tail : nullptr);
+            if (fold) *tail_done = true;
             mark(19);
             HIP_TRY(hipGetLastError());
             return SYN_OK;
@@ -1956,7 +1965,7 @@
 
 size_t syn_workspace_bytes(syn_handle *, int B) {
     if (B <= 0) return 0;
-    return ((size_t)B * (ws_floats_per_face() + syn::kRecFloatsPerFace) + 1024 + syn::kRecSlack) * sizeof(float);
+    return ((size_t)B * (ws_floats_per_face() + 3 * syn::kRecFloatsPerFace) + 1024 + 3 * syn::kRecSlack) * sizeof(float);
 }
 
 int syn_backbone_forward(syn_handle *h, const float *img, int B, float *param, float *pool, void *stream) {
@@ -1975,6 +1984,48 @@
     DeviceGuard g(h->device);
     if (h->arch == 1) return run_resnet50(h, nullptr, img, B, param, pool, (hipStream_t)stream);
     return run_backbone(h, nullptr, img, B, param, pool, (hipStream_t)stream);
+}
+
+int syn_forward_tail_u8(syn_handle *h, const uint8_t *img, int B, int transform, const float *roi, float *param, float *pool, float *lmk,
+                        double *angles, float *t3d, int *records_current, void *stream) {
+    if (!h || !img || !param || !lmk || !angles || !t3d) return fail(SYN_ERR_INVALID, "syn_forward_tail_u8: NULL argument");
+    if (B <= 0) return fail(SYN_ERR_INVALID, "syn_forward_tail_u8: B=%d", B);
+    if (!h->d_backbone) return fail(SYN_ERR_NOT_LOADED, "syn_forward_tail_u8: backbone weights not loaded");
+    if (!h->d_basis) return fail(SYN_ERR_NOT_LOADED, "syn_forward_tail_u8: 3DMM basis not loaded");
+    DeviceGuard g(h->device);
+    hipStream_t s = (hipStream_t)stream;
+    if (records_current) *records_current = 0;
+    static const bool knob_fold = syn::test_knob("head_tail", 1) != 0;
+    bool folded = false;
+    int rc;
+    if (h->arch == 1) {
+        rc = run_resnet50(h, nullptr, img, B, param, pool, s);
+    } else {
+        syn::HeadTail t{};
+        const bool want_rec = records_current && h->fusion >= 2;
+        if (knob_fold && want_rec) {
+            rc = ensure_rec(h, B);
+            if (rc) return rc;
+        }
+        if (knob_fold) {
+            t.mean = basis_mean(h); t.stdv = basis_std(h); t.mean_cs = basis_mean_cs(h); t.std_cs = basis_std_cs(h);
+            t.basis_lmk = basis_lmk(h); t.roi = roi; t.lmk = lmk; t.angles = angles; t.t3d = t3d;
+            t.rec3 = want_rec ? reinterpret_cast<unsigned *>(rec_region(h, 1 + (h->tail_slot ^ 1))) : nullptr;
+            t.n_lmk = h->n_lmk; t.transform = transform;
+        }
+        rc = run_backbone(h, nullptr, img, B, param, pool, s, -1, nullptr, -1, nullptr, nullptr, nullptr, knob_fold ? &t : nullptr, &folded);
+        if (rc == SYN_OK && folded && want_rec) {
+            h->tail_slot ^= 1;
+            h->rec_cur.param = param; h->rec_cur.roi = roi; h->rec_cur.B = B; h->rec_cur.transform = transform != 0; h->rec_cur.slot = 1 + h->tail_slot;
+            *records_current = 1;
+        }
+    }
+    if (rc) return rc;
+    if (!folded) {
+        syn::launch_lmk_pose(param, basis_mean(h), basis_std(h), basis_lmk(h), h->n_lmk, h->nlp, roi, transform, lmk, angles, t3d, B, s);
+        HIP_TRY(hipGetLastError());
+    }
+    return SYN_OK;
 }
 
 int syn_backbone_profile(syn_handle *h, const uint8_t *img_hwc, int B, int max_launches, int *feature_of_launch,
@@ -2118,6 +2169,7 @@
     HIP_TRY(hipDeviceSynchronize());
     HIP_TRY(hipMemset(h->ws, byte, h->ws_bytes));
     HIP_TRY(hipMemset(h->rec, byte, h->rec_bytes));
+    h->rec_cur.param = nullptr;
     if (h->rws) HIP_TRY(hipMemset(h->rws, byte, h->rws_bytes));
     if (h->dws) HIP_TRY(hipMemset(h->dws, byte, h->dws_bytes));
     HIP_TRY(hipDeviceSynchronize());
@@ -2152,16 +2204,22 @@
     if (param_len != SYN_PARAM_DIM) return fail(SYN_ERR_PARAM_LEN, "length of params mismatch");
     if (B <= 0) return fail(SYN_ERR_INVALID, "syn_reconstruct: B=%d", B);
     if (!h->d_basis) return fail(SYN_ERR_NOT_LOADED, "syn_reconstruct: 3DMM basis not loaded");
+    const bool current = (dense & SYN_RECON_RECORDS_CURRENT) != 0;
+    dense &= ~SYN_RECON_RECORDS_CURRENT;
+    if (current && (h->fusion < 2 || !h->rec || h->rec_cur.param != param || h->rec_cur.B != B || h->rec_cur.transform != (transform != 0) ||
+                    h->rec_cur.roi != roi))
+        return fail(SYN_ERR_STALE_RECORDS, "syn_reconstruct: SYN_RECON_RECORDS_CURRENT, but the handle's records are not those of this batch "
+                    "(they belong to the last syn_forward_tail_u8 that reported records_current, with the same param / roi pointers, B and transform)");
     const int n = dense ? h->n_vert : h->n_lmk;
     if (row_pitch < n) return fail(SYN_ERR_INVALID, "syn_reconstruct: row_pitch=%d < %d columns", row_pitch, n);
     DeviceGuard g(h->device);
     int rc = ensure_rec(h, B);
     if (rc) return rc;
-    float *rec = h->rec;
+    float *rec = current ? rec_region(h, h->rec_cur.slot) : rec_region(h, 0);
     hipStream_t s = (hipStream_t)stream;
     if (h->fusion >= 2)
         syn::launch_reconstruct_f16(param, basis_mean_cs(h), basis_std_cs(h), dense ? basis_f16_dense(h) : basis_f16_lmk(h), n, dense ? h->nvp : h->nlp,
-                                   roi, transform, out, row_pitch, pad_writable, B, s, rec);
+                                   roi, transform, out, row_pitch, pad_writable, B, s, rec, nullptr, current);
     else
         syn::launch_reconstruct(param, basis_mean(h), basis_std(h), dense ? basis_dense(h) : basis_lmk(h), n, dense ? h->nvp : h->nlp,
                                 roi, transform, out, row_pitch, B, s, rec);
diff --git a/synergynet_amd/csrc/tail_face.h b/synergynet_amd/csrc/tail_face.h
--- /dev/null
+++ b/synergynet_amd/csrc/tail_face.h
@@ -0,0 +1,189 @@
+#pragma once
+#include "syn_internal.h"
+
+#ifdef __HIPCC__
+namespace syn {
+
+typedef float f32x2 __attribute__((ext_vector_type(2)));
+typedef float f32x4 __attribute__((ext_vector_type(4)));
+typedef unsigned u32x4 __attribute__((ext_vector_type(4)));
+
+__device__ __forceinline__ void pose_of_face(const float (&p)[12], const float *__restrict__ roi5 , double *__restrict__ angles3 ,
+                                             float *__restrict__ t3d3, float *__restrict__ pmat12 ) {
+    const float n1 = sqrtf(p[0] * p[0] + p[1] * p[1] + p[2] * p[2]);
+    const float n2 = sqrtf(p[4] * p[4] + p[5] * p[5] + p[6] * p[6]);
+    const float r1[3] = {p[0] / n1, p[1] / n1, p[2] / n1};
+    const float r2[3] = {p[4] / n2, p[5] / n2, p[6] / n2};
+    const float r3[3] = {r1[1] * r2[2] - r1[2] * r2[1], r1[2] * r2[0] - r1[0] * r2[2], r1[0] * r2[1] - r1[1] * r2[0]};
+    const double PI = 3.14159265358979323846;
+    double x, y, z;
+    if (r3[0] != 1.0f && r3[0] != -1.0f) {
+        x = asin((double)r3[0]);
+        const double cx = cos(x);
+        y = atan2((double)r2[2] / cx, (double)r3[2] / cx);
+        z = atan2((double)r1[1] / cx, (double)r1[0] / cx);
+    } else {
+        z = 0.0;
+        if (r3[0] == -1.0f) { x = PI / 2; y = z + atan2((double)r1[1], (double)r1[2]); }
+        else                { x = -PI / 2; y = -z + atan2(-(double)r1[1], -(double)r1[2]); }
+    }
+    if (pmat12) {
+        float *m = pmat12;
+        m[0] = r1[0]; m[1] = r1[1]; m[2] = r1[2]; m[3] = p[3];
+        m[4] = r2[0]; m[5] = r2[1]; m[6] = r2[2]; m[7] = p[7];
+        m[8] = r3[0]; m[9] = r3[1]; m[10] = r3[2]; m[11] = p[11];
+    }
+    if (!angles3) return;
+    angles3[0] = x * 180.0 / PI;
+    angles3[1] = y * 180.0 / PI;
+    angles3[2] = z * 180.0 / PI;
+    float tx = p[3], ty = p[7], tz = p[11];
+    if (roi5) {
+        const float sx = roi5[0], sy = roi5[1], ex = roi5[2], ey = roi5[3];
+        tx = tx * ((ex - sx) / 120.0f) + sx;
+        ty = ty * ((ey - sy) / 120.0f) + sy;
+    }
+    t3d3[0] = tx;
+    t3d3[1] = ty;
+    t3d3[2] = tz;
+}
+
+__device__ __forceinline__ void lmk_affine(const float *p, const float *__restrict__ roi , int b, int transform, float (&aff)[12]) {
+#pragma unroll
+    for (int c = 0; c < 3; ++c) {
+        float sc = 1.0f, of = 0.0f;
+        if (roi) {
+            const float sx = roi[b * 5 + 0], sy = roi[b * 5 + 1], ex = roi[b * 5 + 2], ey = roi[b * 5 + 3];
+            const float scx = (ex - sx) / 120.0f, scy = (ey - sy) / 120.0f;
+            if (c == 0) { sc = scx; of = sx; }
+            else if (c == 1) { sc = scy; of = sy; }
+            else { sc = (scx + scy) * 0.5f; }
+        }
+        float m0 = p[4 * c + 0], m1 = p[4 * c + 1], m2 = p[4 * c + 2], t = p[4 * c + 3];
+        if (transform && c == 1) { m0 = -m0; m1 = -m1; m2 = -m2; t = (float)(kImg + 1) - t; }
+        aff[3 * c + 0] = m0 * sc;
+        aff[3 * c + 1] = m1 * sc;
+        aff[3 * c + 2] = m2 * sc;
+        aff[9 + c] = t * sc + of;
+    }
+}
+
+template <bool SB = false>
+__device__ __forceinline__ void lmk_of_point(const float *p, const float *__restrict__ basis , const float (&aff)[12], int v,
+                                             int n_lmk, int b, float *__restrict__ lmk ) {
+    const int T = v >> 5, j = v & 31;
+    float S[3];
+#pragma unroll
+    for (int c = 0; c < 3; ++c) {
+        const float *bc = basis + ((size_t)T * 3 + c) * (kBasisK * 32);
+        float acc = 0.f;
+#pragma unroll
+        for (int t = 0; t < 6; ++t)
+#pragma unroll
+            for (int h = 0; h < 2; ++h) {
+                const f32x4 w = *(const f32x4 *)(bc + t * 256 + (32 * h + j) * 4);
+#pragma unroll
+                for (int s = 0; s < 4; ++s) acc = __builtin_fmaf(w[s], p[12 + 8 * t + 4 * h + s], acc);
+            }
+        const f32x2 w0 = *(const f32x2 *)(bc + 6 * 256 + j * 2), w1 = *(const f32x2 *)(bc + 6 * 256 + (32 + j) * 2);
+        acc = __builtin_fmaf(w0[0], p[12 + 48], acc);
+        acc = __builtin_fmaf(w0[1], p[12 + 49], acc);
+        acc += w1[0];
+        S[c] = acc;
+        if (SB) __builtin_amdgcn_sched_barrier(0);
+    }
+#pragma unroll
+    for (int c = 0; c < 3; ++c)
+        lmk[((size_t)b * 3 + c) * n_lmk + v] = aff[3 * c + 0] * S[0] + aff[3 * c + 1] * S[1] + aff[3 * c + 2] * S[2] + aff[9 + c];
+}
+
+__device__ __forceinline__ void split2r(float x0, float x1, unsigned &a, unsigned &b) {
+    a = __builtin_bit_cast(unsigned, __builtin_amdgcn_cvt_pkrtz(x0, x1));
+    float r0, r1;
+    asm("v_fma_mix_f32 %0, %1, -1.0, %2 op_sel_hi:[1,0,0]" : "=v"(r0) : "v"(a), "v"(x0));
+    asm("v_fma_mix_f32 %0, %1, -1.0, %2 op_sel:[1,0,0] op_sel_hi:[1,0,0]" : "=v"(r1) : "v"(a), "v"(x1));
+    b = __builtin_bit_cast(unsigned, __builtin_amdgcn_cvt_pkrtz(r0, r1));
+}
+
+__device__ __forceinline__ void recon_prep_lane(const float *pp, bool ok, int b, int l, const float *__restrict__ mean, const float *__restrict__ stdv,
+                                                const float *__restrict__ roi, int transform, unsigned *__restrict__ rt) {
+    const int i = l & 31, hh = l >> 5;
+    float al[3][8];
+    float amax = 0.f;
+#pragma unroll
+    for (int ks = 0; ks < 3; ++ks)
+#pragma unroll
+        for (int e = 0; e < 8; ++e) {
+            const int k = 12 + 16 * ks + 8 * hh + e;
+            al[ks][e] = ok ? pp[k] * stdv[k] + mean[k] : 0.f;
+            amax = fmaxf(amax, fabsf(al[ks][e]));
+        }
+    const float a48 = ok ? pp[12 + 48] * stdv[12 + 48] + mean[12 + 48] : 0.f;
+    const float a49 = ok ? pp[12 + 49] * stdv[12 + 49] + mean[12 + 49] : 0.f;
+    amax = fmaxf(amax, fmaxf(fabsf(a48), fabsf(a49)));
+#pragma unroll
+    for (int ks = 0; ks < 3; ++ks)
+#pragma unroll
+        for (int e = 0; e < 8; ++e) {
+            const int k = 12 + 16 * ks + 8 * (hh ^ 1) + e;
+            amax = fmaxf(amax, fabsf(ok ? pp[k] * stdv[k] + mean[k] : 0.f));
+        }
+    const float cu = mean[62];
+    amax = fmaxf(amax, cu);
+    int ex = (int)((__builtin_bit_cast(unsigned, amax) >> 23) & 0xff) - 126;
+    ex = 14 - ex;
+    const int ex_cu = (int)((__builtin_bit_cast(unsigned, cu) >> 23) & 0xff) - 127;
+    ex = ex < -14 - ex_cu ? -14 - ex_cu : ex;
+    ex = ex < -100 ? -100 : (ex > 100 ? 100 : ex);
+    const float Sa = __builtin_bit_cast(float, (unsigned)(127 + ex) << 23);
+    const float inv_ab = __builtin_bit_cast(float, (unsigned)(127 - ex) << 23);
+#pragma unroll
+    for (int ks = 0; ks < 3; ++ks) {
+        u32x4 pc[2];
+#pragma unroll
+        for (int d = 0; d < 4; ++d) {
+            unsigned a, b2;
+            split2r(al[ks][2 * d] * Sa, al[ks][2 * d + 1] * Sa, a, b2);
+            pc[0][d] = a; pc[1][d] = b2;
+        }
+#pragma unroll
+        for (int p = 0; p < 2; ++p) *(u32x4 *)&rt[((ks * 2 + p) * 64 + l) * 4] = pc[p];
+    }
+    {
+        unsigned a, b2;
+        split2r(a48 * Sa, a49 * Sa, a, b2);
+        const unsigned a8 = a & 0xffffu, b8 = b2 & 0xffffu, a9 = a >> 16, b9 = b2 >> 16;
+        const unsigned sa16 = ok ? (__builtin_bit_cast(unsigned, __builtin_amdgcn_cvt_pkrtz(cu * Sa, cu * Sa)) & 0xffffu) : 0u;
+        u32x4 fx = {0u, 0u, 0u, 0u};
+        if (hh == 0) fx = (u32x4){a8 | (b8 << 16), a8 | (a9 << 16), b9 | (a9 << 16), sa16 | (sa16 << 16)};
+        *(u32x4 *)&rt[(6 * 64 + l) * 4] = fx;
+    }
+    if (hh == 0) {
+        float r[16];
+        float p12[12];
+#pragma unroll
+        for (int q = 0; q < 12; ++q) p12[q] = ok ? pp[q] * stdv[q] + mean[q] : 0.f;
+#pragma unroll
+        for (int c = 0; c < 3; ++c) {
+            float sc = 1.0f, of = 0.0f;
+            if (roi && ok) {
+                const float sx = roi[b * 5 + 0], sy = roi[b * 5 + 1], ex = roi[b * 5 + 2], ey = roi[b * 5 + 3];
+                const float scx = (ex - sx) / 120.0f, scy = (ey - sy) / 120.0f;
+                if (c == 0) { sc = scx; of = sx; }
+                else if (c == 1) { sc = scy; of = sy; }
+                else { sc = (scx + scy) * 0.5f; }
+            }
+            float m0 = p12[4 * c + 0], m1 = p12[4 * c + 1], m2 = p12[4 * c + 2], t = p12[4 * c + 3];
+            if (transform && c == 1) { m0 = -m0; m1 = -m1; m2 = -m2; t = (float)(kImg + 1) - t; }
+            r[3 * c + 0] = m0 * sc * inv_ab; r[3 * c + 1] = m1 * sc * inv_ab; r[3 * c + 2] = m2 * sc * inv_ab;
+            r[9 + c] = t * sc + of;
+        }
+        r[12] = 0.f; r[13] = 0.f; r[14] = 0.f; r[15] = 0.f;
+        float *rr = reinterpret_cast<float *>(rt + 7 * 256) + i * 16;
+#pragma unroll
+        for (int q = 0; q < 4; ++q) *(f32x4 *)&rr[4 * q] = (f32x4){r[4 * q], r[4 * q + 1], r[4 * q + 2], r[4 * q + 3]};
+    }
+}
+
+}
+#endif
diff --git a/synergynet_amd/streams.py b/synergynet_amd/streams.py
--- a/synergynet_amd/streams.py
+++ b/synergynet_amd/streams.py
@@ -30,7 +30,7 @@
         if self._inflight[k] is not None:
             self.s_main.wait_event(self._inflight[k][1])
         with torch.cuda.stream(self.s_main):
-            param = m.forward_crops_u8(crops_u8)
+            param, lmk, pose, cur, rois_dev = m.forward_tail_u8(crops_u8, roi=rois, lmk_out=lmk_out, records=dense)
             ready = torch.cuda.Event()
             ready.record(self.s_main)
         s_tail = self.s_rec if dense else self.s_main
@@ -39,11 +39,10 @@
             if self._tail_stream is not s_tail and self.last_done is not None:
                 s_tail.wait_event(self.last_done)
             self._tail_stream = s_tail
-            lmk, pose = m.landmarks_and_pose(param, roi=rois, out=lmk_out)
-            mesh = m.reconstruct(param, roi=rois, dense=True, out=mesh_out) if dense else None
+            mesh = m.reconstruct(param, roi=rois_dev, dense=True, out=mesh_out, records_current=cur) if dense else None
             done = torch.cuda.Event()
             done.record(s_tail)
-        self._inflight[k] = ((param, lmk, mesh, pose, crops_u8, rois), done)
+        self._inflight[k] = ((param, lmk, mesh, pose, crops_u8, rois, rois_dev), done)
         self.last_done = done
         return param, lmk, mesh, pose
 
@@ -67,9 +66,8 @@
         m, st = self.models[i], self.streams[i]
         st.wait_stream(torch.cuda.current_stream(m.device))
         with torch.cuda.stream(st):
-            param = m.forward_crops_u8(crops_u8)
-            lmk, pose = m.landmarks_and_pose(param, roi=rois, out=lmk_out)
-            mesh = m.reconstruct(param, roi=rois, dense=True, out=mesh_out) if dense else None
+            param, lmk, pose, cur, rois_dev = m.forward_tail_u8(crops_u8, roi=rois, lmk_out=lmk_out, records=dense)
+            mesh = m.reconstruct(param, roi=rois_dev, dense=True, out=mesh_out, records_current=cur) if dense else None
             done = torch.cuda.Event()
             done.record(st)
         for t in (crops_u8, rois):
diff --git a/synergynet_amd/synergy3DMM.py b/synergynet_amd/synergy3DMM.py
--- a/synergynet_amd/synergy3DMM.py
+++ b/synergynet_amd/synergy3DMM.py
@@ -402,7 +402,34 @@
                                                                              pool.data_ptr() if return_pool else None, self._stream())))
         return (param, pool) if return_pool else param
 
-    def reconstruct(self, param, roi=None, dense=False, transform=True, out=None):
+    def forward_tail_u8(self, crops, roi=None, transform=True, lmk_out=None, records=False):
+        if not isinstance(crops, torch.Tensor):
+            crops = torch.as_tensor(np.asarray(crops))
+        if crops.dtype != torch.uint8 or crops.dim() != 4 or tuple(crops.shape[1:]) != (120, 120, 3):
+            raise RuntimeError('forward_crops_u8 expects uint8 [B,120,120,3]')
+        x = crops.to(self.device).contiguous()
+        B, n = x.shape[0], self._n_lmk
+        r = self._dev_f32(roi) if roi is not None else None
+        if r is not None and tuple(r.shape) != (B, 5):
+            raise RuntimeError('roi must be [B,5] (sx,sy,ex,ey,score)')
+        with torch.cuda.device(self.device):
+            if lmk_out is not None and (tuple(lmk_out.shape) != (B, 3, n) or lmk_out.dtype != torch.float32 or lmk_out.device != self.device):
+                raise RuntimeError(f'out must be a float32 [B,3,{n}] tensor on {self.device}')
+            if lmk_out is not None and not lmk_out.is_contiguous():
+                param = self.forward_crops_u8(x)
+                lmk, pose = self.landmarks_and_pose(param, roi=r, transform=transform, out=lmk_out)
+                return param, lmk, pose, False, r
+            param = torch.empty((B, 62), dtype=torch.float32, device=self.device)
+            lmk = lmk_out if lmk_out is not None else torch.empty((B, 3, n), dtype=torch.float32, device=self.device)
+            ang = torch.empty((B, 3), dtype=torch.float64, device=self.device)
+            t3d = torch.empty((B, 3), dtype=torch.float32, device=self.device)
+            cur = C.c_int(0)
+            self._guarded(lambda: abi.check(self._lib.syn_forward_tail_u8(
+                self._h, x.data_ptr(), B, int(transform), r.data_ptr() if r is not None else None, param.data_ptr(), None, lmk.data_ptr(),
+                ang.data_ptr(), t3d.data_ptr(), C.byref(cur) if records else None, self._stream())))
+        return param, lmk, (ang, t3d), bool(cur.value), r
+
+    def reconstruct(self, param, roi=None, dense=False, transform=True, out=None, records_current=False):
         p = self._dev_f32(param)
         if p.dim() != 2:
             raise RuntimeError('param must be [B,62]')
@@ -422,7 +449,8 @@
             if out.stride(2) != 1 or pitch < n or (B > 1 and out.stride(0) != 3 * pitch):
                 raise RuntimeError('out must have unit column stride and equally pitched rows (a [B,3,pitch][..., :n] view)')
             try:
-                abi.check(self._lib.syn_reconstruct_pitched(self._h, p.data_ptr(), B, p.shape[1], int(dense), int(transform),
+                abi.check(self._lib.syn_reconstruct_pitched(self._h, p.data_ptr(), B, p.shape[1],
+                                                            int(bool(dense)) | (abi.SYN_RECON_RECORDS_CURRENT if records_current else 0), int(transform),
                                                             r.data_ptr() if r is not None else None, out.data_ptr(), int(pitch),
                                                             int(getattr(out, '_syn_pad_writable', False)), self._stream()))
             except abi.SynergyHipError as e:
```

Result: no change. 1.024 million (median of 3 runs) (+0.0%).
